# contineu-ai/ACMMP-Spherical

Measured on AMD Instinct MI355X. Metric: Mpixels/sec PatchMatch propagation + ms/depth-map, 2000x1500, 1/2/4/8 GPU, higher is better.
Workload: dtype f32

## Files before the change

acmmp-spherical_amd/acmmp/capi.py:

```python
from __future__ import annotations

import ctypes as C
import dataclasses
import mmap
import os
import threading
import weakref

import numpy as np

from .types import CAMERA_DTYPE, PARAMS_DTYPE

HERE = os.path.dirname(os.path.abspath(__file__))
LIB_PATH = os.environ.get("ACMMP_LIB") or os.path.join(HERE, "libacmmp.so")

class _HostPool:

    def __init__(self, cap: int | None = None):
        if cap is None:
            cap = int(os.environ.get("ACMMP_HOST_POOL_BYTES", str(1 << 30)))
        self.cap, self.held = cap, 0
        self.free = {}
        self.order = []
        self.lock = threading.Lock()

    def take(self, n: int):
        with self.lock:
            lst = self.free.get(n)
            if lst:
                mm = lst.pop()
                self.order = [(k, m) for (k, m) in self.order if m is not mm]
                self.held -= n
                return mm
        mm = mmap.mmap(-1, n, flags=mmap.MAP_PRIVATE | mmap.MAP_ANONYMOUS)
        if hasattr(mmap, "MADV_HUGEPAGE"):
            mm.madvise(mmap.MADV_HUGEPAGE)
        return mm

    def give(self, mm, n: int):
        if n > self.cap:
            return
        with self.lock:
            while self.held + n > self.cap and self.order:
                k, old = self.order.pop(0)
                self.free[k].remove(old)
                self.held -= k
            self.free.setdefault(n, []).append(mm)
            self.order.append((n, mm))
            self.held += n

    def release(self):
        with self.lock:
            self.free, self.order, self.held = {}, [], 0


_POOL = _HostPool()


def host_empty(shape, dtype=np.float32) -> np.ndarray:
    dt = np.dtype(dtype)
    count = int(np.prod(shape))
    n = count * dt.itemsize
    if n < (4 << 20):
        return np.empty(shape, dt)
    size = (n + (2 << 20) - 1) // (2 << 20) * (2 << 20) + (2 << 20)
    mm = _POOL.take(size)
    base = np.frombuffer(mm, np.uint8)
    off = (-base.ctypes.data) % (2 << 20)
    del base
    flat = np.frombuffer(mm, dt, count, off)
    weakref.finalize(flat, _POOL.give, mm, size)
    return flat.reshape(shape)


STATUS = {0: "ok", 1: "invalid argument", 2: "HIP runtime error", 3: "out of device memory",
          4: "call order violated", 5: "unsupported configuration", 6: "no HIP device"}

EXPORTS = [
    "acmmp_abi_version", "acmmp_device_count", "acmmp_create", "acmmp_destroy", "acmmp_status_str", "acmmp_last_error",
    "acmmp_set_params", "acmmp_upload_views", "acmmp_upload_depths", "acmmp_set_state",
    "acmmp_set_scaled_state", "acmmp_set_planar_prior", "acmmp_run_patchmatch", "acmmp_run_patchmatch_ex",
    "acmmp_download", "acmmp_download_aux", "acmmp_device_outputs", "acmmp_synchronize", "acmmp_last_timing",
    "acmmp_last_kernel_timing", "acmmp_last_work", "acmmp_last_planar_timing", "acmmp_texel_bytes", "acmmp_set_math", "acmmp_get_math", "acmmp_jbu",
    "acmmp_debug_ncc", "acmmp_debug_geom", "acmmp_debug_ncc_nb", "acmmp_debug_ncc_ref", "acmmp_debug_band_cvec",
    "acmmp_support_points", "acmmp_delaunay", "acmmp_prior_plane_params", "acmmp_depth_from_plane_param",
    "acmmp_planar_prior_host", "acmmp_set_planar_prior_from_maps", "acmmp_set_planar_prior_from_state",
    "acmmp_download_planar_prior",
    "acmmp_upload_depths_device", "acmmp_upload_views_device", "acmmp_export_depth", "acmmp_export_state", "acmmp_set_state_device", "acmmp_device_alloc", "acmmp_device_free", "acmmp_memcpy",
    "acmmp_comm_unique_id", "acmmp_comm_create", "acmmp_comm_destroy", "acmmp_comm_broadcast", "acmmp_comm_after",
    "acmmp_comm_allreduce_max", "acmmp_comm_band_exchange", "acmmp_run_patchmatch_band",
    "acmmp_band_begin", "acmmp_band_sweep", "acmmp_band_sweeps_left", "acmmp_band_halo_ranges",
    "acmmp_band_copy_rows", "acmmp_band_get_rows", "acmmp_band_set_rows", "acmmp_band_end",
    "acmmp_strip_plan",
    "acmmp_fusion_create", "acmmp_fusion_set_view", "acmmp_fusion_run", "acmmp_fusion_last_error",
    "acmmp_fusion_destroy", "acmmp_fusion_run_scene", "acmmp_fusion_scene_points", "acmmp_fusion_reset_used",
    "acmmp_fusion_download_used", "acmmp_fusion_voxelize", "acmmp_fusion_voxel_points", "acmmp_fusion_voxel_table",
    "acmmp_fusion_set_scene", "acmmp_fusion_voxel_clean", "acmmp_fusion_clean_points", "acmmp_fusion_voxel_labels",
    "acmmp_fusion_component_table",
    "acmmp_fusion_voxel_visibility", "acmmp_fusion_visible_points", "acmmp_fusion_visibility_tallies",
    "acmmp_fusion_voxel_mesh", "acmmp_fusion_mesh_vertices", "acmmp_fusion_mesh_faces", "acmmp_fusion_mesh_samples",
    "acmmp_fusion_mesh_table", "acmmp_fusion_set_mesh", "acmmp_fusion_mesh_render", "acmmp_fusion_render_maps",
    "acmmp_fusion_render_plan",
    "acmmp_fusion_set_reference_cloud", "acmmp_fusion_cloud_distance", "acmmp_fusion_distance_results",
    "acmmp_fusion_distance_grid",
    "acmmp_fusion_surface_distance", "acmmp_fusion_surface_results", "acmmp_fusion_surface_plan",
    "acmmp_fusion_surface_grid",
    "acmmp_fusion_set_cloud_transform", "acmmp_fusion_get_cloud_transform", "acmmp_fusion_cloud_align",
    "acmmp_fusion_align_records", "acmmp_fusion_cloud_align_plane", "acmmp_fusion_align_plane_records",
    "acmmp_image_cache_create", "acmmp_image_cache_destroy", "acmmp_image_cache_stats",
    "acmmp_upload_views_keyed", "acmmp_device_checksum", "acmmp_device_identity", "acmmp_clock_probe",
]


class AcmmpError(RuntimeError):
    pass


def strip_plan(rows: int, want_strips: int):
    L = load_library()
    bounds = np.zeros(65, np.int32)
    waits = np.full(192, -1, np.int32)
    ns = int(L.acmmp_strip_plan(int(rows), int(want_strips), _p(bounds), _p(waits)))
    if ns < 1:
        raise AcmmpError(f"strip_plan: invalid arguments (rows={rows})")
    return [int(b) for b in bounds[:ns + 1]], [[int(w) for w in waits[3 * i:3 * i + 3] if w >= 0] for i in range(ns)]


_lib = None


def load_library(path: str = LIB_PATH):
    global _lib
    if _lib is not None:
        return _lib
    if not os.path.exists(path):
        raise AcmmpError(f"{path} is missing: build it with `python acmmp-spherical_amd/build.py` "
                         "(there is no CPU fallback)")
    L = C.CDLL(path)
    vp, i32, u64 = C.c_void_p, C.c_int, C.c_uint64
    L.acmmp_abi_version.restype = i32
    L.acmmp_device_count.restype = i32
    L.acmmp_create.argtypes = [i32, C.POINTER(vp)]
    L.acmmp_destroy.argtypes = [vp]
    L.acmmp_destroy.restype = None
    L.acmmp_status_str.argtypes = [i32]
    L.acmmp_status_str.restype = C.c_char_p
    L.acmmp_last_error.argtypes = [vp]
    L.acmmp_last_error.restype = C.c_char_p
    L.acmmp_set_params.argtypes = [vp, vp]
    L.acmmp_upload_views.argtypes = [vp, i32, vp, vp, vp]
    L.acmmp_upload_depths.argtypes = [vp, i32, vp, vp, vp]
    L.acmmp_set_state.argtypes = [vp, vp, vp]
    L.acmmp_set_scaled_state.argtypes = [vp, vp, i32, i32]
    L.acmmp_set_planar_prior.argtypes = [vp, vp, vp]
    L.acmmp_run_patchmatch.argtypes = [vp, u64]
    L.acmmp_run_patchmatch_ex.argtypes = [vp, u64, i32, i32]
    L.acmmp_download.argtypes = [vp, vp, vp]
    L.acmmp_download_aux.argtypes = [vp, vp, vp]
    L.acmmp_device_outputs.argtypes = [vp, C.POINTER(vp), C.POINTER(vp)]
    L.acmmp_last_timing.argtypes = [vp, vp]
    L.acmmp_last_kernel_timing.argtypes = [vp, vp, vp]
    L.acmmp_last_work.argtypes = [vp, vp, vp]
    L.acmmp_last_planar_timing.argtypes = [vp, vp]
    L.acmmp_texel_bytes.argtypes = [vp]
    L.acmmp_set_math.argtypes = [vp, i32]
    L.acmmp_get_math.argtypes = [vp]
    L.acmmp_synchronize.argtypes = [vp]
    L.acmmp_jbu.argtypes = [vp, vp, i32, i32, vp, i32, i32, i32, vp]
    L.acmmp_debug_ncc.argtypes = [vp, i32, vp, vp, vp, vp]
    L.acmmp_debug_geom.argtypes = [vp, i32, vp, vp, vp, vp]
    L.acmmp_debug_ncc_nb.argtypes = [vp, i32, vp, vp, vp, vp]
    L.acmmp_debug_ncc_ref.argtypes = [vp, i32, vp, vp, vp, vp]
    L.acmmp_support_points.argtypes = [vp, i32, i32, vp, i32, vp]
    L.acmmp_delaunay.argtypes = [vp, i32, i32, i32, vp, i32, vp]
    L.acmmp_prior_plane_params.argtypes = [vp, vp, i32, i32, vp, vp]
    L.acmmp_depth_from_plane_param.argtypes = [vp, vp, i32, i32]
    L.acmmp_upload_depths_device.argtypes = [vp, i32, vp, vp, vp]
    L.acmmp_upload_views_device.argtypes = [vp, i32, vp, vp, vp]
    L.acmmp_export_depth.argtypes = [vp, vp]
    L.acmmp_export_state.argtypes = [vp, vp, vp]
    L.acmmp_set_state_device.argtypes = [vp, vp, vp]
    L.acmmp_device_alloc.argtypes = [i32, C.c_size_t, C.POINTER(vp)]
    L.acmmp_device_free.argtypes = [i32, vp]
    L.acmmp_memcpy.argtypes = [i32, vp, vp, C.c_size_t, i32]
    L.acmmp_comm_unique_id.argtypes = [vp]
    L.acmmp_comm_create.argtypes = [i32, vp, i32, i32, C.POINTER(vp)]
    L.acmmp_comm_destroy.argtypes = [vp]
    L.acmmp_comm_broadcast.argtypes = [vp, i32, vp, vp, vp]
    L.acmmp_comm_after.argtypes = [vp, vp]
    L.acmmp_comm_allreduce_max.argtypes = [vp, vp, i32]
    L.acmmp_comm_band_exchange.argtypes = [vp, vp, i32, i32, i32]
    L.acmmp_run_patchmatch_band.argtypes = [vp, vp, u64, i32, i32, i32, i32]
    L.acmmp_band_begin.argtypes = [vp, u64, i32, i32]
    L.acmmp_band_sweep.argtypes = [vp, C.POINTER(i32)]
    L.acmmp_band_sweeps_left.argtypes = [vp]
    L.acmmp_band_halo_ranges.argtypes = [vp, vp]
    L.acmmp_strip_plan.argtypes = [i32, i32, vp, vp]
    L.acmmp_band_copy_rows.argtypes = [vp, vp, i32, i32, i32]
    L.acmmp_band_get_rows.argtypes = [vp, i32, i32, i32, vp, vp, vp]
    L.acmmp_band_set_rows.argtypes = [vp, i32, i32, i32, vp, vp, vp]
    L.acmmp_debug_band_cvec.argtypes = [vp, i32, i32, i32, vp]
    L.acmmp_band_end.argtypes = [vp, i32]
    L.acmmp_fusion_create.argtypes = [i32, i32, vp, C.POINTER(vp)]
    L.acmmp_fusion_set_view.argtypes = [vp, i32, vp, vp, vp]
    L.acmmp_fusion_run.argtypes = [vp, i32, i32, vp, vp, i32, vp]
    L.acmmp_fusion_last_error.argtypes = [vp]
    L.acmmp_fusion_destroy.argtypes = [vp]
    L.acmmp_fusion_run_scene.argtypes = [vp, i32, vp, vp, vp, i32, vp, C.POINTER(C.c_int64)]
    L.acmmp_fusion_scene_points.argtypes = [vp, C.c_int64, C.c_int64, vp, vp, vp, vp]
    L.acmmp_fusion_reset_used.argtypes = [vp]
    L.acmmp_fusion_download_used.argtypes = [vp, i32, vp]
    L.acmmp_fusion_voxelize.argtypes = [vp, C.c_float, vp, i32, vp, vp, vp, vp]
    L.acmmp_fusion_voxel_points.argtypes = [vp, C.c_int64, C.c_int64, vp, vp]
    L.acmmp_fusion_voxel_table.argtypes = [vp, C.c_int64, vp, vp, vp, vp]
    L.acmmp_fusion_set_scene.argtypes = [vp, C.c_int64, vp, vp, vp, vp]
    L.acmmp_fusion_voxel_clean.argtypes = [vp, i32, i32, C.c_int64, C.c_int64, vp, vp, vp, vp, vp]
    L.acmmp_fusion_clean_points.argtypes = [vp, C.c_int64, C.c_int64, vp, vp, vp]
    L.acmmp_fusion_voxel_labels.argtypes = [vp, C.c_int64, C.c_int64, vp, vp]
    L.acmmp_fusion_component_table.argtypes = [vp, C.c_int64, C.c_int64, vp, vp, vp]
    L.acmmp_fusion_voxel_visibility.argtypes = [vp, i32, i32, vp, C.c_float, i32, i32, i32, vp, vp, vp, vp]
    L.acmmp_fusion_visible_points.argtypes = [vp, C.c_int64, C.c_int64, vp, vp, vp]
    L.acmmp_fusion_visibility_tallies.argtypes = [vp, C.c_int64, C.c_int64, vp]
    L.acmmp_fusion_voxel_mesh.argtypes = [vp, i32, i32, vp, C.c_float, i32, vp, vp, vp, vp, vp, vp]
    L.acmmp_fusion_mesh_vertices.argtypes = [vp, C.c_int64, C.c_int64, vp]
    L.acmmp_fusion_mesh_faces.argtypes = [vp, C.c_int64, C.c_int64, vp]
    L.acmmp_fusion_mesh_samples.argtypes = [vp, C.c_int64, C.c_int64, vp, vp, vp]
    L.acmmp_fusion_mesh_table.argtypes = [vp, C.c_int64, vp, vp, vp, vp]
    L.acmmp_fusion_set_mesh.argtypes = [vp, C.c_int64, vp, C.c_int64, vp]
    L.acmmp_fusion_mesh_render.argtypes = [vp, i32, vp, C.c_float, vp, vp]
    L.acmmp_fusion_render_maps.argtypes = [vp, vp, vp, vp, vp]
    L.acmmp_fusion_render_plan.argtypes = [vp, i32, vp, vp, vp]
    L.acmmp_fusion_set_reference_cloud.argtypes = [vp, C.c_int64, vp]
    L.acmmp_fusion_cloud_distance.argtypes = [vp, i32, i32, C.c_float, i32, vp, vp]
    L.acmmp_fusion_distance_results.argtypes = [vp, C.c_int64, C.c_int64, vp, vp]
    L.acmmp_fusion_distance_grid.argtypes = [vp, C.c_float, vp, vp, vp, vp]
    L.acmmp_fusion_surface_distance.argtypes = [vp, i32, C.c_float, i32, vp, vp]
    L.acmmp_fusion_surface_results.argtypes = [vp, C.c_int64, C.c_int64, vp, vp]
    L.acmmp_fusion_surface_plan.argtypes = [vp, i32, vp, vp, vp, vp]
    L.acmmp_fusion_surface_grid.argtypes = [vp, C.c_float, vp, vp, vp, vp]
    L.acmmp_fusion_set_cloud_transform.argtypes = [vp, vp]
    L.acmmp_fusion_get_cloud_transform.argtypes = [vp, vp, vp]
    L.acmmp_fusion_cloud_align.argtypes = [vp, i32, i32, C.c_float, i32, i32, C.c_double, vp, vp, vp, vp]
    L.acmmp_fusion_align_records.argtypes = [vp, C.c_int64, C.c_int64, vp, vp, vp]
    L.acmmp_fusion_cloud_align_plane.argtypes = [vp, i32, C.c_float, i32, i32, C.c_double, vp, vp, vp, vp]
    L.acmmp_fusion_align_plane_records.argtypes = [vp, C.c_int64, C.c_int64, vp, vp, vp]
    L.acmmp_planar_prior_host.argtypes = [vp, vp, vp, i32, i32, C.c_float, C.c_float, vp, vp, vp]
    L.acmmp_set_planar_prior_from_maps.argtypes = [vp, vp, vp, C.c_float, C.c_float, vp]
    L.acmmp_set_planar_prior_from_state.argtypes = [vp, C.c_float, C.c_float, vp]
    L.acmmp_download_planar_prior.argtypes = [vp, vp, vp]
    L.acmmp_image_cache_create.argtypes = [i32, C.c_size_t, C.POINTER(vp)]
    L.acmmp_image_cache_destroy.argtypes = [vp]
    L.acmmp_image_cache_stats.argtypes = [vp, vp]
    L.acmmp_upload_views_keyed.argtypes = [vp, vp, i32, vp, vp, vp, vp, i32]
    L.acmmp_device_checksum.argtypes = [i32, vp, C.c_size_t, vp]
    L.acmmp_device_identity.argtypes = [i32, vp, i32, vp]
    L.acmmp_clock_probe.argtypes = [i32, C.c_float, vp]
    for name in EXPORTS:
        fn = getattr(L, name)
        if name not in ("acmmp_destroy", "acmmp_status_str", "acmmp_last_error", "acmmp_abi_version", "acmmp_device_count",
                        "acmmp_depth_from_plane_param", "acmmp_comm_destroy", "acmmp_fusion_last_error",
                        "acmmp_fusion_destroy", "acmmp_image_cache_destroy"):
            fn.restype = i32
    L.acmmp_depth_from_plane_param.restype = C.c_float
    L.acmmp_fusion_last_error.restype = C.c_char_p
    L.acmmp_image_cache_destroy.restype = None
    _lib = L
    return L


def device_count() -> int:
    return int(load_library().acmmp_device_count())


def _p(a):
    return None if a is None else a.ctypes.data_as(C.c_void_p)


def checksum_host(arr) -> int:
    w = np.frombuffer(np.ascontiguousarray(arr).tobytes(), np.uint32).astype(np.uint64)
    z = (np.arange(w.size, dtype=np.uint64) << np.uint64(32)) | w
    with np.errstate(over="ignore"):
        z = (z ^ (z >> np.uint64(30))) * np.uint64(0xbf58476d1ce4e5b9)
        z = (z ^ (z >> np.uint64(27))) * np.uint64(0x94d049bb133111eb)
        z = z ^ (z >> np.uint64(31))
# ... 220 lines not shown
        return n.value

    def download_planar_prior(self):
        prior = host_empty((self.H, self.W, 4), np.float32)
        masks = host_empty((self.H, self.W), np.uint32)
        self._check(self.L.acmmp_download_planar_prior(self.h, _p(prior), _p(masks)), "download_planar_prior")
        return prior, masks

    def run_patchmatch(self, seed: int, n_half_sweeps: int = -1, do_post: bool = True):
        self._check(self.L.acmmp_run_patchmatch_ex(self.h, C.c_uint64(seed), n_half_sweeps, int(do_post)),
                    "run_patchmatch")

    def download(self):
        planes = host_empty((self.H, self.W, 4), np.float32)
        costs = host_empty((self.H, self.W), np.float32)
        self._check(self.L.acmmp_download(self.h, _p(planes), _p(costs)), "download")
        return planes, costs

    def download_into(self, planes, costs):
        for a, tail in ((planes, (4,)), (costs, ())):
            if a.dtype != np.float32 or not a.flags.c_contiguous or a.shape != (self.H, self.W) + tail:
                raise ValueError("download_into: need C-contiguous float32 (H, W, 4) planes and (H, W) costs")
        self._check(self.L.acmmp_download(self.h, _p(planes), _p(costs)), "download")

    def download_rows_into(self, planes, costs, row0: int, row1: int):
        n = row1 - row0
        for a, tail in ((planes, (4,)), (costs, ())):
            if a.dtype != np.float32 or not a.flags.c_contiguous or a.shape != (n, self.W) + tail:
                raise ValueError("download_rows_into: need C-contiguous float32 (rows, W, 4) and (rows, W)")
        if not (0 <= row0 < row1 <= self.H):
            raise ValueError("download_rows_into: rows outside the view")
        pp, cp = self.device_outputs()
        dev = self.device
        _host_check(self.L.acmmp_memcpy(dev, _p(planes), C.c_void_p(pp + 16 * row0 * self.W), 16 * n * self.W, 1),
                    "memcpy D2H")
        _host_check(self.L.acmmp_memcpy(dev, _p(costs), C.c_void_p(cp + 4 * row0 * self.W), 4 * n * self.W, 1),
                    "memcpy D2H")

    def download_aux(self):
        sel = host_empty((self.H, self.W), np.uint32)
        pre = host_empty((self.H, self.W), np.float32)
        self._check(self.L.acmmp_download_aux(self.h, _p(sel), _p(pre)), "download_aux")
        return sel, pre

    def device_outputs(self):
        a, b = C.c_void_p(), C.c_void_p()
        self._check(self.L.acmmp_device_outputs(self.h, C.byref(a), C.byref(b)), "device_outputs")
        return a.value, b.value

    BAND_HALO = 23

    def band_begin(self, seed: int, row0: int, row1: int):
        self._check(self.L.acmmp_band_begin(self.h, seed, row0, row1), "band_begin")

    def band_sweep(self) -> int:
        colour = C.c_int32(0)
        self._check(self.L.acmmp_band_sweep(self.h, C.byref(colour)), "band_sweep")
        return colour.value

    def band_sweeps_left(self) -> int:
        return int(self.L.acmmp_band_sweeps_left(self.h))

    def band_halo_ranges(self):
        r = np.zeros(8, np.int32)
        self._check(self.L.acmmp_band_halo_ranges(self.h, _p(r)), "band_halo_ranges")
        return tuple((int(r[2 * k]), int(r[2 * k + 1])) for k in range(4))

    def band_copy_rows_from(self, src: "Context", colour: int, row_a: int, row_b: int):
        self._check(self.L.acmmp_band_copy_rows(self.h, src.h, colour, row_a, row_b), "band_copy_rows")

    def band_get_rows(self, colour: int, row_a: int, row_b: int) -> np.ndarray:
        n = (row_b - row_a) * ((self.W + 1) // 2)
        pl = np.empty((n, 4), np.float32)
        co = np.empty(n, np.float32)
        sel = np.empty(n, np.uint32)
        self._check(self.L.acmmp_band_get_rows(self.h, colour, row_a, row_b, _p(pl), _p(co), _p(sel)), "band_get_rows")
        return np.concatenate([pl.view(np.uint32), co.view(np.uint32)[:, None], sel[:, None]], axis=1)

    def debug_band_cvec(self, colour: int, row_a: int, row_b: int) -> np.ndarray:
        out = np.empty((self.N - 1, (row_b - row_a) * ((self.W + 1) // 2)), np.float32)
        self._check(self.L.acmmp_debug_band_cvec(self.h, colour, row_a, row_b, _p(out)), "debug_band_cvec")
        return out

    def band_set_rows(self, colour: int, row_a: int, row_b: int, rows: np.ndarray):
        rows = np.asarray(rows, np.uint32).reshape(-1, 6)
        pl = np.ascontiguousarray(rows[:, :4]).view(np.float32)
        co = np.ascontiguousarray(rows[:, 4]).view(np.float32)
        sel = np.ascontiguousarray(rows[:, 5])
        self._check(self.L.acmmp_band_set_rows(self.h, colour, row_a, row_b, _p(pl), _p(co), _p(sel)), "band_set_rows")

    def band_end(self, do_post: bool = True):
        self._check(self.L.acmmp_band_end(self.h, int(do_post)), "band_end")

    def run_patchmatch_band(self, seed: int, row0: int, row1: int, comm=None, rank_up: int = -1,
                            rank_down: int = -1):
        self._check(self.L.acmmp_run_patchmatch_band(self.h, comm.h if comm is not None else None, seed, row0, row1,
                                                     rank_up, rank_down), "run_patchmatch_band")

    def synchronize(self):
        self._check(self.L.acmmp_synchronize(self.h), "synchronize")

    def last_timing(self):
        ms = np.zeros(3, np.float32)
        self._check(self.L.acmmp_last_timing(self.h, _p(ms)), "last_timing")
        return {"init_ms": float(ms[0]), "prop_ms": float(ms[1]), "post_ms": float(ms[2])}

    KERNELS = ("k_eval_nb", "k_select", "k_eval_ref", "k_finish")

    def last_kernel_timing(self):
        ms = np.zeros(4, np.float32)
        n = np.zeros(4, np.int32)
        self._check(self.L.acmmp_last_kernel_timing(self.h, _p(ms), _p(n)), "last_kernel_timing")
        return {k: (float(ms[i]), int(n[i])) for i, k in enumerate(self.KERNELS)}

    def last_work(self):
        e, t = C.c_ulonglong(0), C.c_ulonglong(0)
        self._check(self.L.acmmp_last_work(self.h, C.byref(e), C.byref(t)), "last_work")
        return e.value, t.value

    def last_planar_timing(self):
        ms = np.zeros(4, np.float32)
        self._check(self.L.acmmp_last_planar_timing(self.h, _p(ms)), "last_planar_timing")
        return {"support_ms": float(ms[0]), "delaunay_ms": float(ms[1]), "planes_ms": float(ms[2]),
                "device_ms": float(ms[3])}

    def texel_bytes(self) -> int:
        return int(self.L.acmmp_texel_bytes(self.h))

    def jbu(self, ref, coarse, imagescale: int):
        ref = np.ascontiguousarray(ref, np.float32)
        coarse = np.ascontiguousarray(coarse, np.float32)
        out = np.empty_like(ref)
        self._check(self.L.acmmp_jbu(self.h, _p(ref), ref.shape[1], ref.shape[0], _p(coarse), coarse.shape[1],
                                     coarse.shape[0], imagescale, _p(out)), "jbu")
        return out

    def _debug(self, fn, px, py, planes):
        px = np.ascontiguousarray(px, np.int32)
        py = np.ascontiguousarray(py, np.int32)
        pl = np.ascontiguousarray(planes, np.float32).reshape(-1, 4)
        out = np.empty((len(px), self.N - 1), np.float32)
        self._check(fn(self.h, len(px), _p(px), _p(py), _p(pl), _p(out)), "debug")
        return out

    def debug_ncc(self, px, py, planes):
        return self._debug(self.L.acmmp_debug_ncc, px, py, planes)

    def debug_geom(self, px, py, planes):
        return self._debug(self.L.acmmp_debug_geom, px, py, planes)

    def _debug_k(self, fn, k, px, py, planes, what):
        px = np.ascontiguousarray(px, np.int32)
        py = np.ascontiguousarray(py, np.int32)
        pl = np.ascontiguousarray(planes, np.float32).reshape(len(px), k, 4)
        out = np.empty((len(px), k, self.N - 1), np.float32)
        self._check(fn(self.h, len(px), _p(px), _p(py), _p(pl), _p(out)), what)
        return out

    def debug_ncc_nb(self, px, py, planes):
        return self._debug_k(self.L.acmmp_debug_ncc_nb, 8, px, py, planes, "debug_ncc_nb")

    def debug_ncc_ref(self, px, py, planes):
        return self._debug_k(self.L.acmmp_debug_ncc_ref, 5, px, py, planes, "debug_ncc_ref")



# ... 612 lines not shown
```

acmmp-spherical_amd/csrc/capi.cpp:

```cpp
#include "../../include/acmmp.h"

#include <hip/hip_runtime.h>

#include <algorithm>
#include <chrono>
#include <cmath>
#include <cstdio>
#include <cstdlib>
#include <cstring>
#include <mutex>
#include <string>
#include <type_traits>
#include <unordered_map>
#include <vector>

#include "devbuf.h"
#include "engine.h"
#include "planar.h"

using namespace acmmp;

static_assert(sizeof(acmmp_camera) == 120, "Camera layout (main.h:40-54)");
static_assert(sizeof(acmmp_params) == 68, "PatchMatchParams layout (ACMMP.h:32-55)");
static_assert(offsetof(acmmp_params, scaled_cols) == 52, "PatchMatchParams layout");
// ... 756 lines not shown
    const acmmp_status st = planar_triangles(c->cams[0], depths, costs, c->W, c->H, &pt);
    if (st != ACMMP_OK) return fail(c, st, "planar_triangles");
    c->planar_ms[0] = 0.f;
    c->planar_ms[1] = pt.delaunay_ms;
    c->planar_ms[2] = ms_since(t0) - pt.delaunay_ms;
    return upload_planar(c, pt, depth_min, depth_max, n_triangles);
}

acmmp_status acmmp_set_planar_prior_from_state(acmmp_ctx* c, float depth_min, float depth_max, int* n_triangles) {
    if (!c) return ACMMP_ERR_INVALID_ARGUMENT;
    if (c->N == 0) return fail(c, ACMMP_ERR_STATE, "upload_views and run_patchmatch first");
    if (!c->has_result) return fail(c, ACMMP_ERR_STATE, "no depth / cost maps since the last upload_views");
    HIP_TRY(c, hipSetDevice(c->device));
    const int W = c->W, H = c->H;
    const size_t nb = static_cast<size_t>((W + 4) / 5) * ((H + 4) / 5);
    const auto t0 = planar_clock::now();
    HIP_TRY(c, c->d_support.reserve_pow2(nb, static_cast<size_t>(1) << 17));
    HIP_TRY(c, launch_support_points(c->d_costs_rm, c->d_planes_rm, W, H, c->d_support, c->stream));
    std::vector<int4> blocks(nb);
    HIP_TRY(c, hipMemcpyAsync(blocks.data(), c->d_support, sizeof(int4) * nb, hipMemcpyDeviceToHost, c->stream));
    HIP_TRY(c, hipStreamSynchronize(c->stream));
    std::vector<int> xy;
    std::vector<float> depth_at;
    for (const int4& b : blocks) {
        if (!b.x) continue;
        xy.push_back(b.y);
        xy.push_back(b.z);
        float d;
        std::memcpy(&d, &b.w, sizeof d);
        depth_at.push_back(d);
    }
    c->planar_ms[0] = ms_since(t0);
    const auto t1 = planar_clock::now();
    PlanarTriangles pt;
    const acmmp_status st = planar_triangles_pts(c->cams[0], xy, depth_at, W, H, &pt);
    if (st != ACMMP_OK) return fail(c, st, "planar_triangles");
    c->planar_ms[1] = pt.delaunay_ms;
    c->planar_ms[2] = ms_since(t1) - pt.delaunay_ms;
    return upload_planar(c, pt, depth_min, depth_max, n_triangles);
}

acmmp_status acmmp_download_planar_prior(acmmp_ctx* c, float* prior, uint32_t* masks) {
    if (!c) return ACMMP_ERR_INVALID_ARGUMENT;
    if (!c->has_prior) return fail(c, ACMMP_ERR_STATE, "no planar prior set since the last upload_views");
    HIP_TRY(c, hipSetDevice(c->device));
    HIP_TRY(c, hipStreamSynchronize(c->stream));
    const size_t P = P_of(c);
    if (prior) HIP_TRY(c, d2h(prior, c->d_prior, sizeof(float4) * P));
    if (masks) HIP_TRY(c, d2h(masks, c->d_mask, sizeof(uint32_t) * P));
    return ACMMP_OK;
}

static unsigned long long colour_pixels(const acmmp_ctx* c, const KParams& kp, int colour) {
    unsigned long long n = 0;
    for (int y = kp.row_lo; y < kp.row_hi; ++y) {
        const int first = (y + colour) & 1;
        n += first < c->W ? static_cast<unsigned long long>((c->W - first + 1) / 2) : 0ull;
    }
    return n;
}

static int ref_split_point(int V, size_t Pc, bool interp_ref) {
    const char* e_on = std::getenv("ACMMP_REF_SPLIT");
    const char* e_at = std::getenv("ACMMP_REF_SPLIT_AT");
    const int enabled = e_on ? std::atoi(e_on) : 1;
    const int at = e_at ? std::atoi(e_at) : 0;
    if (!enabled || V < 2 || Pc >= (static_cast<size_t>(1) << 29)) return 0;
    if (at > 0) return at < V ? at : 0;
    if (interp_ref && V > 8) return 8;
    return V <= 4 ? V / 2 : 4;
}

static int default_strips(int model, int W, int H, int V) {
    return (model == kSphere && V <= 4 && static_cast<long long>(W) * H >= 2000000LL) ? 2 : 1;
}

int acmmp_strip_plan(int rows, int want_strips, int* bounds, int* waits) {
    if (rows < 1 || !bounds) return 0;
    const int ns = strip_plan(rows, want_strips, bounds);
    for (int i = 0; waits && i < ns; ++i) strip_waits(ns, i, waits + 3 * i);
    return ns;
}

static acmmp_status build_kparams(acmmp_ctx* c, KParams& kp, uint64_t seed, int want_strips = 1) {
    const acmmp_params& p = c->params;
    if (!c->has_params) return fail(c, ACMMP_ERR_STATE, "set_params first");
    if (c->N == 0) return fail(c, ACMMP_ERR_STATE, "upload_views first");
    if (p.num_images != c->N) return fail(c, ACMMP_ERR_INVALID_ARGUMENT, "params.num_images != uploaded images");
    if (p.geom_consistency && !c->has_depths) return fail(c, ACMMP_ERR_STATE, "geom_consistency needs upload_depths");
    if (p.planar_prior && !c->has_prior) return fail(c, ACMMP_ERR_STATE, "planar_prior needs set_planar_prior");
    if (!p.geom_consistency && p.hierarchy && !p.planar_prior && !c->has_scaled)
        return fail(c, ACMMP_ERR_STATE, "hierarchy needs set_scaled_state");
    if (p.upsample && !p.planar_prior && p.hierarchy &&
        (c->sw != static_cast<int>(p.scaled_cols) || c->sh != static_cast<int>(p.scaled_rows)))
        return fail(c, ACMMP_ERR_INVALID_ARGUMENT, "scaled_cols/rows != scaled state size");
    if (p.hierarchy && !p.upsample && !p.geom_consistency && !p.planar_prior && (c->sw != c->W || c->sh != c->H))
        return fail(c, ACMMP_ERR_INVALID_ARGUMENT, "hierarchy reuse needs a full-size scaled state");
    const int R = p.patch_size / 2;
    if (R > 64) return fail(c, ACMMP_ERR_UNSUPPORTED, "patch radius > 64");
    int nside = 0;
    for (int i = -R; i <= R; i += p.radius_increment) ++nside;
    kp = KParams{};
    kp.model = c->model;
    kp.W = c->W; kp.H = c->H; kp.Wh = Wh_of(c); kp.N = c->N; kp.V = c->N - 1;
    kp.R = R; kp.inc = p.radius_increment; kp.nside = nside; kp.S = nside * nside;
    kp.interp = c->model == kSphere && nside == 6 && 2000LL * R <= 5LL * c->W && 1000LL * R <= 5LL * c->H;
    kp.ref_neg_tau = -1.0f;
    if (kp.interp && c->math == ACMMP_MATH_FAST && c->tex16 && kp.V <= 4) {
        kp.ref_neg_tau = 0x1p-35f;
        if (const char* e = std::getenv("ACMMP_REF_NEG_TAU")) kp.ref_neg_tau = std::strtof(e, nullptr);
        if (const char* e = std::getenv("ACMMP_REF_NEG_SKIP")) if (std::atoi(e) == 0) kp.ref_neg_tau = -1.0f;
    }
    if (const char* e = std::getenv("ACMMP_INTERP")) kp.interp = kp.interp && std::atoi(e) != 0;
    kp.homog = 1;
    if (const char* e = std::getenv("ACMMP_PIN_HOMOG")) kp.homog = std::atoi(e) != 0;
    kp.spread_max = 256.0f;
    if (const char* e = std::getenv("ACMMP_SPREAD_MAX")) kp.spread_max = std::strtof(e, nullptr);
    kp.neg_tau = 0x1p-35f;
    if (const char* e = std::getenv("ACMMP_NEG_TAU")) kp.neg_tau = std::strtof(e, nullptr);
    if (const char* e = std::getenv("ACMMP_NEG_SKIP")) if (std::atoi(e) == 0) kp.neg_tau = -1.0f;
    kp.rows = std::min(c->H, 32 * (((c->H / 2) + 15) / 16));
    kp.row_lo = 0; kp.row_hi = kp.rows;
    kp.init_lo = 0; kp.init_hi = c->H;
    kp.merge_lo = 0; kp.merge_hi = c->H;
    for (int k = 0; k < 2; ++k) { kp.filt_lo[k] = 0; kp.filt_hi[k] = kp.rows; }
    kp.dpitch = c->W + 2 * R;
    kp.depth_min = p.depth_min; kp.depth_max = p.depth_max;
    kp.sigma_spatial = p.sigma_spatial; kp.sigma_color = p.sigma_color;
    kp.top_k = p.top_k;
    kp.geom = p.geom_consistency; kp.planar = p.planar_prior; kp.hier = p.hierarchy; kp.upsample = p.upsample;
    kp.scaled_cols = p.scaled_cols; kp.scaled_rows = p.scaled_rows;
    kp.sw = c->sw; kp.sh = c->sh;
    kp.seed_lo = static_cast<uint32_t>(seed);
    kp.seed_hi = static_cast<uint32_t>(seed >> 32);
    kp.Pc = static_cast<long long>(c->H) * kp.Wh;
    const size_t Pc = static_cast<size_t>(kp.Pc);

    if (kp.S > 64) return fail(c, ACMMP_ERR_UNSUPPORTED, "more than 64 patch samples (patch_size / radius_increment)");
    kp.cams = c->d_cams;
    if (c->dirs_R != R) {
        if (c->model == kSphere) {
            c->d_dirs.reset();
            HIP_TRY(c, c->d_sph_row.alloc(static_cast<size_t>(c->H + 2 * R)));
            HIP_TRY(c, c->d_sph_col.alloc(static_cast<size_t>(c->W + 2 * R)));
        } else {
            HIP_TRY(c, c->d_dirs.alloc(static_cast<size_t>(c->W + 2 * R) * (c->H + 2 * R)));
        }
        HIP_TRY(c, launch_ray_tables(kp, c->d_dirs, c->d_sph_row, c->d_sph_col, c->stream));
        c->dirs_R = R;
    }
    kp.color_den = 2.0f * p.sigma_color * p.sigma_color;
    HIP_TRY(c, c->d_spatial.reserve(static_cast<size_t>(c->model == kSphere ? c->H : 1) * kp.S));
    HIP_TRY(c, launch_spatial_table(kp, c->d_spatial, c->stream));
    kp.nb_chunk = nb_view_chunk(kp);
    kp.nb_tile = nb_tile_order(kp);
    size_t fix_max_pc = static_cast<size_t>(1) << 24;
    if (const char* e = std::getenv("ACMMP_NBFIX_MAX_PC")) fix_max_pc = std::min<size_t>(fix_max_pc, std::strtoull(e, nullptr, 10));
    const bool fixq = c->model == kSphere && c->math == ACMMP_MATH_FAST && c->tex16 && kp.interp && Pc < fix_max_pc;
    if (!fixq && c->model == kSphere && c->math == ACMMP_MATH_FAST && c->tex16 && kp.interp && Pc >= fix_max_pc) kp.interp = 0;
    if (!kp.interp || !kp.nb_tile) kp.neg_tau = -1.0f;
    if (c->math == ACMMP_MATH_FAST && (c->model != kSphere || (kp.interp && kp.V > 4))) want_strips = 1;
    int sb[kMaxStrips + 1];
    const int ns = strip_plan(kp.rows, want_strips, sb);
    const int ref_split = ref_split_point(kp.V, Pc, kp.model == kSphere && c->math == ACMMP_MATH_FAST && c->tex16 &&
                                                        kp.interp && kp.V > 4);
    size_t ref_blocks[kMaxStrips], fix_cap[kMaxStrips], fix_total = 0, ref_total = 0;
    for (int i = 0; i < ns; ++i) {
        const size_t srows = static_cast<size_t>(sb[i + 1] - sb[i]);
        const size_t nb_blocks = static_cast<size_t>(nb_block_count(static_cast<long long>(srows), kp.Wh, kp.nb_tile));
        ref_blocks[i] = (srows * kp.Wh + kRefPix - 1) / kRefPix;
        fix_cap[i] = !fixq ? 0 : std::max(
            (nb_blocks + kNbFixRegions - 1) / kNbFixRegions * kNbPix * 8 * static_cast<size_t>(kp.nb_chunk),
            (ref_blocks[i] + kNbFixRegions - 1) / kNbFixRegions * kRefSlots * static_cast<size_t>(std::max(ref_split, 0)));
        fix_total += fix_cap[i];
        ref_total += ref_blocks[i];
    }
    kp.cams = c->d_cams;
    kp.tex16 = c->tex16;
    kp.fast = c->math == ACMMP_MATH_FAST;
    kp.dep = c->d_dep;
    kp.dirs = c->d_dirs;
    kp.sph_row = c->d_sph_row;
    kp.sph_col = c->d_sph_col;
    kp.spatial = c->d_spatial;
    kp.planes_rm = c->d_planes_rm; kp.w_rm = c->d_w_rm; kp.costs_rm = c->d_costs_rm; kp.pre_rm = c->d_pre; kp.sel_rm = c->d_sel_rm;
    kp.scaled = c->d_scaled; kp.prior = c->d_prior; kp.mask = c->d_mask;
    for (int k = 0; k < 2; ++k) {
        kp.plane_cs[k] = c->d_plane_cs[k][0];
        kp.cost_cs[k] = c->d_cost_cs[k][0];
        kp.sel_cs[k] = c->d_sel_cs[k];
        kp.rng_cs[k] = c->d_rng_cs[k];
    }
    uint8_t* dead = nullptr;
    auto carve = [&](char* slab) -> size_t {
        size_t at = 0;
        auto piece = [&](auto*& field, size_t count) {
            using T = std::remove_reference_t<decltype(*field)>;
            field = slab ? reinterpret_cast<T*>(slab + at) : nullptr;
            at = (at + sizeof(T) * count + 255) & ~static_cast<size_t>(255);
        };
        const size_t VP = static_cast<size_t>(kp.V) * Pc;
        const size_t surv_n = std::max(5 * Pc + 256, ref_total * kRefSlots);
        piece(kp.hyp_cost, 8 * VP);
        piece(kp.nbpos, 8 * Pc);
        piece(kp.cand, 5 * Pc);
        piece(kp.cand_dep, 5 * Pc);
        piece(kp.cand_cost, 5 * Pc);
        piece(kp.pst, Pc);
        piece(kp.cvec[0], VP);
        piece(kp.cvec[1], VP);
        piece(kp.cand_vcost, 5 * VP);
        piece(kp.surv, surv_n);
        piece(kp.surv_count, std::max(Pc / 51 + 2, ref_total));
        piece(kp.psum, Pc);
        piece(kp.nbfix, kNbFixRegions * fix_total);
        piece(kp.nbfix_count, static_cast<size_t>(kNbFixRegions) * ns);
        piece(kp.surv_pre, std::max(Pc / 51 + 3, ref_total + ns));
        piece(kp.surv_dense, surv_n);
        piece(kp.cand_rough, 5 * Pc);
        piece(dead, 2 * Pc);
        return at;
    };
    HIP_TRY(c, c->d_scratch.reserve(carve(nullptr)));
    carve(c->d_scratch);
    if (!fixq) kp.nbfix = nullptr;
    {
        const char* e = std::getenv("ACMMP_DEAD_SKIP");
        const bool skip = c->model == kSphere && !(e && std::atoi(e) == 0);
        for (int k = 0; k < 2; ++k) kp.dead[k] = skip ? dead + k * Pc : nullptr;
    }
    kp.nbfix_cap = static_cast<unsigned>(fix_cap[0]);
    c->strips.assign(ns, StripSlice{});
    {
        size_t ref_at = 0, fix_at = 0;
        for (int i = 0; i < ns; ++i) {
            StripSlice& t = c->strips[i];
            t.row_lo = sb[i]; t.row_hi = sb[i + 1];
            t.surv = kp.surv + ref_at * kRefSlots;
            t.surv_count = kp.surv_count + ref_at;
            t.surv_pre = kp.surv_pre + ref_at + i;
            t.surv_dense = kp.surv_dense + ref_at * kRefSlots;
            t.nbfix = kp.nbfix ? kp.nbfix + kNbFixRegions * fix_at : nullptr;
            t.nbfix_count = kp.nbfix_count + kNbFixRegions * i;
            t.nbfix_cap = static_cast<unsigned>(fix_cap[i]);
            ref_at += ref_blocks[i];
            fix_at += fix_cap[i];
        }
    }
    kp.ref_split = ref_split;
    if (!c->d_work) HIP_TRY(c, c->d_work.alloc(258));
    kp.work = c->d_work;
    kp.status = reinterpret_cast<unsigned*>(c->d_work + 256);
    kp.dead_any = reinterpret_cast<unsigned*>(c->d_work + 257);
    kp.nb_views = kp.V >= 32 ? 0xFFFFFFFFu : ((1u << kp.V) - 1u);
    kp.nb_count_work = 1;
    return ACMMP_OK;
}

static acmmp_status run_begin(acmmp_ctx* c, const KParams& kp, hipStream_t s) {
    const size_t Pc = static_cast<size_t>(kp.Pc);
    HIP_TRY(c, hipMemsetAsync(c->d_work, 0, sizeof(unsigned long long) * 258, s));
    HIP_TRY(c, hipEventRecord(c->ev[0], s));
    HIP_TRY(c, launch_init(kp, s));
    for (int k = 0; k < 2; ++k) {
        HIP_TRY(c, hipMemcpyAsync(c->d_plane_cs[k][1], c->d_plane_cs[k][0], sizeof(float4) * Pc,
                                  hipMemcpyDeviceToDevice, s));
        HIP_TRY(c, hipMemcpyAsync(c->d_cost_cs[k][1], c->d_cost_cs[k][0], sizeof(float) * Pc,
                                  hipMemcpyDeviceToDevice, s));
    }
    HIP_TRY(c, hipEventRecord(c->ev[1], s));
    return ACMMP_OK;
}

static acmmp_status run_end(acmmp_ctx* c, const KParams& kp, const int cur[2], int do_post) {
    hipStream_t s = c->stream;
    HIP_TRY(c, hipEventRecord(c->ev[2], s));
    HIP_TRY(c, launch_post(kp, do_post, s));
    HIP_TRY(c, hipEventRecord(c->ev[3], s));
    if (!c->h_work) HIP_TRY(c, c->h_work.alloc(257));
    HIP_TRY(c, hipMemcpyAsync(c->h_work, c->d_work, sizeof(unsigned long long) * 257, hipMemcpyDeviceToHost, s));
    HIP_TRY(c, hipStreamSynchronize(s));
    for (int k = 0; k < 2; ++k) {
        if (cur[k]) {
            std::swap(c->d_plane_cs[k][0], c->d_plane_cs[k][1]);
            std::swap(c->d_cost_cs[k][0], c->d_cost_cs[k][1]);
        }
    }
    for (int i = 0; i < 3; ++i) HIP_TRY(c, hipEventElapsedTime(&c->timing[i], c->ev[i], c->ev[i + 1]));
    if (const unsigned long long status = c->h_work[256])
        return fail(c, ACMMP_ERR_HIP, "run status " + std::to_string(status) + ": an interpolation fallback queue overflowed");
    c->has_result = true;
    return ACMMP_OK;
}

acmmp_status acmmp_run_patchmatch_ex(acmmp_ctx* c, uint64_t seed, int n_half_sweeps, int do_post) {
    if (!c) return ACMMP_ERR_INVALID_ARGUMENT;
    HIP_TRY(c, hipSetDevice(c->device));
// ... 144 lines not shown
    c->band_cur[0] = c->band_cur[1] = 0;
    c->band_active = true;
    return ACMMP_OK;
}

acmmp_status acmmp_band_sweep(acmmp_ctx* c, int* colour_out) {
    if (!c) return ACMMP_ERR_INVALID_ARGUMENT;
    if (!c->band_active) return fail(c, ACMMP_ERR_STATE, "band_begin first");
    if (c->band_sw >= c->band_nsw) return fail(c, ACMMP_ERR_STATE, "every half-sweep of the run is done");
    HIP_TRY(c, hipSetDevice(c->device));
    KParams& kp = c->band_kp;
    const int sw = c->band_sw, colour = sw & 1, iter = sw / 2;
    int* cur = c->band_cur;
    SweepOut out{c->d_plane_cs[colour][cur[colour] ^ 1], c->d_cost_cs[colour][cur[colour] ^ 1]};
    HIP_TRY(c, launch_propagate(kp, colour, iter, out, c->stream, nullptr));
    cur[colour] ^= 1;
    kp.plane_cs[colour] = c->d_plane_cs[colour][cur[colour]];
    kp.cost_cs[colour] = c->d_cost_cs[colour][cur[colour]];
    ++c->band_sw;
    if (colour_out) *colour_out = colour;
    return ACMMP_OK;
}

int acmmp_band_sweeps_left(const acmmp_ctx* c) { return c && c->band_active ? c->band_nsw - c->band_sw : 0; }

acmmp_status acmmp_band_halo_ranges(const acmmp_ctx* c, int ranges[8]) {
    if (!c || !ranges) return ACMMP_ERR_INVALID_ARGUMENT;
    if (!c->band_active) return ACMMP_ERR_STATE;
    band_ranges(c->band_kp, c->band_lo, c->band_hi, ranges[0], ranges[1], ranges[2], ranges[3], ranges[4], ranges[5],
                ranges[6], ranges[7]);
    return ACMMP_OK;
}

acmmp_status acmmp_band_copy_rows(acmmp_ctx* dst, acmmp_ctx* src, int colour, int row_a, int row_b) {
    if (!dst || !src || dst == src) return ACMMP_ERR_INVALID_ARGUMENT;
    BandBuffers d{}, s{};
    acmmp_status st = band_buffers(dst, colour, &d);
    if (st == ACMMP_OK) st = band_buffers(src, colour, &s);
    if (st != ACMMP_OK) return st;
    if (d.Wh != s.Wh || dst->H != src->H || row_a < 0 || row_b > dst->H || row_a > row_b)
        return fail(dst, ACMMP_ERR_INVALID_ARGUMENT, "band contexts differ in size or rows out of range");
    if (row_a == row_b) return ACMMP_OK;
    HIP_TRY(src, hipSetDevice(src->device));
    HIP_TRY(src, hipStreamSynchronize(src->stream));
    HIP_TRY(dst, hipSetDevice(dst->device));
    const size_t off = static_cast<size_t>(row_a) * d.Wh, n = static_cast<size_t>(row_b - row_a) * d.Wh;
    HIP_TRY(dst, hipMemcpyAsync(d.plane + off, s.plane + off, sizeof(float4) * n, hipMemcpyDeviceToDevice, dst->stream));
    HIP_TRY(dst, hipMemcpyAsync(d.cost + off, s.cost + off, sizeof(float) * n, hipMemcpyDeviceToDevice, dst->stream));
    HIP_TRY(dst, hipMemcpyAsync(d.sel + off, s.sel + off, sizeof(uint32_t) * n, hipMemcpyDeviceToDevice, dst->stream));
    return ACMMP_OK;
}

acmmp_status acmmp_band_get_rows(acmmp_ctx* c, int colour, int row_a, int row_b, float* planes, float* costs,
                                 uint32_t* sel) {
    if (!c || !planes || !costs || !sel) return ACMMP_ERR_INVALID_ARGUMENT;
    BandBuffers b{};
    const acmmp_status st = band_buffers(c, colour, &b);
    if (st != ACMMP_OK) return st;
    if (row_a < 0 || row_b > c->H || row_a > row_b) return fail(c, ACMMP_ERR_INVALID_ARGUMENT, "rows out of range");
    if (row_a == row_b) return ACMMP_OK;
    HIP_TRY(c, hipSetDevice(c->device));
    HIP_TRY(c, hipStreamSynchronize(c->stream));
    const size_t off = static_cast<size_t>(row_a) * b.Wh, n = static_cast<size_t>(row_b - row_a) * b.Wh;
    HIP_TRY(c, d2h(planes, b.plane + off, sizeof(float4) * n));
    HIP_TRY(c, d2h(costs, b.cost + off, sizeof(float) * n));
    HIP_TRY(c, d2h(sel, b.sel + off, sizeof(uint32_t) * n));
    return ACMMP_OK;
}

acmmp_status acmmp_debug_band_cvec(acmmp_ctx* c, int colour, int row_a, int row_b, float* out) {
    if (!c || !out) return ACMMP_ERR_INVALID_ARGUMENT;
    BandBuffers b{};
    const acmmp_status st = band_buffers(c, colour, &b);
    if (st != ACMMP_OK) return st;
    if (row_a < 0 || row_b > c->H || row_a > row_b) return fail(c, ACMMP_ERR_INVALID_ARGUMENT, "rows out of range");
    if (row_a == row_b) return ACMMP_OK;
    HIP_TRY(c, hipSetDevice(c->device));
    HIP_TRY(c, hipStreamSynchronize(c->stream));
    const KParams& kp = c->band_kp;
    const size_t off = static_cast<size_t>(row_a) * b.Wh, n = static_cast<size_t>(row_b - row_a) * b.Wh;
    for (int v = 0; v < kp.V; ++v)
        HIP_TRY(c, d2h(out + static_cast<size_t>(v) * n, kp.cvec[colour] + static_cast<size_t>(v) * kp.Pc + off, sizeof(float) * n));
    return ACMMP_OK;
}

acmmp_status acmmp_band_set_rows(acmmp_ctx* c, int colour, int row_a, int row_b, const float* planes, const float* costs,
                                 const uint32_t* sel) {
    if (!c || !planes || !costs || !sel) return ACMMP_ERR_INVALID_ARGUMENT;
    BandBuffers b{};
    const acmmp_status st = band_buffers(c, colour, &b);
    if (st != ACMMP_OK) return st;
    if (row_a < 0 || row_b > c->H || row_a > row_b) return fail(c, ACMMP_ERR_INVALID_ARGUMENT, "rows out of range");
    if (row_a == row_b) return ACMMP_OK;
    HIP_TRY(c, hipSetDevice(c->device));
    const size_t off = static_cast<size_t>(row_a) * b.Wh, n = static_cast<size_t>(row_b - row_a) * b.Wh;
    HIP_TRY(c, hipMemcpyAsync(b.plane + off, planes, sizeof(float4) * n, hipMemcpyHostToDevice, c->stream));
    HIP_TRY(c, hipMemcpyAsync(b.cost + off, costs, sizeof(float) * n, hipMemcpyHostToDevice, c->stream));
    HIP_TRY(c, hipMemcpyAsync(b.sel + off, sel, sizeof(uint32_t) * n, hipMemcpyHostToDevice, c->stream));
    HIP_TRY(c, hipStreamSynchronize(c->stream));
    return ACMMP_OK;
}

acmmp_status acmmp_band_end(acmmp_ctx* c, int do_post) {
    if (!c) return ACMMP_ERR_INVALID_ARGUMENT;
    if (!c->band_active) return fail(c, ACMMP_ERR_STATE, "band_begin first");
    HIP_TRY(c, hipSetDevice(c->device));
    const acmmp_status st = run_end(c, c->band_kp, c->band_cur, do_post);
    c->band_active = false;
    return st;
}

acmmp_status acmmp_download(acmmp_ctx* c, float* planes, float* costs) {
    if (!c) return ACMMP_ERR_INVALID_ARGUMENT;
    if (c->N == 0) return fail(c, ACMMP_ERR_STATE, "nothing to download");
    HIP_TRY(c, hipSetDevice(c->device));
    const size_t P = P_of(c);
    if (planes) HIP_TRY(c, d2h(planes, c->d_planes_rm, sizeof(float4) * P));
    if (costs) HIP_TRY(c, d2h(costs, c->d_costs_rm, sizeof(float) * P));
    return ACMMP_OK;
}

acmmp_status acmmp_download_aux(acmmp_ctx* c, uint32_t* sel, float* pre) {
    if (!c) return ACMMP_ERR_INVALID_ARGUMENT;
    if (c->N == 0) return fail(c, ACMMP_ERR_STATE, "nothing to download");
    HIP_TRY(c, hipSetDevice(c->device));
    const size_t P = P_of(c);
    if (sel) HIP_TRY(c, d2h(sel, c->d_sel_rm, sizeof(uint32_t) * P));
    if (pre) HIP_TRY(c, d2h(pre, c->d_pre, sizeof(float) * P));
    return ACMMP_OK;
}

acmmp_status acmmp_device_outputs(acmmp_ctx* c, void** planes, void** costs) {
    if (!c) return ACMMP_ERR_INVALID_ARGUMENT;
    if (planes) *planes = c->d_planes_rm;
    if (costs) *costs = c->d_costs_rm;
    return ACMMP_OK;
}

acmmp_status acmmp_synchronize(acmmp_ctx* c) {
    if (!c) return ACMMP_ERR_INVALID_ARGUMENT;
    HIP_TRY(c, hipSetDevice(c->device));
    HIP_TRY(c, hipDeviceSynchronize());
    return ACMMP_OK;
}

acmmp_status acmmp_last_timing(const acmmp_ctx* c, float ms[3]) {
    if (!c || !ms) return ACMMP_ERR_INVALID_ARGUMENT;
    for (int i = 0; i < 3; ++i) ms[i] = c->timing[i];
    return ACMMP_OK;
}

acmmp_status acmmp_last_planar_timing(const acmmp_ctx* c, float ms[4]) {
    if (!c || !ms) return ACMMP_ERR_INVALID_ARGUMENT;
    for (int i = 0; i < 4; ++i) ms[i] = c->planar_ms[i];
    return ACMMP_OK;
}

acmmp_status acmmp_last_work(const acmmp_ctx* c, unsigned long long* evaluated, unsigned long long* total) {
    if (!c || !evaluated || !total) return ACMMP_ERR_INVALID_ARGUMENT;
    *evaluated = c->work_busy;
    *total = c->work_total;
    return ACMMP_OK;
}

int acmmp_texel_bytes(const acmmp_ctx* c) {
    if (!c || c->N == 0) return 0;
// ... 76 lines not shown
```

acmmp-spherical_amd/csrc/engine.h:

```cpp
#pragma once
#include <hip/hip_runtime.h>
#include <stdint.h>

#include "acmmp.h"

namespace acmmp {

constexpr int kPinhole = 0;
constexpr int kSphere = 11;
constexpr int kMaxViews = 32;
constexpr int kNbPix = 32;
constexpr int kNbFixRegions = 256;
constexpr int kRefLanes = 5;
constexpr int kRefPix = 51;
constexpr int kRefSlots = kRefPix * kRefLanes;
constexpr unsigned kStatusFixOverflow = 1u;

struct DevCam {
    float FRxy[6];
    float FRz[3];
    float Ft[3];
    float fkx, fky;
    float cx, cy;
    const uint16_t* img16_base;
// ... 12 lines not shown
    float inv_fx, inv_fy;
    float C[3];
    long long dep_off;
    int dep_w, dep_h;
    int img_bytes;
    const float* img_base;
};

struct PixState {
    float4 plane_now;
    float4 cur_plane;
    uint4 vw;
    float cost_now, depth_now, cur_cost, restricted_cost;
    uint32_t cur_sel, flags;
    float weight_norm;
    uint32_t src;
};

struct KParams {
    int model;
    int tex16;
    int fast;
    int W, H, Wh, N, V;
    int R, inc, nside, S;
    int interp;
    int homog;
    float spread_max;
    int rows;
    int row_lo, row_hi;
    int init_lo, init_hi;
    int merge_lo, merge_hi;
    int filt_lo[2], filt_hi[2];
    int dpitch;
    float depth_min, depth_max, sigma_spatial, sigma_color;
    int top_k;
    int geom, planar, hier, upsample;
    float scaled_cols, scaled_rows;
    int sw, sh;
    uint32_t seed_lo, seed_hi;
    const DevCam* cams;
    const float* dep;
    const float4* dirs;
    const float2* sph_row;
    const float2* sph_col;
    const float* spatial;
    float color_den;
    float neg_tau;
    float4* planes_rm;
    float* w_rm;
    float* costs_rm;
    float* pre_rm;
    uint32_t* sel_rm;
    const float4* scaled;
    const float4* prior;
    const uint32_t* mask;
    float4* plane_cs[2];
    float* cost_cs[2];
    uint32_t* sel_cs[2];
    uint32_t* rng_cs[2];
    float* hyp_cost;
    float* cvec[2];
    float* cand_vcost;
    int* nbpos;
    float4* cand;
    float* cand_dep;
    float* cand_cost;
    PixState* pst;
    unsigned long long* work;
    uint32_t nb_views;
    int nb_chunk;
    int nb_tile;
    int nb_count_work;
    long long Pc;
    int ref_split;
    float ref_neg_tau;
    uint32_t* surv;
    unsigned* surv_count;
    unsigned* surv_pre;
    uint32_t* surv_dense;
    float4* psum;
    uint32_t* nbfix;
    unsigned* nbfix_count;
    unsigned nbfix_cap;
    uint32_t* cand_rough;
    uint8_t* dead[2];
    unsigned* dead_any;
    unsigned* status;
};

struct SweepOut {
    float4* plane;
    float* cost;
};

constexpr int kMaxStrips = 64;
constexpr int kMaxStripStreams = 4;

struct StripSlice {
    int row_lo, row_hi;
    uint32_t* surv;
    unsigned* surv_count;
    unsigned* surv_pre;
    uint32_t* surv_dense;
    uint32_t* nbfix;
    unsigned* nbfix_count;
    unsigned nbfix_cap;
};

inline int strip_plan(int rows, int want, int* bounds) {
    const int units = rows / 4, per = (ACMMP_BAND_HALO + 3) / 4;
    int ns = want < 1 ? 1 : (want > kMaxStrips ? kMaxStrips : want);
    if (ns > units / per) ns = units / per;
    if (ns < 1) ns = 1;
    int at = 0;
    for (int i = 0; i < ns; ++i) {
        bounds[i] = 4 * at;
        at += units / ns + (i < units % ns ? 1 : 0);
    }
    bounds[0] = 0;
    bounds[ns] = rows;
    return ns;
}

inline void strip_waits(int ns, int i, int waits[3]) {
    waits[0] = (ns > 1 && i > 0) ? i - 1 : -1;
    waits[1] = ns > 1 ? i : -1;
    waits[2] = (ns > 1 && i + 1 < ns) ? i + 1 : -1;
}

inline int cdiv(long long a, int b) { return static_cast<int>((a + b - 1) / b); }

hipError_t launch_ray_tables(const KParams& kp, float4* dirs, float2* sph_row, float2* sph_col, hipStream_t s);
hipError_t launch_spatial_table(const KParams& kp, float* spatial, hipStream_t s);
hipError_t launch_init(const KParams& kp, hipStream_t s);
hipError_t launch_propagate(const KParams& kp, int colour, int iter, SweepOut out, hipStream_t s,
                            hipEvent_t* ev = nullptr, bool all_marks = true);
hipError_t launch_post(const KParams& kp, int do_post, hipStream_t s);
DevCam make_devcam(const acmmp_camera& cam);
void set_relative_frame(DevCam& d, const acmmp_camera& ref, const acmmp_camera& cam);
struct BandBuffers {
    float4* plane;
    float* cost;
    uint32_t* sel;
    int Wh;
    hipStream_t stream;
    int device;
};
acmmp_status band_buffers(acmmp_ctx* c, int colour, BandBuffers* out);
acmmp_status engine_stream(acmmp_ctx* c, int* device, hipStream_t* stream);

hipError_t launch_jbu(const float* ref, int W, int H, const float* coarse, int sw, int sh, int imagescale,
                      float* out, hipStream_t s);
hipError_t launch_export_depth(const float4* planes, long long P, float* dst, hipStream_t s);
hipError_t launch_copy(const void* src, void* dst, size_t bytes, hipStream_t s);
struct ClockStamp {
    unsigned long long cycles, ticks;
};
hipError_t launch_clock_probe(const float* rnd, int iters, int blocks, ClockStamp* stamps, float* sink, hipStream_t s);
hipError_t launch_checksum(const void* ptr, size_t bytes, unsigned long long* out, hipStream_t s);
int nb_view_chunk(const KParams& kp);
int nb_tile_order(const KParams& kp);
inline long long nb_block_count(long long rows, long long Wh, int tile) {
    return tile ? ((rows + 3) / 4) * ((Wh + 7) / 8) : (rows * Wh + 31) / 32;
}
hipError_t launch_debug(const KParams& kp, int which, int n, const int* px, const int* py, const float4* planes,
                        float* out, hipStream_t s);
hipError_t launch_debug_nb(const KParams& kp, int n, const int* px, const int* py, const float4* planes, float* out,
                           hipStream_t s);
hipError_t launch_debug_ref(const KParams& kp, int n, const int* px, const int* py, const float4* planes, float* out,
                            hipStream_t s);
hipError_t launch_to_f16_pairs(const float* src, int W, int H, uint32_t* dst, int* inexact, hipStream_t s);
// ... 14 lines not shown
```

acmmp-spherical_amd/csrc/kernels.hip:

```cpp
#include <algorithm>
#include <cstdlib>

#include "camera_dev.h"
#include "detmath.h"
#include "engine.h"

#ifndef ACMMP_TU
#define ACMMP_TU -1
#endif
#define ACMMP_IN_TU(n) (ACMMP_TU < 0 || ACMMP_TU == (n))

namespace acmmp {

typedef float f32x2 __attribute__((ext_vector_type(2)));
__device__ __forceinline__ f32x2 pk_fma(f32x2 a, f32x2 b, f32x2 c) { return __builtin_elementwise_fma(a, b, c); }
__device__ __forceinline__ f32x2 splat2(float x) { return (f32x2){x, x}; }


__device__ __forceinline__ uint4 philox10(uint32_t c0, uint32_t c1, uint32_t c2, uint32_t c3, uint32_t k0,
                                          uint32_t k1) {
#pragma unroll
    for (int r = 0; r < 10; ++r) {
        const uint32_t lo0 = 0xD2511F53u * c0, hi0 = __umulhi(0xD2511F53u, c0);
        const uint32_t lo1 = 0xCD9E8D57u * c2, hi1 = __umulhi(0xCD9E8D57u, c2);
// ... 143 lines not shown
    t = pk_fma((f32x2){c.FRxy[2], c.FRxy[3]}, splat2(P.y), t);
    t = pk_fma((f32x2){c.FRxy[4], c.FRxy[5]}, splat2(P.z), t);
    tz = fmaf(c.FRz[2], P.z, fmaf(c.FRz[1], P.y, fmaf(c.FRz[0], P.x, fz)));
}

template <int MODEL, typename Cam>
__device__ __forceinline__ void project_fast(Cam& c, float3 P, float& ox, float& oy, const float* ft = nullptr) {
    f32x2 t;
    float tz;
    rigid_fast(c, P, t, tz, ft);
    if (MODEL == kSphere) {
        sphere_pixel_fast(c, t, tz, ox, oy);
    } else {
        const f32x2 o = t * splat2(__builtin_amdgcn_rcpf(tz));
        ox = o.x;
        oy = o.y;
    }
}

template <int MODEL, typename Cam>
__device__ __forceinline__ float3 cam_point_fast(Cam& c, int x, int y, float depth, float4 d) {
    if (MODEL == kSphere) return make_float3(d.x * depth, d.y * depth, d.z * depth);
    return make_float3((depth * (static_cast<float>(x) - c.K[2])) * c.inv_fx,
                       (depth * (static_cast<float>(y) - c.K[5])) * c.inv_fy, depth);
}

__device__ __forceinline__ float depth_from_plane_fast(float4 ph, float4 d) {
    const float denom = dot3(ph.x, ph.y, ph.z, d.x, d.y, d.z);
    return (fabsf(denom) < 1e-6f) ? 1e6f : (-ph.w * __builtin_amdgcn_rcpf(denom));
}

__device__ __forceinline__ float dist_to_origin(float4 d, float depth, float4 n) {
    return -dot3(n.x, n.y, n.z, d.x * depth, d.y * depth, d.z * depth);
}

__device__ __forceinline__ float4 to_world(const DevCam& c, float4 n) {
    return make_float4(dot3(c.R[0], c.R[3], c.R[6], n.x, n.y, n.z), dot3(c.R[1], c.R[4], c.R[7], n.x, n.y, n.z),
                       dot3(c.R[2], c.R[5], c.R[8], n.x, n.y, n.z), n.w);
}
__device__ __forceinline__ float4 to_ref(const DevCam& c, float4 n) {
    return make_float4(dot3(c.R[0], c.R[1], c.R[2], n.x, n.y, n.z), dot3(c.R[3], c.R[4], c.R[5], n.x, n.y, n.z),
                       dot3(c.R[6], c.R[7], c.R[8], n.x, n.y, n.z), n.w);
}

__device__ __forceinline__ float dot3n(float4 a, float4 b) { return dot3(a.x, a.y, a.z, b.x, b.y, b.z); }


__device__ __forceinline__ int clampi(int v, int lo, int hi) { return v < lo ? lo : (v > hi ? hi : v); }

__device__ __forceinline__ float texel_padded(const float* img, int pitch, int W, int H, int ix, int iy) {
    return img[static_cast<long long>(clampi(iy, 0, H - 1) + 1) * pitch + clampi(ix, 0, W - 1) + 1];
}

__device__ __forceinline__ float texel_plain(const float* img, int W, int H, int ix, int iy) {
    return img[static_cast<long long>(clampi(iy, 0, H - 1)) * W + clampi(ix, 0, W - 1)];
}


template <int MODEL>
__device__ __forceinline__ float4 ray_at(const KParams& kp, int x, int y) {
    if (MODEL == kSphere) {
        const float2 r = kp.sph_row[y + kp.R];
        const float2 c = kp.sph_col[x + kp.R];
        return make_float4(r.y * c.x, -r.x, r.y * c.y, 0.0f);
    }
    return kp.dirs[static_cast<long long>(y + kp.R) * kp.dpitch + (x + kp.R)];
}
__device__ __forceinline__ long long cs_index(const KParams& kp, int x, int y) {
    return static_cast<long long>(y) * kp.Wh + (x >> 1);
}
__device__ __forceinline__ int uniform_int(int v) { return __builtin_amdgcn_readfirstlane(v); }


struct Patch {
    const float4* rw;
    const float* rr;
    const float2* wr;
    const float2* row;
    const float2* col;
    int stride;
    float center;
    float sbw, sref, srr;
    const uint32_t* neg = nullptr;
};

typedef float float2u __attribute__((ext_vector_type(2), aligned(4)));

__device__ __forceinline__ float bilinear_pair(const float* img, int pitch, int W, int H, float x, float y) {
    const float fx = floorf(x), fy = floorf(y);
    const float a = x - fx, b = y - fy;
    const int ix = clampi(f2i_sat(fx), -1, W - 1);
    const int iy = clampi(f2i_sat(fy), -1, H - 1);
    const float* p0 = img + static_cast<long long>(iy + 1) * pitch + (ix + 1);
    const float2u top = *reinterpret_cast<const float2u*>(p0);
    const float2u bot = *reinterpret_cast<const float2u*>(p0 + pitch);
    const float r0 = fmaf(a, top.y - top.x, top.x);
    const float r1 = fmaf(a, bot.y - bot.x, bot.x);
    return fmaf(b, r1 - r0, r0);
}

typedef unsigned u32x2 __attribute__((ext_vector_type(2)));
struct Tap {
    float a, b;
    f32x2 top, bot;
    u32x2 pw;
};

template <int TEX, bool Y_IN_RANGE, typename Cam>
__device__ __forceinline__ Tap fetch_tap(__amdgpu_buffer_rsrc_t rs, Cam& c, float x, float y) {
    const float fx = floorf(x), fy = floorf(y);
    Tap t;
    t.a = x - fx;
    t.b = y - fy;
    if (TEX == 1) {
        t.a = __builtin_amdgcn_fractf(x);
        t.b = __builtin_amdgcn_fractf(y);
        const unsigned ix4 = (static_cast<unsigned>(clamp_m1(cvt_flr_i32(x), c.Wm1)) << 2) + 4u;
        if (Y_IN_RANGE) {
            const unsigned off = mad_u24(static_cast<unsigned>(cvt_flr_i32(y)), c.pitch4, ix4);
            t.pw = __builtin_amdgcn_raw_buffer_load_b64(rs, off, c.pitch4, 0);
        } else {
            const unsigned off = mad_u24(static_cast<unsigned>(clamp_m1(cvt_flr_i32(y), c.Hm1) + 1), c.pitch4, ix4);
            t.pw = __builtin_amdgcn_raw_buffer_load_b64(rs, off, 0, 0);
        }
        return t;
    }
    const unsigned ix4 = (static_cast<unsigned>(clamp_m1(cvt_i32(fx), c.Wm1)) << 2) + 4u;
    if (Y_IN_RANGE) {
        const unsigned off = mad_u24(static_cast<unsigned>(cvt_i32(fy)), c.pitch4, ix4);
        t.top = __builtin_bit_cast(f32x2, __builtin_amdgcn_raw_buffer_load_b64(rs, off, c.pitch4, 0));
        t.bot = __builtin_bit_cast(f32x2, __builtin_amdgcn_raw_buffer_load_b64(rs, off, 2 * c.pitch4, 0));
    } else {
        const unsigned off = mad_u24(static_cast<unsigned>(clamp_m1(cvt_i32(fy), c.Hm1) + 1), c.pitch4, ix4);
        t.top = __builtin_bit_cast(f32x2, __builtin_amdgcn_raw_buffer_load_b64(rs, off, 0, 0));
        t.bot = __builtin_bit_cast(f32x2, __builtin_amdgcn_raw_buffer_load_b64(rs, off, c.pitch4, 0));
    }
    return t;
}

template <typename Cam>
__device__ __forceinline__ bool pin_in_image(Cam& c, int ix, int iy) {
    return (static_cast<unsigned>(ix) <= static_cast<unsigned>(c.Wm1)) &
           (static_cast<unsigned>(iy) <= static_cast<unsigned>(c.Hm1));
}

template <int TEX>
__device__ __forceinline__ Tap fetch_tap_pin_p(__amdgpu_buffer_rsrc_t rs, int pitch4, float x, float y, int ix, int iy) {
    Tap t;
    const unsigned off = mad_u24(static_cast<unsigned>(iy), pitch4, (static_cast<unsigned>(ix) << 2) + 4u);
    if (TEX == 1) {
        t.a = __builtin_amdgcn_fractf(x);
        t.b = __builtin_amdgcn_fractf(y);
        t.pw = __builtin_amdgcn_raw_buffer_load_b64(rs, off, pitch4, 0);
        return t;
    }
    t.a = x - floorf(x);
    t.b = y - floorf(y);
    t.top = __builtin_bit_cast(f32x2, __builtin_amdgcn_raw_buffer_load_b64(rs, off, pitch4, 0));
    t.bot = __builtin_bit_cast(f32x2, __builtin_amdgcn_raw_buffer_load_b64(rs, off, 2 * pitch4, 0));
    return t;
}
template <int TEX, typename Cam>
__device__ __forceinline__ Tap fetch_tap_pin(__amdgpu_buffer_rsrc_t rs, Cam& c, float x, float y, int ix, int iy) {
    return fetch_tap_pin_p<TEX>(rs, c.pitch4, x, y, ix, iy);
}

__device__ __forceinline__ float f16_fma_lo(float a, float d, unsigned v) {
// ... 34 lines not shown
template <int MODEL>
__device__ __forceinline__ float4 patch_sample(const KParams& kp, int px, int py, int s, int i, int j, float center,
                                               float& r) {
    const DevCam& rc = kp.cams[0];
    r = texel_padded(rc.img_base, rc.img_pitch, rc.W, rc.H, px + i, py + j);
    const float sp = kp.spatial[(MODEL == kSphere ? static_cast<long long>(py) * kp.S : 0) + s];
    const float w = det_exp(sp - fabsf(r - center) / kp.color_den);
    const float4 d = ray_at<MODEL>(kp, px + i, py + j);
    return make_float4(d.x, d.y, d.z, w);
}

__device__ __forceinline__ void patch_fold_sample(float w, float r, Patch& pt) {
    pt.sbw += w;
    pt.sref = fmaf(w, r, pt.sref);
    pt.srr = fmaf(w * r, r, pt.srr);
}

template <int MODEL>
__device__ __forceinline__ void patch_sums(const KParams& kp, Patch& pt, int px, int py) {
    pt.sbw = 0.f; pt.sref = 0.f; pt.srr = 0.f;
    if (MODEL == kSphere) {
        for (int s = 0; s < kp.S; ++s) {
            float r;
            const float w = patch_sample<MODEL>(kp, px, py, s, -kp.R + (s / kp.nside) * kp.inc,
                                                -kp.R + (s % kp.nside) * kp.inc, pt.center, r).w;
            patch_fold_sample(w, r, pt);
        }
    }
}

template <int MODEL>
__device__ __forceinline__ Patch make_patch(const KParams& kp, int px, int py) {
    const DevCam& rc = kp.cams[0];
    Patch pt;
    pt.rw = nullptr; pt.rr = nullptr; pt.wr = nullptr; pt.row = pt.col = nullptr; pt.stride = 0;
    pt.center = texel_padded(rc.img_base, rc.img_pitch, rc.W, rc.H, px, py);
    patch_sums<MODEL>(kp, pt, px, py);
    return pt;
}


__device__ __forceinline__ float ncc_cost(float sbw, f32x2 srrr, f32x2 ssrs, float sss) {
    asm volatile("" : "+v"(sbw), "+v"(srrr));
    float out = 2.0f;
    if (!(sbw < 1e-6f)) {
        const float inv = 1.0f / sbw;
        const float m_ref = srrr.x * inv, m_src = ssrs.x * inv;
        const float e_rr = srrr.y * inv, e_ss = sss * inv, e_rs = ssrs.y * inv;
        const float var_ref = fmaf(-m_ref, m_ref, e_rr);
        const float var_src = fmaf(-m_src, m_src, e_ss);
        if (!(var_ref < 1e-5f || var_src < 1e-5f)) {
            const float covar = fmaf(-m_ref, m_src, e_rs);
            const float ncc = 1.0f - covar / sqrtf(var_ref * var_src);
            out = fmaxf(0.0f, fminf(2.0f, ncc));
        }
    }
    return out;
}

template <int TEX, typename Cam>
__device__ __forceinline__ float sphere_sample_texel(Cam& c, float4 ph, __amdgpu_buffer_rsrc_t rs, float4 rw) {
    const float dep = depth_from_plane_fast(ph, rw);
    float x, y;
    project_fast<kSphere>(c, cam_point_fast<kSphere>(c, 0, 0, dep, rw), x, y);
    x = fmaf(-floorf(x * c.invW), c.Wf, x);
    y = __builtin_amdgcn_fmed3f(y, 0.0f, c.Hm1f);
    return lerp_tap<TEX>(fetch_tap<TEX, true>(rs, c, x, y));
}

__device__ __forceinline__ void sphere_fold_sample(float w, float r, float sp, f32x2& ssrs, float& sss) {
    const f32x2 wwr = (f32x2){w, w * r};
    ssrs = pk_fma(wwr, splat2(sp), ssrs);
    const float ws = w * sp;
    sss = fmaf(ws, sp, sss);
}

constexpr uint32_t kFixNone = ~0u, kFixNan = ~0u - 1u;

__device__ __forceinline__ int lane_id_here() {
    int l;
    asm volatile("v_mbcnt_lo_u32_b32 %0, -1, 0\n\tv_mbcnt_hi_u32_b32 %0, -1, %0" : "=v"(l));
    return l;
}
template <int MODEL, int VB, int STAGED, bool PIPE, int TEX, int FM = 0, bool FULL = false, int NB = 0, bool PNEG = false>
__device__ __forceinline__ void ncc_chunk(const KParams& kp, int px, int py, const Patch& pt, float4 ph,
                                          const int (&vlist)[VB], int nv_rt, float (&cost)[VB],
                                          uint32_t fixkey = kFixNone) {
    const int nv = FULL ? VB : uniform_int(nv_rt);
    constexpr bool kScalarGuard = MODEL == kSphere && STAGED == 3 && FM;
    auto has = [&](int v) -> bool {
        if (FULL) return true;
        if constexpr (kScalarGuard) {
            int n;
            asm volatile("s_mov_b32 %0, %1" : "=s"(n) : "s"(nv));
            return v < n;
        }
        return v < nv;
    };
    if (MODEL == kSphere && pt.sbw < 1e-6f) {
#pragma unroll
        for (int v = 0; v < VB; ++v) cost[v] = 2.0f;
        return;
    }
    const DevCam& rc = kp.cams[0];
    float sbw[VB], sss[VB];
    f32x2 ssrs[VB], srrr[VB];
    bool cval[VB];
    int cv[VB];
#pragma unroll
    for (int v = 0; v < VB; ++v) cv[v] = uniform_int(v < nv ? vlist[v] : vlist[0]);
    typedef const __attribute__((address_space(4))) DevCam ConstCam;
    ConstCam* ccams = (ConstCam*)(kp.cams);
#define PCV(v) ccams[cv[v]]
    const float4 dc = ray_at<MODEL>(kp, px, py);
    const float3 Pc3 = FM ? cam_point_fast<MODEL>(rc, px, py, depth_from_plane_fast(ph, dc), dc)
                          : world_point_ray<MODEL>(rc, px, py, depth_from_plane(ph, dc), dc);
#pragma unroll
    for (int v = 0; v < VB; ++v) {
        sbw[v] = pt.sbw;
        srrr[v] = (f32x2){pt.sref, pt.srr};
        sss[v] = 0.f;
        ssrs[v] = splat2(0.f);
        cval[v] = true;
        if (MODEL == kPinhole && v < nv) {
            float ox, oy, od;
            if (FM) project_fast<MODEL>(PCV(v), Pc3, ox, oy);
            else project<MODEL>(PCV(v), Pc3, ox, oy, od);
            cval[v] = !(ox < 0.0f || ox >= PCV(v).Wf || oy < 0.0f || oy >= PCV(v).Hf);
        }
    }
    constexpr bool kFtV = FM && MODEL == kSphere && STAGED == 3 && !(TEX == 1);
    float ftv[VB][3];
#pragma unroll
    for (int v = 0; v < VB; ++v) {
#pragma unroll
        for (int k = 0; k < 3; ++k) {
            ftv[v][k] = 0.f;
            if (kFtV) asm volatile("v_mov_b32 %0, %1" : "=v"(ftv[v][k]) : "s"(PCV(v).Ft[k]));
        }
    }
    const int R = kp.R, inc = kp.inc;
    constexpr int G = PIPE ? VB : 1;
#define ACMMP_ACCUMULATE_Z(v, T, W_, WWR_, R_, OK_, ZERO_)                   \
    do {                                                             \
        const float sp = (ZERO_) ? 0.f : lerp_tap<TEX>(T);           \
        if (MODEL == kPinhole) {                                     \
            const bool ok_ = (OK_);                                  \
            const f32x2 wwr_ = ok_ ? (WWR_) : splat2(0.f);           \
            const float sp_ = ok_ ? sp : 0.f;                        \
            sbw[v] += wwr_.x;                                        \
            srrr[v] = pk_fma(wwr_, splat2(R_), srrr[v]);             \
            ssrs[v] = pk_fma(wwr_, splat2(sp_), ssrs[v]);            \
            const float ws = wwr_.x * sp_;                           \
            sss[v] = fmaf(ws, sp_, sss[v]);                          \
        } else if (has(v)) {                                         \
            ssrs[v] = pk_fma(WWR_, splat2(sp), ssrs[v]);             \
            const float ws = (W_) * sp;                              \
            sss[v] = fmaf(ws, sp, sss[v]);                           \
        }                                                            \
    } while (0)
#define ACMMP_ACCUMULATE_T(v, T, W_, WWR_, R_, OK_) ACMMP_ACCUMULATE_Z(v, T, W_, WWR_, R_, OK_, false)
#define ACMMP_ACCUMULATE(v) ACMMP_ACCUMULATE_T(v, tap[v], w, wwr, r, ok[v])
    constexpr bool kInterp = FM && MODEL == kSphere && STAGED == 3 && TEX == 1;
    int interp_done = 0;
    uint32_t rough_nan = 0u;
    if constexpr (kInterp) {
        if (kp.interp) if (fixkey != kFixNone) {
// ... 216 lines not shown
                z0[v] = hz;
                hiz[v] = hi[2];
                hjz[v] = hj[2];
            }
        }
        __amdgpu_buffer_rsrc_t rsv[VB];
        int wm1[VB], hm1[VB], p4[VB];
        float ftz[VB];
#pragma unroll
        for (int v = 0; v < VB; ++v) {
            ConstCam& c = PCV(v);
            rsv[v] = TEX == 1
                ? __builtin_amdgcn_make_buffer_rsrc(const_cast<uint16_t*>(c.img16_base), 0, c.img16_bytes, 0x00020000)
                : __builtin_amdgcn_make_buffer_rsrc(const_cast<float*>(c.img_base), 0, c.img_bytes, 0x00020000);
            wm1[v] = uniform_int(c.Wm1);
            hm1[v] = uniform_int(c.Hm1);
            p4[v] = uniform_int(c.pitch4);
            ftz[v] = c.Ft[2];
        }
        int s = 0;
        for (int i = -R; i <= R; i += inc) {
            const float fi = static_cast<float>(i);
            f32x2 nr[VB];
            float zr[VB];
#pragma unroll
            for (int v = 0; v < VB; ++v) {
                nr[v] = pk_fma(splat2(fi), hi2[v], n0[v]);
                zr[v] = fmaf(fi, hiz[v], z0[v]);
            }
            auto issue = [&](int jv, int sv, Tap (&tp)[VB], bool (&okv)[VB], float& w_o, float& r_o, f32x2& wwr_o) {
                const float fj = static_cast<float>(jv);
                const float4 q = pt.rw[sv * pt.stride];
                r_o = pt.rr[sv * pt.stride];
                const float D = dot3(ph.x, ph.y, ph.z, q.x, q.y, q.z);
                const float dS = (fabsf(D) < 1e-6f ? w_clamp : -D) - s0;
                w_o = q.w;
                wwr_o = (f32x2){w_o, w_o * r_o};
#pragma unroll
                for (int v = 0; v < VB; ++v) {
                    okv[v] = false;
                    if (has(v)) {
                        f32x2 nn = pk_fma(splat2(fj), hj2[v], nr[v]);
                        float tz = fmaf(fj, hjz[v], zr[v]);
                        nn = pk_fma(splat2(dS), ft2[v], nn);
                        tz = fmaf(dS, ftz[v], tz);
                        const f32x2 o = pk_fma(nn, splat2(__builtin_amdgcn_rcpf(tz)), xy0[v]);
                        const int ix = cvt_flr_i32(o.x), iy = cvt_flr_i32(o.y);
                        okv[v] = (static_cast<unsigned>(ix) <= static_cast<unsigned>(wm1[v])) &
                                 (static_cast<unsigned>(iy) <= static_cast<unsigned>(hm1[v]));
                        tp[v] = fetch_tap_pin_p<TEX>(rsv[v], p4[v], o.x, o.y, ix, iy);
                    }
                }
            };
            int j = -R;
            if constexpr (NB ? ACMMP_PIN_PAIRS : ACMMP_PIN_PAIRS_REF) {
                for (; j + inc <= R; j += 2 * inc, s += 2) {
                    Tap ta[VB], tb[VB];
                    bool oka[VB], okb[VB];
                    float wa, ra, wb, rb;
                    f32x2 wwra, wwrb;
                    issue(j, s, ta, oka, wa, ra, wwra);
                    issue(j + inc, s + 1, tb, okb, wb, rb, wwrb);
#pragma unroll
                    for (int v = 0; v < VB; ++v)
                        if (has(v)) ACMMP_ACCUMULATE_T(v, ta[v], wa, wwra, ra, oka[v]);
#pragma unroll
                    for (int v = 0; v < VB; ++v)
                        if (has(v)) ACMMP_ACCUMULATE_T(v, tb[v], wb, wwrb, rb, okb[v]);
                }
            }
            for (; j <= R; j += inc, ++s) {
                Tap tap[VB];
                bool ok[VB];
                float w, r;
                f32x2 wwr;
                issue(j, s, tap, ok, w, r, wwr);
#pragma unroll
                for (int v = 0; v < VB; ++v)
                    if (has(v)) ACMMP_ACCUMULATE(v);
            }
        }
    }
    if (!interp_done) {
        const float neg_lim = PNEG ? kp.ref_neg_tau * pt.sbw : 0.f;
#define ACMMP_ACCUMULATE_N(v) ACMMP_ACCUMULATE_Z(v, tap[v], w, wwr, r, ok[v], PNEG && mine)
        int s = 0, ii = 0;
        for (int i = -R; i <= R; i += inc, ++ii) {
            int jj = 0;
            const float2 cs = STAGED == 4 ? pt.col[ii] : make_float2(0.f, 0.f);
            for (int j = -R; j <= R; j += inc, ++s, ++jj) {
                float r;
                float4 rw;
                if (STAGED == 4) {
                    const float2 rs = pt.row[jj];
                    const float2 q = pt.wr[s];
                    rw = make_float4(rs.y * cs.x, -rs.x, rs.y * cs.y, q.x);
                    r = q.y;
                } else if (STAGED == 3) {
                    const float4 q = pt.rw[s * pt.stride];
                    if (MODEL == kSphere) {
                        rw = make_float4(q.x, pt.rr[jj * pt.stride], q.y, q.z);
                        r = q.w;
                    } else {
                        rw = q;
                        r = pt.rr[s * pt.stride];
                    }
                } else {
                    rw = patch_sample<MODEL>(kp, px, py, s, i, j, pt.center, r);
                }
                const bool mine = PNEG && rw.w <= neg_lim;
                if constexpr (PNEG) if (__all(mine)) continue;
                const float w = mine ? 0.f : rw.w;
                float3 P;
                const float dep = FM ? depth_from_plane_fast(ph, rw) : depth_from_plane(ph, rw);
                if (FM)
                    P = cam_point_fast<MODEL>(ccams[0], px + i, py + j, dep, rw);
                else if (!PIPE)
                    P = world_point_ray<MODEL>(ccams[0], px + i, py + j, dep, rw);
                else
                    P = world_point_ray<MODEL>(rc, px + i, py + j, dep, rw);
                const float wr = w * r;
                const f32x2 wwr = (f32x2){w, wr};
                Tap tap[VB];
                bool ok[VB];
#pragma unroll
                for (int v = 0; v < VB; ++v) {
                    ok[v] = false;
                    if (has(v)) {
                        ConstCam& c = PCV(v);
                        float sx, sy, sd;
                        if (FM) project_fast<MODEL>(c, P, sx, sy, kFtV ? ftv[v] : nullptr);
                        else project<MODEL>(c, P, sx, sy, sd);
                        ok[v] = true;
                        const __amdgpu_buffer_rsrc_t rs = TEX == 1
                            ? __builtin_amdgcn_make_buffer_rsrc(const_cast<uint16_t*>(c.img16_base), 0, c.img16_bytes, 0x00020000)
                            : __builtin_amdgcn_make_buffer_rsrc(const_cast<float*>(c.img_base), 0, c.img_bytes, 0x00020000);
                        if (MODEL == kSphere) {
                            sx = fmaf(-floorf(sx * c.invW), c.Wf, sx);
                            sy = FM ? __builtin_amdgcn_fmed3f(sy, 0.0f, c.Hm1f) : clamp0(sy, c.Hm1f);
                            tap[v] = fetch_tap<TEX, true>(rs, c, sx, sy);
                        } else {
                            const int ix = cvt_flr_i32(sx), iy = cvt_flr_i32(sy);
                            ok[v] = pin_in_image(c, ix, iy);
                            tap[v] = fetch_tap_pin<TEX>(rs, c, sx, sy, ix, iy);
                        }
                        if (G == 1) ACMMP_ACCUMULATE_N(v);
                    }
                    if (FULL && MODEL == kSphere) __builtin_amdgcn_sched_barrier(0);
                    if (G > 1 && ((v + 1) % G == 0 || v == VB - 1)) {
#pragma unroll
                        for (int u = v - (v % G); u <= v; ++u)
                            if (has(u)) ACMMP_ACCUMULATE_N(u);
                    }
                }
            }
        }
    }
#undef ACMMP_ACCUMULATE
#undef ACMMP_ACCUMULATE_N
#undef ACMMP_ACCUMULATE_T
#undef ACMMP_ACCUMULATE_Z
#pragma unroll
    for (int v = 0; v < VB; ++v) {
        cost[v] = cval[v] ? ncc_cost(sbw[v], srrr[v], ssrs[v], sss[v]) : 2.0f;
        if (kInterp && ((rough_nan >> v) & 1u)) cost[v] = __builtin_nanf("");
    }
#undef PCV
}

template <int MODEL>
__device__ __forceinline__ float geom_cost(const KParams& kp, int sv, float4 ph, int px, int py, float4 dc) {
    const DevCam& rc = kp.cams[0];
    const DevCam& sc = kp.cams[sv];
    const float depth = depth_from_plane(ph, dc);
    const float3 fwd = world_point_ray<MODEL>(rc, px, py, depth, dc);
    float sx, sy, sd;
    project<MODEL>(sc, fwd, sx, sy, sd);
    const float src_depth = texel_plain(kp.dep + sc.dep_off, sc.dep_w, sc.dep_h, f2i_sat(sx), f2i_sat(sy));
    if (src_depth == 0.0f) return 3.0f;
    const float3 s3 = world_point<MODEL>(sc, sx, sy, src_depth);
    float bx, by, bd;
    project<MODEL>(rc, s3, bx, by, bd);
    const float dcol = static_cast<float>(px) - bx, drow = static_cast<float>(py) - by;
    return fminf(3.0f, sqrtf(fmaf(drow, drow, dcol * dcol)));
}

__device__ __forceinline__ uint32_t wave_or(uint32_t mask, int V) {
    uint32_t r = 0u;
    for (int v = 0; v < V; ++v)
        if (__ballot((mask >> v) & 1u)) r |= 1u << v;
    return uniform_int(static_cast<int>(r));
}


__device__ __forceinline__ float sample_depth_inv(Rng& rs, float dmin, float dmax) {
    dmin = fmaxf(dmin, 1e-6f);
    dmax = fmaxf(dmax, dmin + 1e-6f);
    const float inv_min = 1.0f / dmax;
    const float inv_max = 1.0f / dmin;
    const float u = rs.uniform();
    const float inv = fmaf(u, inv_max - inv_min, inv_min);
    return 1.0f / inv;
}

__device__ __forceinline__ float4 random_normal(float4 v, Rng& rs) {
    float q1 = 1.0f, q2 = 1.0f, s = 2.0f;
    while (s >= 1.0f) {
        q1 = fmaf(2.0f, rs.uniform(), -1.0f);
        q2 = fmaf(2.0f, rs.uniform(), -1.0f);
        s = fmaf(q2, q2, q1 * q1);
    }
    const float sq = sqrtf(1.0f - s);
    float4 n = make_float4((2.0f * q1) * sq, (2.0f * q2) * sq, fmaf(-2.0f, s, 1.0f), 0.0f);
    if (dot3n(n, v) > 0.0f) { n.x = -n.x; n.y = -n.y; n.z = -n.z; }
    normalize3(n.x, n.y, n.z);
    return n;
}

__device__ __forceinline__ float4 perturbed_normal(float4 v, float4 n, Rng& rs, float perturbation) {
    const float a1 = (rs.uniform() - 0.5f) * perturbation;
    const float a2 = (rs.uniform() - 0.5f) * perturbation;
    const float a3 = (rs.uniform() - 0.5f) * perturbation;
    float s1, c1, s2, c2, s3, c3;
    det_sincos(a1, &s1, &c1);
    det_sincos(a2, &s2, &c2);
    det_sincos(a3, &s3, &c3);
    const float R0 = c2 * c3;
    const float R1 = fmaf(-c1, s3, (c3 * s1) * s2);
    const float R2 = fmaf(c1 * c3, s2, s1 * s3);
    const float R3 = c2 * s3;
    const float R4 = fmaf(s1 * s2, s3, c1 * c3);
    const float R5 = fmaf(-c3, s1, (c1 * s2) * s3);
    const float R6 = -s2;
    const float R7 = c2 * s1;
    const float R8 = c1 * c2;
    float4 p = make_float4(dot3(R0, R1, R2, n.x, n.y, n.z), dot3(R3, R4, R5, n.x, n.y, n.z),
                           dot3(R6, R7, R8, n.x, n.y, n.z), n.w);
    if (dot3n(p, v) >= 0.0f) p = n;
    normalize3(p.x, p.y, p.z);
    return p;
}


template <int MODEL, int VB, int STAGED, bool PIPE, int TEX, int FM, int NOFULL = 0, bool PNEG = false, typename F>
__device__ __forceinline__ void for_all_views_t(const KParams& kp, int px, int py, const Patch& pt, float4 ph,
                                                uint32_t wave_mask, F&& f, uint32_t fixkey = kFixNone) {
    int v = 0;
    const int V = kp.V;
    while (true) {
        int vlist[VB];
        int nv = 0;
#pragma unroll
        for (int k = 0; k < VB; ++k) vlist[k] = 1;
        while (v < V && nv < VB) {
            if ((wave_mask >> v) & 1u) {
#pragma unroll
                for (int k = 0; k < VB; ++k)
                    if (k == nv) vlist[k] = v + 1;
                ++nv;
            }
            ++v;
        }
        if (nv == 0) break;
        float cost[VB];
        constexpr bool kFullCopy = (MODEL == kSphere ? VB <= 2 : true) && VB > 1 &&
                                   !(NOFULL && MODEL == kSphere && STAGED == 3 && FM && TEX == 1);
        if (kFullCopy && nv == VB)
            ncc_chunk<MODEL, VB, STAGED, PIPE, TEX, FM, true, NOFULL, PNEG>(kp, px, py, pt, ph, vlist, nv, cost, fixkey);
        else
            ncc_chunk<MODEL, VB, STAGED, PIPE, TEX, FM, false, NOFULL, PNEG>(kp, px, py, pt, ph, vlist, nv, cost, fixkey);
#pragma unroll
        for (int k = 0; k < VB; ++k)
            if (k < nv) f(vlist[k] - 1, cost[k]);
        if (v >= V) break;
    }
}

template <int MODEL, int VB, int STAGED, bool PIPE, bool PIPE_FM = PIPE, typename F>
__device__ __forceinline__ void for_all_views(const KParams& kp, int px, int py, const Patch& pt, float4 ph,
                                              uint32_t wave_mask, F&& f) {
    if (kp.fast) {
        if (kp.tex16) for_all_views_t<MODEL, VB, STAGED, PIPE_FM, 1, 1>(kp, px, py, pt, ph, wave_mask, f);
        else for_all_views_t<MODEL, VB, STAGED, PIPE_FM, 0, 1>(kp, px, py, pt, ph, wave_mask, f);
    } else {
        if (kp.tex16) for_all_views_t<MODEL, VB, STAGED, PIPE, 1, 0>(kp, px, py, pt, ph, wave_mask, f);
        else for_all_views_t<MODEL, VB, STAGED, PIPE, 0, 0>(kp, px, py, pt, ph, wave_mask, f);
    }
}

template <int MODEL, int VB, int STAGED, bool PIPE, int TF, bool PIPE_FM = PIPE, bool PNEG = false, typename F>
__device__ __forceinline__ void for_all_views_tf(const KParams& kp, int px, int py, const Patch& pt, float4 ph,
                                                 uint32_t wave_mask, F&& f, uint32_t fixkey = kFixNone) {
    if constexpr (TF == 0) {
        if (kp.fast) for_all_views_t<MODEL, VB, STAGED, PIPE_FM, 0, 1>(kp, px, py, pt, ph, wave_mask, f);
        else for_all_views_t<MODEL, VB, STAGED, PIPE, 0, 0>(kp, px, py, pt, ph, wave_mask, f);
    } else {
        for_all_views_t<MODEL, VB, STAGED, TF == 2 ? PIPE_FM : PIPE, 1, TF == 2 ? 1 : 0, 0, PNEG && TF == 2 && MODEL == kSphere>(
            kp, px, py, pt, ph, wave_mask, f, fixkey);
    }
}
static inline int tf_of(const KParams& kp) { return kp.tex16 ? (kp.fast ? 2 : 1) : 0; }

__device__ __forceinline__ float vw_get(const uint32_t (&vwp)[4], int v) {
    const uint32_t word = v < 8 ? vwp[0] : (v < 16 ? vwp[1] : (v < 24 ? vwp[2] : vwp[3]));
    return static_cast<float>((word >> ((v & 7) * 4)) & 15u);
}

constexpr unsigned kXcdStrip = 256;
__device__ __forceinline__ long long xcd_block(unsigned b) {
    const unsigned x = b & 7u, k = b >> 3;
    const unsigned j = k / kXcdStrip, r = k - j * kXcdStrip;
    return (static_cast<long long>(j) * 8 + x) * kXcdStrip + r;
}

static inline unsigned xcd_grid(long long nblocks) {
    const long long strips = (nblocks + kXcdStrip - 1) / kXcdStrip;
    return static_cast<unsigned>((strips + 7) / 8 * 8 * kXcdStrip);
}


#if ACMMP_IN_TU(0)
__global__ void k_to_f16_pairs(const float* __restrict__ src, int W2, int rows, uint32_t* __restrict__ dst,
                               int* __restrict__ inexact) {
    const long long i = static_cast<long long>(blockIdx.x) * blockDim.x + threadIdx.x;
    if (i >= static_cast<long long>(W2) * rows) return;
    uint32_t out = 0;
#pragma unroll
    for (int k = 0; k < 2; ++k) {
        const float x = src[i + k * W2];
        const _Float16 h = static_cast<_Float16>(x);
        if (!(static_cast<float>(h) == x) || (x != 0.0f && !(fabsf(x) >= 6.103515625e-05f)) || fabsf(x) > 65504.0f)
            atomicOr(inexact, 1);
        out |= static_cast<uint32_t>(__builtin_bit_cast(uint16_t, h)) << (16 * k);
    }
    dst[i] = out;
}

__global__ void k_pad_image(const float* __restrict__ src, size_t pitch, int W, int H, float* __restrict__ dst,
                            int dpitch) {
    const int x = blockIdx.x * blockDim.x + threadIdx.x - 1;
    const int y = blockIdx.y * blockDim.y + threadIdx.y - 1;
    if (x > W || y > H) return;
    dst[static_cast<long long>(y + 1) * dpitch + (x + 1)] =
        src[static_cast<long long>(clampi(y, 0, H - 1)) * pitch + clampi(x, 0, W - 1)];
}

__global__ void k_ray_tables(const KParams kp, float4* __restrict__ dirs, float2* __restrict__ sph_row,
                             float2* __restrict__ sph_col) {
    const int x = blockIdx.x * blockDim.x + threadIdx.x;
    const int y = blockIdx.y * blockDim.y + threadIdx.y;
    const int TW = kp.W + 2 * kp.R, TH = kp.H + 2 * kp.R;
    const DevCam& c = kp.cams[0];
    if (kp.model == kSphere) {
        if (y == 0 && x < TW) {
            const float lon = (static_cast<float>(x - kp.R) - c.cx) / static_cast<float>(c.W) * 2.0f * kCudartPiF;
            float sl, cl;
            det_sincos(lon, &sl, &cl);
            sph_col[x] = make_float2(sl, cl);
        }
        if (y == 1 && x < TH) {
            const float lat = -(static_cast<float>(x - kp.R) - c.cy) / static_cast<float>(c.H) * kCudartPiF;
            float sa, ca;
            det_sincos(lat, &sa, &ca);
            sph_row[x] = make_float2(sa, ca);
        }
        return;
    }
    if (x >= TW || y >= TH) return;
    const float3 d = pixel_to_dir(c, x - kp.R, y - kp.R);
    dirs[static_cast<long long>(y) * kp.dpitch + x] = make_float4(d.x, d.y, d.z, 0.0f);
}

__global__ void k_spatial(const KParams kp, float* __restrict__ spatial) {
    const int y = blockIdx.x * blockDim.x + threadIdx.x;
    const int rows = kp.model == kSphere ? kp.H : 1;
    if (y >= rows) return;
    const DevCam& rc = kp.cams[0];
    float scale_x = 1.0f, scale_y = 1.0f, sig = kp.sigma_spatial;
    if (kp.model == kSphere) {
        const float lat_c = -(static_cast<float>(y) - rc.cy) / static_cast<float>(rc.H) * kCudartPiF;
        scale_x = (2.0f * kCudartPiF / static_cast<float>(rc.W)) * det_cos(lat_c);
        scale_y = (kCudartPiF / static_cast<float>(rc.H));
        sig = kp.sigma_spatial * (kCudartPiF / static_cast<float>(rc.H));
    }
    int s = 0;
    for (int i = -kp.R; i <= kp.R; i += kp.inc) {
        for (int j = -kp.R; j <= kp.R; j += kp.inc, ++s) {
            const float dx = kp.model == kSphere ? static_cast<float>(i) * scale_x : static_cast<float>(i);
            const float dy = kp.model == kSphere ? static_cast<float>(j) * scale_y : static_cast<float>(j);
            const float sd = sqrtf(fmaf(dy, dy, dx * dx));
            spatial[static_cast<long long>(y) * kp.S + s] = (-sd) / (2.0f * sig * sig);
        }
    }
}

#endif


__device__ __forceinline__ void sort_small(float* d, int n) {
    int j;
    for (int i = 1; i < n; i++) {
        const float tmp = d[i];
        for (j = i; j >= 1 && tmp < d[j - 1]; j--) d[j] = d[j - 1];
        d[j] = tmp;
    }
}

template <int MODEL, int VB, int VMAXB, int TF, bool PNEG = false>
__device__ float initial_cost(const KParams& kp, int px, int py, const Patch& pt, float4 ph, uint32_t* sel,
                              float* cvec = nullptr) {
    constexpr int VMAX = VMAXB < 8 ? VMAXB : kMaxViews;
    float cv[VMAX], cvc[VMAX];
    int nvalid = 0;
    const uint32_t all = kp.V >= 32 ? 0xFFFFFFFFu : ((1u << kp.V) - 1u);
    for_all_views_tf<MODEL, VB, 0, true, TF, true, PNEG>(kp, px, py, pt, ph, all, [&](int v, float c) {
        cv[v] = c;
        cvc[v] = c;
        if (c < 2.0f) nvalid++;
    });
    if (cvec)
        for (int v = 0; v < kp.V; ++v) cvec[v * kp.Pc] = cvc[v];
    sort_small(cv, kp.V);
    *sel = 0;
    const int top_k = nvalid < kp.top_k ? nvalid : kp.top_k;
    if (top_k > 0) {
        float cost = 0.0f;
        for (int i = 0; i < top_k; ++i) cost += cv[i];
        const float thr = cv[top_k - 1];
        for (int i = 0; i < kp.V; ++i)
            if (cvc[i] <= thr) *sel |= (1u << i);
        return cost / static_cast<float>(top_k);
    }
    return 2.0f;
}

__device__ __forceinline__ float spatial_gauss(float x1, float y1, float x2, float y2, float sigma) {
    const float dx = x1 - x2, dy = y1 - y2;
    const float dis = (dx * dx + dy * dy) - 0.0f;
    return det_exp(-dis / (2.0f * sigma * sigma));
}
__device__ __forceinline__ float range_gauss(float x, float sigma) {
    const float xp = x - 0.0f;
    return det_exp(-(xp * xp) / (2.0f * sigma * sigma));
}


enum InitBranch { kInitRandom = 0, kInitPlanar = 1, kInitUpsample = 2, kInitReuse = 3 };

[[maybe_unused]] constexpr int kInitVB = 4;

template <int MODEL, int VB, int BR, int VMAXB, int TF, bool PNEG = false>
__global__ __launch_bounds__(256) void k_init(const KParams kp) {
    const long long tile = xcd_block(blockIdx.x);
    const int tiles_x = (kp.W + 15) >> 4;
    const int x = static_cast<int>(tile % tiles_x) * 16 + threadIdx.x;
    const int y = kp.init_lo + static_cast<int>(tile / tiles_x) * 16 + threadIdx.y;
    if (x >= kp.W || y >= kp.init_hi) return;
    const DevCam& rc = kp.cams[0];
    const long long center = static_cast<long long>(y) * kp.W + x;
    const int colour = (x + y) & 1;
    const long long ci = cs_index(kp, x, y);
    const Patch pt = make_patch<MODEL>(kp, x, y);
    if (MODEL == kSphere && kp.dead[0]) {
        const bool dead = pt.sbw < 1e-6f;
        (colour ? kp.dead[1] : kp.dead[0])[ci] = dead ? 1 : 0;
        if (dead) *kp.dead_any = 1u;
    }
    float* cvec = kp.cvec[colour] + ci;
    Rng rs;
    rs.init(kp.seed_lo, kp.seed_hi, static_cast<uint32_t>(center), 0u);
    const float4 dc = ray_at<MODEL>(kp, x, y);
    float4 ph;
    float cost;
    uint32_t sel = 0;
    if (BR == kInitRandom) {
        const float depth = fmaf(rs.uniform(), kp.depth_max - kp.depth_min, kp.depth_min);
        ph = random_normal(dc, rs);
        ph.w = dist_to_origin(dc, depth, ph);
        cost = initial_cost<MODEL, VB, VMAXB, TF, PNEG>(kp, x, y, pt, ph, &sel, cvec);
    } else if (BR == kInitPlanar) {
        if (kp.mask[center] > 0 && kp.costs_rm[center] >= 0.1f) {
            const float perturbation = 0.02f;
            const float4 prior = kp.prior[center];
            float dp = prior.w;
            const float dmin_p = (1 - 3 * perturbation) * dp;
            const float dmax_p = (1 + 3 * perturbation) * dp;
            dp = fmaf(rs.uniform(), dmax_p - dmin_p, dmin_p);
            ph = perturbed_normal(dc, prior, rs, static_cast<float>(3 * perturbation * kMPi));
            ph.w = dp;
        } else {
            ph = kp.planes_rm[center];
            const float depth = ph.w;
            ph.w = dist_to_origin(dc, depth, ph);
        }
        cost = initial_cost<MODEL, VB, VMAXB, TF, PNEG>(kp, x, y, pt, ph, &sel, cvec);
    } else if (BR == kInitUpsample) {
        const float scale = static_cast<float>(1.0 * static_cast<double>(kp.scaled_cols) / static_cast<double>(kp.W));
        const float sigmad = 0.50f, sigmar = 25.5f;
        const int Imagescale = f2i_sat(fmaxf(static_cast<float>(kp.W) / kp.scaled_cols,
                                             static_cast<float>(kp.H) / kp.scaled_rows));
        const int nn = (Imagescale * Imagescale + 1) / 2;
        const float o_y = static_cast<float>(y) * scale, o_x = static_cast<float>(x) * scale;
        const float* ref = rc.img_base;
        const float refPix = texel_padded(ref, rc.img_pitch, rc.W, rc.H, x, y);
        float nf = 0.0f;
        float nx = 0.f, ny = 0.f, nz = 0.f;
        for (int j = -nn; j <= nn; ++j) {
            int r_y = f2i_sat(o_y + static_cast<float>(j));
            r_y = (r_y > 0 ? (static_cast<float>(r_y) < kp.scaled_rows ? r_y : f2i_sat(kp.scaled_rows - 1)) : 0);
            const int r_ys = y + j;
            for (int i = -nn; i <= nn; ++i) {
                int r_x = f2i_sat(o_x + static_cast<float>(i));
                r_x = (r_x > 0 ? (static_cast<float>(r_x) < kp.scaled_cols ? r_x : f2i_sat(kp.scaled_cols - 1)) : 0);
                const int s_center = f2i_sat(static_cast<float>(r_y) * kp.scaled_cols + static_cast<float>(r_x));
                const float4 sn = kp.scaled[s_center];
                const float nbPix = texel_padded(ref, rc.img_pitch, rc.W, rc.H, x + i, r_ys);
                const float tg = spatial_gauss(o_x, o_y, static_cast<float>(r_x), static_cast<float>(r_y), sigmad) *
                                 range_gauss(fabsf(refPix - nbPix), sigmar);
                nf += tg;
                nx = nx + sn.x * tg;
                ny = ny + sn.y * tg;
                nz = nz + sn.z * tg;
            }
        }
        nx = nx / nf; ny = ny / nf; nz = nz / nf;
        normalize3(nx, ny, nz);
        const float4 cur = kp.planes_rm[center];
        uint32_t sel0;
        kp.pre_rm[center] = initial_cost<MODEL, VB, VMAXB, TF, PNEG>(kp, x, y, pt, cur, &sel0);
        ph = to_ref(rc, make_float4(nx, ny, nz, 0.0f));
        ph.w = dist_to_origin(dc, cur.w, ph);
        cost = initial_cost<MODEL, VB, VMAXB, TF, PNEG>(kp, x, y, pt, ph, &sel, cvec);
    } else {
        ph = kp.hier ? kp.scaled[center] : kp.planes_rm[center];
        ph = to_ref(rc, ph);
        const float depth = ph.w;
        ph.w = dist_to_origin(dc, depth, ph);
        cost = initial_cost<MODEL, VB, VMAXB, TF, PNEG>(kp, x, y, pt, ph, &sel, cvec);
    }
    kp.plane_cs[colour][ci] = ph;
    kp.cost_cs[colour][ci] = cost;
    kp.sel_cs[colour][ci] = sel;
    kp.rng_cs[colour][ci] = rs.n;
}


__device__ __forceinline__ float cost_at(const KParams& kp, int x, int y) {
    const float* b = ((x + y) & 1) ? kp.cost_cs[1] : kp.cost_cs[0];
    return b[cs_index(kp, x, y)];
}
__device__ __forceinline__ float4 plane_at(const KParams& kp, int pos) {
    const int x = pos & 0xFFFF, y = pos >> 16;
    const float4* b = ((x + y) & 1) ? kp.plane_cs[1] : kp.plane_cs[0];
    return b[cs_index(kp, x, y)];
}
__device__ __forceinline__ int packpos(int x, int y) { return x | (y << 16); }

__device__ __forceinline__ int pick_neighbour(const KParams& kp, int d, int px, int py) {
    const int width = kp.W, height = kp.H;
    float cmin;
    int cpos;
    auto take = [&](bool ok, int x, int y) {
        const float c = cost_at(kp, x, y);
        const bool better = ok && c < cmin;
        cmin = better ? c : cmin;
        cpos = better ? packpos(x, y) : cpos;
    };
    switch (d) {
    case 1:
        if (!(py > 2)) return -1;
        cmin = cost_at(kp, px, py - 3); cpos = packpos(px, py - 3);
#pragma unroll
        for (int i = 1; i < 11; ++i) {
            const bool ok = py > 2 + 2 * i;
            take(ok, px, ok ? py - 3 - 2 * i : py - 3);
        }
        return cpos;
    case 3:
        if (!(py < height - 3)) return -1;
        cmin = cost_at(kp, px, py + 3); cpos = packpos(px, py + 3);
#pragma unroll
        for (int i = 1; i < 11; ++i) {
            const bool ok = py < height - 3 - 2 * i;
            take(ok, px, ok ? py + 3 + 2 * i : py + 3);
        }
        return cpos;
    case 5:
        if (!(px > 2)) return -1;
        cmin = cost_at(kp, px - 3, py); cpos = packpos(px - 3, py);
#pragma unroll
        for (int i = 1; i < 11; ++i) {
            const bool ok = px > 2 + 2 * i;
            take(ok, ok ? px - 3 - 2 * i : px - 3, py);
        }
        return cpos;
    case 7:
        if (!(px < width - 3)) return -1;
        cmin = cost_at(kp, px + 3, py); cpos = packpos(px + 3, py);
#pragma unroll
        for (int i = 1; i < 11; ++i) {
            const bool ok = px < width - 3 - 2 * i;
            take(ok, ok ? px + 3 + 2 * i : px + 3, py);
        }
        return cpos;
    case 0:
        if (!(py > 0)) return -1;
        cmin = cost_at(kp, px, py - 1); cpos = packpos(px, py - 1);
#pragma unroll
        for (int i = 0; i < 3; ++i) {
            const bool a = py > 1 + i && px > i, b = py > 1 + i && px < width - 1 - i;
            take(a, a ? px - i : px, a ? py - 2 - i : py - 1);
            take(b, b ? px + i : px, b ? py - 2 - i : py - 1);
        }
        return cpos;
    case 2:
        if (!(py < height - 1)) return -1;
        cmin = cost_at(kp, px, py + 1); cpos = packpos(px, py + 1);
#pragma unroll
        for (int i = 0; i < 3; ++i) {
            const bool a = py < height - 2 - i && px > i, b = py < height - 2 - i && px < width - 1 - i;
            take(a, a ? px - i : px, a ? py + 2 + i : py + 1);
            take(b, b ? px + i : px, b ? py + 2 + i : py + 1);
        }
        return cpos;
    case 4:
        if (!(px > 0)) return -1;
// ... 31 lines not shown
    return kp.dead[0] && *((ConstWord*)(kp.dead_any)) != 0u;
}
__device__ __forceinline__ bool dead_pixel(const KParams& kp, int colour, long long ci) {
    const uint8_t* m = colour ? kp.dead[1] : kp.dead[0];
    return dead_view(kp) && m[ci];
}

constexpr int kEvalVB = 4;
constexpr bool kNbPipeExact = false, kNbPipeFast = true;
#ifndef ACMMP_NB_PIN_VB
#define ACMMP_NB_PIN_VB 2
#endif
template <int MODEL, int VB, int FM>
constexpr int nb_vb() {
    constexpr int cap = (MODEL == kPinhole && FM) ? ACMMP_NB_PIN_VB : kEvalVB;
    return VB > cap ? cap : VB;
}
constexpr int kNbLanes = 8;

static inline size_t nb_lds_bytes(int model, int S, int nside, int npix = kNbPix) {
    return model == kSphere ? (sizeof(float4) * S + sizeof(float) * nside) * npix
                            : (sizeof(float4) + sizeof(float)) * S * npix;
}

template <int MODEL, int NPIX = kNbPix, int NLANES = kNbLanes>
__device__ __forceinline__ Patch coop_patch_nb(const KParams& kp, bool valid, int px, int py, int lp, int h,
                                               float4* lds) {
    float4* rw = lds + lp;
    float* tail = reinterpret_cast<float*>(lds + NPIX * kp.S);
    float* rr = tail + lp;
    if (valid) {
        const DevCam& rc = kp.cams[0];
        const float center = texel_padded(rc.img_base, rc.img_pitch, rc.W, rc.H, px, py);
        for (int s = h; s < kp.S; s += NLANES) {
            const int i = -kp.R + (s / kp.nside) * kp.inc, j = -kp.R + (s % kp.nside) * kp.inc;
            float r;
            const float4 q = patch_sample<MODEL>(kp, px, py, s, i, j, center, r);
            if (MODEL == kSphere) {
                rw[s * NPIX] = make_float4(q.x, q.z, q.w, r);
                if (s < kp.nside) rr[s * NPIX] = q.y;
            } else {
                rw[s * NPIX] = q;
                rr[s * NPIX] = r;
            }
        }
    }
    __syncthreads();
    Patch pt;
    pt.rw = rw; pt.rr = rr; pt.wr = nullptr; pt.row = pt.col = nullptr; pt.stride = NPIX;
    pt.center = 0.f;
    pt.sbw = 0.f; pt.sref = 0.f; pt.srr = 0.f;
    if (MODEL == kSphere && valid) {
        for (int s = 0; s < kp.S; ++s) {
            patch_fold_sample(rw[s * NPIX].z, rw[s * NPIX].w, pt);
        }
    }
    return pt;
}

constexpr size_t kNbMaskBytes = 8 * (256 / 64);
__device__ __forceinline__ void stage_neg_mask(const KParams& kp, bool valid, Patch& pt, int h, float4* lds) {
    uint32_t* words = reinterpret_cast<uint32_t*>(reinterpret_cast<float*>(lds + kNbPix * kp.S) + kNbPix * kp.nside) +
                      2 * uniform_int(static_cast<int>(threadIdx.x >> 6));
    const bool live = valid && !(pt.sbw < 1e-6f);
    const float lim = kp.neg_tau * pt.sbw;
    unsigned long long keep = 0ull;
    for (int s0 = 0; s0 < kp.S; s0 += kNbLanes) {
        const int s = s0 + h;
        const bool k = live && s < kp.S && !(pt.rw[(s < kp.S ? s : 0) * kNbPix].z <= lim);
        unsigned long long b = __ballot(k);
        b |= b >> 32; b |= b >> 16; b |= b >> 8;
        keep |= (b & 0xffull) << s0;
    }
    const unsigned long long neg = ~keep & ((1ull << 36) - 1ull);
    if ((threadIdx.x & 63u) == 0u) {
        words[0] = static_cast<uint32_t>(neg);
        words[1] = static_cast<uint32_t>(neg >> 32);
    }
    pt.neg = words;
}

static inline size_t sep_lds_bytes(int S, int nside, int npix) { return (8 * static_cast<size_t>(S) + 16 * nside) * npix; }

template <int NPIX, int NLANES>
__device__ __forceinline__ Patch coop_patch_sep(const KParams& kp, bool valid, int px, int py, int lp, int h,
                                                float4* lds) {
    float2* base = reinterpret_cast<float2*>(lds);
    float2* wr = base + lp * kp.S;
    float2* row = base + NPIX * kp.S + lp * 2 * kp.nside;
    float2* col = row + kp.nside;
    if (valid) {
        const DevCam& rc = kp.cams[0];
        const float center = texel_padded(rc.img_base, rc.img_pitch, rc.W, rc.H, px, py);
        for (int s = h; s < kp.S; s += NLANES) {
            const int i = -kp.R + (s / kp.nside) * kp.inc, j = -kp.R + (s % kp.nside) * kp.inc;
            float r;
            const float4 q = patch_sample<kSphere>(kp, px, py, s, i, j, center, r);
            wr[s] = make_float2(q.w, r);
        }
        for (int k = h; k < kp.nside; k += NLANES) {
            row[k] = kp.sph_row[py - kp.R + k * kp.inc + kp.R];
            col[k] = kp.sph_col[px - kp.R + k * kp.inc + kp.R];
        }
    }
    __syncthreads();
    Patch pt;
    pt.rw = nullptr; pt.rr = nullptr; pt.wr = wr; pt.row = row; pt.col = col; pt.stride = 1;
    pt.center = 0.f;
    pt.sbw = 0.f; pt.sref = 0.f; pt.srr = 0.f;
    if (valid) {
        for (int s = 0; s < kp.S; ++s) {
            patch_fold_sample(wr[s].x, wr[s].y, pt);
        }
    }
    return pt;
}

constexpr bool kRefPipe = true;
template <int MODEL, int VB>
constexpr int ref_vb() { return (VB == 4 || (VB > 4 && MODEL == kSphere)) ? 2 : (VB > kEvalVB ? kEvalVB : VB); }
template <int MODEL, int VB, int TF>
constexpr int ref_vb_eval() {
    return (MODEL == kPinhole && TF == 2 && ref_vb<MODEL, VB>() > 2) ? 2 : ref_vb<MODEL, VB>();
}

#if ACMMP_IN_TU(0)
__global__ __launch_bounds__(256) void k_pick(const KParams kp, const int colour) {
    const long long q = static_cast<long long>(blockIdx.x) * blockDim.x + threadIdx.x;
    const int d = blockIdx.y;
    static_assert(kNbFixRegions == 256, "one counter per thread of block (0, 0)");
    if (kp.nbfix && blockIdx.x == 0 && d == 0) kp.nbfix_count[threadIdx.x] = 0u;
    int px = 0, py = 0;
    if (!colour_pixel(kp, colour, q, px, py)) return;
    const long long ci = static_cast<long long>(py) * kp.Wh + (px >> 1);
    if (dead_pixel(kp, colour, ci)) return;
    kp.nbpos[d * kp.Pc + ci] = pick_neighbour(kp, d, px, py);
}

#endif

template <int MODEL, int VB, int TEX, int FM, int NEG = 0>
#ifndef ACMMP_NB_PIN_WAVES
#define ACMMP_NB_PIN_WAVES 5
#endif
#ifndef ACMMP_NB_SPH_WAVES
#define ACMMP_NB_SPH_WAVES 5
#endif
__global__ __launch_bounds__(256, MODEL == kSphere ? (FM ? ACMMP_NB_SPH_WAVES : 8) : (FM ? ACMMP_NB_PIN_WAVES : 1)) void k_eval_nb(
    const KParams kp, const int colour) {
    extern __shared__ float4 lds4[];
    const int t = threadIdx.x;
    const int lp = t / kNbLanes, h = t - lp * kNbLanes;
    long long wrow = 0, wcol = 0;
    if (kp.nb_tile) {
        const int tpr = (kp.Wh + 7) >> 3;
        const int tr = static_cast<int>(blockIdx.x) / tpr;
        wrow = tr * 4 + (t >> 6);
        wcol = (static_cast<int>(blockIdx.x) - tr * tpr) * 8;
    }
    const long long q = kp.nb_tile ? wrow * kp.Wh + wcol + (lp & 7) : static_cast<long long>(blockIdx.x) * kNbPix + lp;
    int px = 0, py = 0;
    const long long Pc = kp.Pc;
    bool dead = false;
    if (MODEL == kSphere) dead = dead_pixel(kp, colour, min(static_cast<long long>(kp.row_lo) * kp.Wh + q, Pc - 1));
    bool valid = (!kp.nb_tile || wcol + (lp & 7) < kp.Wh) && colour_pixel(kp, colour, q, px, py);
    const long long ci = static_cast<long long>(py) * kp.Wh + (px >> 1);
    if (dead) valid = false;
    Patch pt = coop_patch_nb<MODEL>(kp, valid, px, py, lp, h, lds4);
    if constexpr (NEG) stage_neg_mask(kp, valid, pt, h, lds4);
    const int busy = __syncthreads_count(valid && h == 0 && !(MODEL == kSphere && pt.sbw < 1e-6f));
    if (t == 0 && busy && kp.nb_count_work) atomicAdd(kp.work + (blockIdx.x & 255u), static_cast<unsigned long long>(busy));
    if (!valid) return;
    const int pos = kp.nbpos[h * Pc + ci];
    if (pos < 0) return;
    const float4 ph = plane_at(kp, pos);
    const uint32_t all = kp.nb_views;
    const uint32_t wbase = static_cast<uint32_t>(uniform_int(static_cast<int>(
        kp.nb_tile ? (kp.row_lo + wrow) * kp.Wh + wcol : kp.row_lo * kp.Wh + blockIdx.x * kNbPix + (t >> 6) * 8)));
    const uint32_t fixkey = kp.nbfix ? wbase : kFixNone;
    for_all_views_t<MODEL, nb_vb<MODEL, VB, FM>(), 3, FM ? kNbPipeFast : kNbPipeExact, TEX, FM, NEG ? 2 : 1>(
        kp, px, py, pt, ph, all, [&](int v, float c) {
            const int l = lane_id_here();
            kp.hyp_cost[(static_cast<long long>(l & 7) * kp.V + v) * Pc + (wbase + (l >> 3))] = c;
        }, fixkey);
}

constexpr int kFixLanes = 6, kFixPerWave = 64 / kFixLanes, kFixPerBlock = 4 * kFixPerWave;

template <int TEX>
__device__ __forceinline__ void fix_row(const KParams& kp, int px, int py, float4 ph, int v, int j, float4* smp) {
    typedef const __attribute__((address_space(4))) DevCam ConstCam;
    const DevCam& rc = kp.cams[0];
    const float center = texel_padded(rc.img_base, rc.img_pitch, rc.W, rc.H, px, py);
// ... 392 lines not shown
                    cur_plane = nb;
                    cur_cost = fmin;
                    src_cur = min_idx;
                }
            }
        }
    }

    float4 plane_now = cur_plane;
    int src_now = src_cur;
    if (!kp.planar) {
        const int mpos = sel_pos(min_idx);
        if (mpos >= 0) {
            const float4 nb = plane_at(kp, mpos);
            const float db = depth_from_plane(nb, dc);
            const float fmin = sel_f(final_costs, min_idx);
            if (db >= kp.depth_min && db <= kp.depth_max && fmin < cost_now) {
                depth_now = db;
                plane_now = nb;
                cost_now = fmin;
                cur_sel = temp_sel;
                src_now = min_idx;
            }
        }
    }

    uint32_t flags = use_prior ? 1u : 0u;
    if (weight_norm > 0.0f) {
        flags |= 2u;
        const float perturbation = 0.02f;
        const float depth_sigma = (kp.depth_max - kp.depth_min) / 64.0f;
        const float angle_sigma = kCudartPiF * (5.0f / 180.0f);
        float depth_rand;
        float4 n_rand;
        if (use_prior) {
            const float4 prior = kp.prior[center];
            const float dprior = depth_from_plane(prior, dc);
            depth_rand = sample_depth_inv(rs, fmaxf(dprior - 3 * depth_sigma, kp.depth_min),
                                          fminf(dprior + 3 * depth_sigma, kp.depth_max));
            n_rand = perturbed_normal(dc, prior, rs, angle_sigma);
        } else {
            depth_rand = sample_depth_inv(rs, kp.depth_min, kp.depth_max);
            n_rand = random_normal(dc, rs);
        }
        float lo = fmaxf((1.0f - perturbation) * depth_now, kp.depth_min);
        float hi = fminf((1.0f + perturbation) * depth_now, kp.depth_max);
        if (!(hi > lo)) { lo = kp.depth_min; hi = kp.depth_max; }
        float depth_perturbed = depth_now;
        bool ok = false;
        for (int k = 0; k < 32; ++k) {
            const float cand = sample_depth_inv(rs, lo, hi);
            if (cand >= kp.depth_min && cand <= kp.depth_max) { depth_perturbed = cand; ok = true; break; }
        }
        if (!ok) depth_perturbed = fminf(fmaxf(depth_now, kp.depth_min), kp.depth_max);
        const float4 n_pert = perturbed_normal(dc, plane_now, rs, perturbation * kCudartPiF);
#pragma unroll
        for (int i = 0; i < 5; ++i) {
            const float dep = (i == 0 || i == 2) ? depth_rand : (i == 4 ? depth_perturbed : depth_now);
            float4 tp = (i == 1 || i == 2) ? n_rand : (i == 3 ? n_pert : plane_now);
            tp.w = dist_to_origin(dc, dep, tp);
            kp.cand[i * Pc + ci] = tp;
            kp.cand_dep[i * Pc + ci] = dep;
        }
    }
    PixState st;
    st.plane_now = plane_now;
    st.cur_plane = cur_plane;
    st.vw = make_uint4(vwp[0], vwp[1], vwp[2], vwp[3]);
    st.cost_now = cost_now;
    st.depth_now = depth_now;
    st.cur_cost = cur_cost;
    st.restricted_cost = restricted_cost;
    st.cur_sel = cur_sel;
    st.flags = flags;
    st.weight_norm = weight_norm;
    st.src = static_cast<uint32_t>(src_now) | (static_cast<uint32_t>(src_cur) << 8);
    kp.pst[ci] = st;
    kp.rng_cs[colour][ci] = rs.n;
}

#ifndef ACMMP_REF_INTERP_WAVES
#define ACMMP_REF_INTERP_WAVES 4
#endif
template <int MODEL, int VB, bool GEOM, int TF, bool PNEG = false>
__global__ __launch_bounds__(256, (MODEL == kSphere && VB > 4 && TF == 2) ? ACMMP_REF_INTERP_WAVES : 1) void k_eval_ref(const KParams kp, const int colour) {
    extern __shared__ float4 lds4[];
    const int t = threadIdx.x;
    const int lp = t / kRefLanes, h = t - lp * kRefLanes;
    const long long q = static_cast<long long>(blockIdx.x) * kRefPix + lp;
    int px = 0, py = 0;
    bool valid = t < kRefPix * kRefLanes && colour_pixel(kp, colour, q, px, py);
    const long long Pc = kp.Pc;
    const long long ci = valid ? static_cast<long long>(py) * kp.Wh + (px >> 1) : 0;
    uint4 vw = make_uint4(0u, 0u, 0u, 0u);
    float weight_norm = 0.0f;
    if (valid) {
        const PixState& st = kp.pst[ci];
        valid = (st.flags & 2u) != 0u;
        vw = st.vw;
        weight_norm = st.weight_norm;
    }
    constexpr int kStaged = (MODEL == kSphere && VB <= 4) ? 4 : 3;
    Patch pt;
    if constexpr (kStaged == 4) pt = coop_patch_sep<kRefPix, kRefLanes>(kp, valid, px, py, lp, h, lds4);
    else pt = coop_patch_nb<MODEL, kRefPix, kRefLanes>(kp, valid, px, py, lp, h, lds4);
    constexpr int VBA = ref_vb_eval<MODEL, VB, TF>();
    if (!valid) return;
    if (kp.ref_split > 0 && h == 0) {
        const DevCam& rc = kp.cams[0];
        kp.psum[ci] = make_float4(pt.sbw, pt.sref, pt.srr,
                                  texel_padded(rc.img_base, rc.img_pitch, rc.W, rc.H, px, py));
    }
    const float4 dc = ray_at<MODEL>(kp, px, py);
    const float4 tp = kp.cand[h * Pc + ci];
    const float depth_before = depth_from_plane(tp, dc);
    if (depth_before < kp.depth_min || depth_before > kp.depth_max || depth_before >= 1e6f) return;
    const uint32_t vwp[4] = {vw.x, vw.y, vw.z, vw.w};
    uint32_t mask = 0u;
    for (int v = 0; v < kp.V; ++v) if (vw_get(vwp, v) > 0.0f) mask |= 1u << v;
    float temp_cost = 0.0f;
    const uint32_t umask = wave_or(mask, kp.V);
    const int S = kp.ref_split;
    const bool split = S > 0 && __any(!(MODEL == kSphere && pt.sbw < 1e-6f));
    const uint32_t amask = split ? (umask & ((1u << S) - 1u)) : umask;
    float* vcost = kp.cand_vcost + static_cast<long long>(h) * kp.V * Pc + ci;
    for (int v = 0; v < kp.V; ++v)
        if (!((amask >> v) & 1u)) vcost[v * Pc] = __builtin_nanf("");
    constexpr bool kRefInterp = MODEL == kSphere && kStaged == 3 && TF == 2;
    uint32_t rough = 0u;
    for_all_views_tf<MODEL, VBA, kStaged, kRefPipe, TF, kRefPipe, PNEG>(kp, px, py, pt, tp, amask, [&](int v, float c) {
        vcost[v * Pc] = c;
        const bool r = kRefInterp && c != c;
        if (r) rough |= 1u << v;
        const float w = vw_get(vwp, v);
        if (w > 0.0f && !r) {
            if (GEOM) temp_cost = fmaf(w, fmaf(0.1f, geom_cost<MODEL>(kp, v + 1, tp, px, py, dc), c), temp_cost);
            else temp_cost = fmaf(w, c, temp_cost);
        }
    }, kRefInterp ? kFixNan : kFixNone);
    const float partial = temp_cost / weight_norm;
    if (!split) { kp.cand_cost[h * Pc + ci] = partial; return; }
    const PixState& st = kp.pst[ci];
    const bool done = !(st.flags & 1u) && !(partial < st.cost_now);
    kp.cand_cost[h * Pc + ci] = done ? partial : temp_cost;
    if constexpr (kRefInterp) {
        const uint32_t need = done ? 0u : (rough & mask);
        if (!done) kp.cand_rough[h * Pc + ci] = need;
        const unsigned long long any = __ballot(need != 0u);
        if (any) {
            const int lane = lane_id_here();
            const unsigned region = blockIdx.x % kNbFixRegions;
            for (int v = 0; v < S; ++v) {
                const bool redo = (need >> v) & 1u;
                const unsigned long long b = __ballot(redo);
                if (!b) continue;
                const int leader = __ffsll(static_cast<long long>(b)) - 1;
                unsigned base = 0u;
                if (lane == leader) base = atomicAdd(kp.nbfix_count + region, static_cast<unsigned>(__popcll(b)));
                base = __builtin_amdgcn_readlane(base, leader);
                const unsigned slot = base + static_cast<unsigned>(__popcll(b & ((1ull << lane) - 1ull)));
                if (redo && slot < kp.nbfix_cap)
                    kp.nbfix[static_cast<long long>(region) * kp.nbfix_cap + slot] =
                        (static_cast<uint32_t>(ci) << 8) | (static_cast<uint32_t>(h) << 5) | static_cast<uint32_t>(v);
            }
        }
    }
    const unsigned long long b = __ballot(!done);
    if (b) {
        const int lane = __lane_id();
        const int leader = __ffsll(static_cast<long long>(b)) - 1;
        unsigned base = 0u;
        if (lane == leader) base = atomicAdd(kp.surv_count + blockIdx.x, static_cast<unsigned>(__popcll(b)));
        base = __shfl(base, leader);
        if (!done)
            kp.surv[static_cast<long long>(blockIdx.x) * kRefSlots + base + __popcll(b & ((1ull << lane) - 1ull))] =
                static_cast<uint32_t>(ci * 8 + h);
    }
}

#if ACMMP_IN_TU(4)
__global__ __launch_bounds__(1024) void k_tail_scan(const KParams kp, const int nref) {
    constexpr int kPass = 8192, kPer = kPass / 1024;
    __shared__ unsigned cnt[kPass];
    __shared__ unsigned part[1024];
    const int t = threadIdx.x;
    unsigned carry = 0u;
    for (int base = 0; base < nref; base += kPass) {
        const int m = min(kPass, nref - base);
        for (int i = t; i < m; i += 1024) cnt[i] = kp.surv_count[base + i];
        __syncthreads();
        unsigned v[kPer], sum = 0u;
#pragma unroll
        for (int k = 0; k < kPer; ++k) {
            v[k] = t * kPer + k < m ? cnt[t * kPer + k] : 0u;
            sum += v[k];
        }
        part[t] = sum;
        __syncthreads();
        for (int off = 1; off < 1024; off <<= 1) {
            const unsigned add = t >= off ? part[t - off] : 0u;
            __syncthreads();
            part[t] += add;
            __syncthreads();
        }
        unsigned acc = carry + part[t] - sum;
#pragma unroll
        for (int k = 0; k < kPer; ++k) {
            cnt[t * kPer + k] = acc;
            acc += v[k];
        }
        carry += part[1023];
        __syncthreads();
        for (int i = t; i < m; i += 1024) kp.surv_pre[base + i] = cnt[i];
        __syncthreads();
    }
    if (t == 0) kp.surv_pre[nref] = carry;
}

__global__ __launch_bounds__(256) void k_tail_compact(const KParams kp) {
    const int b = blockIdx.x, r = threadIdx.x;
    if (r < static_cast<int>(kp.surv_count[b]))
        kp.surv_dense[kp.surv_pre[b] + r] = kp.surv[static_cast<long long>(b) * kRefSlots + r];
}
#endif

template <int MODEL, int VB, bool GEOM, int TF, bool PNEG = false>
__global__ __launch_bounds__(256) void k_eval_ref_tail(const KParams kp, const int colour, const int nref) {
    const unsigned total = kp.surv_pre[nref];
    const unsigned x = blockIdx.x & 7u, k = blockIdx.x >> 3, nk = gridDim.x >> 3;
    const unsigned seg0 = static_cast<unsigned>(static_cast<unsigned long long>(total) * x / 8u);
    const unsigned seg1 = static_cast<unsigned>(static_cast<unsigned long long>(total) * (x + 1u) / 8u);
    const long long Pc = kp.Pc;
    const int S = kp.ref_split;
    for (unsigned i = seg0 + k * 256u + threadIdx.x; i < seg1; i += nk * 256u) {
        const uint32_t rec = kp.surv_dense[i];
        const long long ci = rec >> 3;
        const int h = static_cast<int>(rec & 7u);
        const int py = static_cast<int>(ci / kp.Wh);
        const int px = 2 * static_cast<int>(ci - static_cast<long long>(py) * kp.Wh) + ((py + colour) & 1);
        const PixState& st = kp.pst[ci];
        const uint4 vw = st.vw;
        const float weight_norm = st.weight_norm;
        const uint32_t vwp[4] = {vw.x, vw.y, vw.z, vw.w};
        constexpr bool kRefInterp = MODEL == kSphere && VB > 4 && TF == 2;
        const uint32_t need = kRefInterp ? kp.cand_rough[h * Pc + ci] : 0u;
        uint32_t mask = 0u;
        for (int v = S; v < kp.V; ++v) if (vw_get(vwp, v) > 0.0f) mask |= 1u << v;
        const uint32_t umask = wave_or(mask, kp.V);
        const float4 dc = ray_at<MODEL>(kp, px, py);
        const float4 tp = kp.cand[h * Pc + ci];
        Patch pt;
        const float4 ps = kp.psum[ci];
        pt.rw = nullptr; pt.rr = nullptr; pt.wr = nullptr; pt.row = pt.col = nullptr; pt.stride = 0;
        pt.sbw = ps.x; pt.sref = ps.y; pt.srr = ps.z; pt.center = ps.w;
        float temp_cost = need ? 0.0f : kp.cand_cost[h * Pc + ci];
        float* vcost = kp.cand_vcost + static_cast<long long>(h) * kp.V * Pc + ci;
        auto add_term = [&](int v, float c) {
            const float w = vw_get(vwp, v);
            if (w > 0.0f) {
                if (GEOM) temp_cost = fmaf(w, fmaf(0.1f, geom_cost<MODEL>(kp, v + 1, tp, px, py, dc), c), temp_cost);
                else temp_cost = fmaf(w, c, temp_cost);
            }
        };
        if (kRefInterp && need)
            for (int v = 0; v < S; ++v) add_term(v, vcost[v * Pc]);
#ifndef ACMMP_TAIL_SPH_VB
#define ACMMP_TAIL_SPH_VB 4
#endif
#ifndef ACMMP_TAIL_PIN_VB
#define ACMMP_TAIL_PIN_VB 4
#endif
        constexpr int VBT = (MODEL == kSphere && VB > 4) ? ACMMP_TAIL_SPH_VB
                          : (MODEL == kPinhole && VB > 4) ? ACMMP_TAIL_PIN_VB : ref_vb<MODEL, VB>();
        for_all_views_tf<MODEL, VBT, 0, kRefPipe, TF, kRefPipe, PNEG>(kp, px, py, pt, tp, umask, [&](int v, float c) {
            vcost[v * Pc] = c;
            add_term(v, c);
        });
        kp.cand_cost[h * Pc + ci] = temp_cost / weight_norm;
    }
}

template <int MODEL>
__global__ __launch_bounds__(256) void k_finish(const KParams kp, const int colour, const SweepOut out) {
    const long long q = static_cast<long long>(blockIdx.x) * blockDim.x + threadIdx.x;
    int px = 0, py = 0;
    if (!colour_pixel(kp, colour, q, px, py)) return;
    const long long Pc = kp.Pc;
    const long long ci = static_cast<long long>(py) * kp.Wh + (px >> 1);
    const long long center = static_cast<long long>(py) * kp.W + px;
    const float4 dc = ray_at<MODEL>(kp, px, py);
    const PixState st = kp.pst[ci];
    float4 plane_now = st.plane_now;
    float cost_now = st.cost_now;
    float restricted_cost = st.restricted_cost;
    int src_now = static_cast<int>(st.src & 255u);
    const int src_cur = static_cast<int>((st.src >> 8) & 255u);
    if (st.flags & 2u) {
        const bool use_prior = (st.flags & 1u) != 0u;
        const float gamma = 0.5f;
        const float depth_sigma = (kp.depth_max - kp.depth_min) / 64.0f;
        const float two_dss = 2 * depth_sigma * depth_sigma;
        const float angle_sigma = kCudartPiF * (5.0f / 180.0f);
        const float two_ass = 2 * angle_sigma * angle_sigma;
        const float beta = 0.18f;
        float4 prior = make_float4(0.f, 0.f, 0.f, 0.f);
        float dprior = 0.f;
        if (use_prior) {
            prior = kp.prior[center];
            dprior = depth_from_plane(prior, dc);
        }
        for (int i = 0; i < 5; ++i) {
            const float4 tp = kp.cand[i * Pc + ci];
            const float depth_before = depth_from_plane(tp, dc);
            if (depth_before < kp.depth_min || depth_before > kp.depth_max || depth_before >= 1e6f) continue;
            const float temp_cost = kp.cand_cost[i * Pc + ci];
            if (use_prior) {
                const float ddiff = kp.cand_dep[i * Pc + ci] - dprior;
                const float ac = fminf(fmaxf(dot3n(prior, tp), -1.0f), 1.0f);
                const float ad = det_acos(ac);
                const float pr = fmaf(det_exp((-ddiff) * ddiff / two_dss), det_exp((-ad) * ad / two_ass), gamma);
                const float rtc = det_exp((-temp_cost) * temp_cost / beta) * pr;
                if (rtc > restricted_cost) {
                    plane_now = tp; cost_now = temp_cost; restricted_cost = rtc; src_now = 9 + i;
                }
            } else if (temp_cost < cost_now) {
                plane_now = tp;
                cost_now = temp_cost;
                src_now = 9 + i;
            }
        }
    }
    float4 cur_plane = st.cur_plane;
    float cur_cost = st.cur_cost;
    int src = src_cur;
    if (kp.hier) {
// ... 200 lines not shown
#if ACMMP_IN_TU(0)
hipError_t launch_to_f16_pairs(const float* src, int W, int H, uint32_t* dst, int* inexact, hipStream_t s) {
    const long long n = static_cast<long long>(W + 2) * (H + 1);
    k_to_f16_pairs<<<static_cast<unsigned>((n + 255) / 256), 256, 0, s>>>(src, W + 2, H + 1, dst, inexact);
    return hipGetLastError();
}


hipError_t launch_pad_image(const float* src, size_t pitch_floats, int W, int H, float* dst, int dst_pitch,
                            hipStream_t s) {
    dim3 blk(64, 4), grd(cdiv(W + 2, 64), cdiv(H + 2, 4));
    k_pad_image<<<grd, blk, 0, s>>>(src, pitch_floats, W, H, dst, dst_pitch);
    return hipGetLastError();
}

hipError_t launch_ray_tables(const KParams& kp, float4* dirs, float2* sph_row, float2* sph_col, hipStream_t s) {
    if (kp.model == kSphere) {
        const int n = std::max(kp.W, kp.H) + 2 * kp.R;
        k_ray_tables<<<dim3(cdiv(n, 256), 2), dim3(256, 1), 0, s>>>(kp, dirs, sph_row, sph_col);
    } else {
        dim3 blk(64, 4), grd(cdiv(kp.W + 2 * kp.R, 64), cdiv(kp.H + 2 * kp.R, 4));
        k_ray_tables<<<grd, blk, 0, s>>>(kp, dirs, sph_row, sph_col);
    }
    return hipGetLastError();
}

hipError_t launch_spatial_table(const KParams& kp, float* spatial, hipStream_t s) {
    const int rows = kp.model == kSphere ? kp.H : 1;
    k_spatial<<<cdiv(rows, 64), 64, 0, s>>>(kp, spatial);
    return hipGetLastError();
}

#endif

static inline int pick_vb(int V) { return V <= 1 ? 1 : (V <= 2 ? 2 : (V <= 4 ? 4 : 8)); }

static inline bool uses_fix_queue(const KParams& kp, bool refinement) {
    return kp.nbfix && kp.model == kSphere && kp.fast && kp.tex16 && kp.interp && (!refinement || kp.V > 4);
}

static inline size_t ref_lds_bytes(const KParams& kp) {
    return (kp.model == kSphere && pick_vb(kp.V) <= 4) ? sep_lds_bytes(kp.S, kp.nside, kRefPix)
                                                       : nb_lds_bytes(kp.model, kp.S, kp.nside, kRefPix);
}

static inline int ref_block_count(const KParams& kp) {
    return cdiv(static_cast<long long>(kp.row_hi - kp.row_lo) * kp.Wh, kRefPix);
}

#define ACMMP_DISPATCH(MODEL_RT, V_RT, BODY)                                             \
    do {                                                                                \
        const int vb_ = pick_vb(V_RT);                                                  \
        if ((MODEL_RT) == kSphere) {                                                    \
            constexpr int M = kSphere;                                                  \
            if (vb_ == 1) { constexpr int VBC = 1; BODY; }                              \
            else if (vb_ == 2) { constexpr int VBC = 2; BODY; }                         \
            else if (vb_ == 4) { constexpr int VBC = 4; BODY; }                         \
            else { constexpr int VBC = 8; BODY; }                                       \
        } else {                                                                        \
            constexpr int M = kPinhole;                                                 \
            if (vb_ == 1) { constexpr int VBC = 1; BODY; }                              \
            else if (vb_ == 2) { constexpr int VBC = 2; BODY; }                         \
            else if (vb_ == 4) { constexpr int VBC = 4; BODY; }                         \
            else { constexpr int VBC = 8; BODY; }                                       \
        }                                                                               \
    } while (0)

#define ACMMP_DISPATCH_TF(KP, BODY)                                                     \
    do {                                                                                \
        const int tf_ = tf_of(KP);                                                      \
        if (tf_ == 2) { constexpr int TF = 2; BODY; }                                   \
        else if (tf_ == 1) { constexpr int TF = 1; BODY; }                              \
        else { constexpr int TF = 0; BODY; }                                            \
    } while (0)

template <int M, int VBC, int TF>
constexpr bool ref_neg_inst() { return M == kSphere && VBC <= 4 && TF == 2; }

#if ACMMP_IN_TU(1)
template <int M, int BR, int VBC, int TF>
static void launch_init_inst(const KParams& kp, dim3 grd, dim3 blk, hipStream_t s) {
    if constexpr (ref_neg_inst<M, VBC, TF>()) {
        if (kp.ref_neg_tau >= 0.0f) {
            k_init<M, kInitVB, BR, VBC, TF, true><<<grd, blk, 0, s>>>(kp);
            return;
        }
    }
    k_init<M, kInitVB, BR, VBC, TF><<<grd, blk, 0, s>>>(kp);
}

hipError_t launch_init(const KParams& kp, hipStream_t s) {
    if (kp.init_hi <= kp.init_lo) return hipSuccess;
    dim3 blk(16, 16), grd(xcd_grid(static_cast<long long>(cdiv(kp.W, 16)) * cdiv(kp.init_hi - kp.init_lo, 16)));
    const int br = (!kp.geom && !kp.hier) ? kInitRandom : kp.planar ? kInitPlanar : kp.upsample ? kInitUpsample
                                                                                                 : kInitReuse;
    if (br == kInitRandom) ACMMP_DISPATCH_TF(kp, ACMMP_DISPATCH(kp.model, kp.V, (launch_init_inst<M, kInitRandom, VBC, TF>(kp, grd, blk, s))));
    else if (br == kInitPlanar)
        ACMMP_DISPATCH_TF(kp, ACMMP_DISPATCH(kp.model, kp.V, (launch_init_inst<M, kInitPlanar, VBC, TF>(kp, grd, blk, s))));
    else if (br == kInitUpsample)
        ACMMP_DISPATCH_TF(kp, ACMMP_DISPATCH(kp.model, kp.V, (launch_init_inst<M, kInitUpsample, VBC, TF>(kp, grd, blk, s))));
    else ACMMP_DISPATCH_TF(kp, ACMMP_DISPATCH(kp.model, kp.V, (launch_init_inst<M, kInitReuse, VBC, TF>(kp, grd, blk, s))));
    return hipGetLastError();
}

hipError_t launch_debug(const KParams& kp, int which, int n, const int* px, const int* py, const float4* planes,
                        float* out, hipStream_t s) {
    dim3 blk(64), grd(cdiv(n, 64));
    ACMMP_DISPATCH(kp.model, kp.V, (k_debug<M, VBC><<<grd, blk, 0, s>>>(kp, which, n, px, py, planes, out)));
    return hipGetLastError();
}

#endif

hipError_t launch_eval_nb(const KParams& kp, int colour, hipStream_t s);
hipError_t launch_eval_nb_views(const KParams& kp, int colour, hipStream_t s);
hipError_t launch_select(const KParams& kp, int colour, int iter, hipStream_t s);
hipError_t launch_eval_ref(const KParams& kp, int colour, hipStream_t s);

template <int TEX, int LANES>
__global__ __launch_bounds__(256) void k_debug_nb_fix(const KParams kp, const int* __restrict__ qx,
                                                      const int* __restrict__ qy, const float4* __restrict__ planes,
                                                      float* __restrict__ out) {
    __shared__ float4 smp[kFixPerBlock][36];
    const int t = threadIdx.x, l = t & 63;
    const int ew = l / kFixLanes, j = l - ew * kFixLanes, e = (t >> 6) * kFixPerWave + ew;
    const unsigned region = blockIdx.x % kNbFixRegions, stripes = gridDim.x / kNbFixRegions;
    const unsigned n = min(kp.nbfix_count[region], kp.nbfix_cap);
    const uint32_t* qu = kp.nbfix + static_cast<long long>(region) * kp.nbfix_cap;
    for (unsigned i0 = (blockIdx.x / kNbFixRegions) * kFixPerBlock; i0 < n; i0 += stripes * kFixPerBlock) {
        const unsigned i = i0 + static_cast<unsigned>(e);
        const bool act = ew < kFixPerWave && i < n;
        long long k = 0;
        int v = 0;
        if (act) {
            const uint32_t key = qu[i];
            const int qq = static_cast<int>(key >> 8), h = static_cast<int>((key >> 5) & 7u);
            v = static_cast<int>(key & 31u);
            k = static_cast<long long>(qq) * LANES + h;
            fix_row<TEX>(kp, qx[qq], qy[qq], planes[k], v, j, smp[e]);
        }
        __syncthreads();
        if (act && j == 0) out[k * kp.V + v] = fix_fold(smp[e]);
        __syncthreads();
    }
}

#if ACMMP_IN_TU(2)
int nb_view_chunk(const KParams& kp) {
    const char* e = std::getenv("ACMMP_NB_VIEW_CHUNK");
    int c = e ? std::atoi(e) : 0;
    if (!e) {
        const double bytes = 4.0 * (kp.W + 2) * (kp.H + 2) * kp.V;
        c = (kp.V > 8 && bytes > 160e6) ? 8 : 0;
    }
    return (c <= 0 || c >= kp.V) ? kp.V : c;
}

int nb_tile_order(const KParams&) {
    const char* e = std::getenv("ACMMP_NB_TILE");
    return e ? (std::atoi(e) != 0) : 1;
}

hipError_t launch_eval_nb(const KParams& kp0, int colour, hipStream_t s) {
    KParams kp = kp0;
    const bool fix = uses_fix_queue(kp, false);
    if (!fix) kp.nbfix = nullptr;
    const int chunk = kp.nb_chunk;
// ... 31 lines not shown
    float* o = out + k * kp.V;
    const uint32_t all = kp.V >= 32 ? 0xFFFFFFFFu : ((1u << kp.V) - 1u);
    const uint32_t fixkey = kp.nbfix ? static_cast<uint32_t>(uniform_int(static_cast<int>(blockIdx.x * kNbPix + (t >> 6) * 8))) : kFixNone;
    for_all_views_t<MODEL, nb_vb<MODEL, VB, FM>(), 3, FM ? kNbPipeFast : kNbPipeExact, TEX, FM, NEG ? 2 : 1>(
        kp, px, py, pt, ph, all, [&](int v, float c) { o[v] = c; }, fixkey);
}

hipError_t launch_debug_nb(const KParams& kp0, int n, const int* px, const int* py, const float4* planes, float* out,
                           hipStream_t s) {
    KParams kp = kp0;
    const bool fix = uses_fix_queue(kp, false) && n < (1 << 24);
    if (!fix) kp.nbfix = nullptr;
    if (fix && static_cast<long long>(cdiv(cdiv(n, kNbPix), kNbFixRegions)) * 256 * kp.V > kp.nbfix_cap)
        return hipErrorInvalidValue;
    hipError_t e0 = hipSuccess;
    if (fix && (e0 = hipMemsetAsync(kp.nbfix_count, 0, sizeof(unsigned) * kNbFixRegions, s)) != hipSuccess) return e0;
    const size_t lds_nb = nb_lds_bytes(kp.model, kp.S, kp.nside);
    const size_t lds_neg = lds_nb + kNbMaskBytes;
    const dim3 grd = static_cast<unsigned>(cdiv(n, kNbPix));
    if (kp.fast) {
        if (kp.tex16 && kp.neg_tau >= 0.0f) ACMMP_DISPATCH(kp.model, kp.V, (k_debug_nb<M, VBC, 1, 1, M == kSphere><<<grd, 256, lds_neg, s>>>(kp, n, px, py, planes, out)));
        else if (kp.tex16) ACMMP_DISPATCH(kp.model, kp.V, (k_debug_nb<M, VBC, 1, 1><<<grd, 256, lds_nb, s>>>(kp, n, px, py, planes, out)));
        else ACMMP_DISPATCH(kp.model, kp.V, (k_debug_nb<M, VBC, 0, 1><<<grd, 256, lds_nb, s>>>(kp, n, px, py, planes, out)));
    } else {
        if (kp.tex16) ACMMP_DISPATCH(kp.model, kp.V, (k_debug_nb<M, VBC, 1, 0><<<grd, 256, lds_nb, s>>>(kp, n, px, py, planes, out)));
        else ACMMP_DISPATCH(kp.model, kp.V, (k_debug_nb<M, VBC, 0, 0><<<grd, 256, lds_nb, s>>>(kp, n, px, py, planes, out)));
    }
    if (fix) k_debug_nb_fix<1, kNbLanes><<<kNbFixRegions, 256, 0, s>>>(kp, px, py, planes, out);
    return hipGetLastError();
}

hipError_t launch_eval_nb_views(const KParams& kp, int colour, hipStream_t s) {
    const size_t lds_nb = nb_lds_bytes(kp.model, kp.S, kp.nside);
    const size_t lds_neg = lds_nb + kNbMaskBytes;
    const dim3 grd = static_cast<unsigned>(nb_block_count(kp.row_hi - kp.row_lo, kp.Wh, kp.nb_tile));
    if (kp.fast) {
        if (kp.tex16 && kp.neg_tau >= 0.0f) ACMMP_DISPATCH(kp.model, kp.V, (k_eval_nb<M, VBC, 1, 1, M == kSphere><<<grd, 256, lds_neg, s>>>(kp, colour)));
        else if (kp.tex16) ACMMP_DISPATCH(kp.model, kp.V, (k_eval_nb<M, VBC, 1, 1><<<grd, 256, lds_nb, s>>>(kp, colour)));
        else ACMMP_DISPATCH(kp.model, kp.V, (k_eval_nb<M, VBC, 0, 1><<<grd, 256, lds_nb, s>>>(kp, colour)));
    } else {
        if (kp.tex16) ACMMP_DISPATCH(kp.model, kp.V, (k_eval_nb<M, VBC, 1, 0><<<grd, 256, lds_nb, s>>>(kp, colour)));
        else ACMMP_DISPATCH(kp.model, kp.V, (k_eval_nb<M, VBC, 0, 0><<<grd, 256, lds_nb, s>>>(kp, colour)));
    }
    return hipGetLastError();
}
#endif

#if ACMMP_IN_TU(3)
hipError_t launch_select(const KParams& kp, int colour, int iter, hipStream_t s) {
    const long long npix = static_cast<long long>(kp.row_hi - kp.row_lo) * kp.Wh;
    const int vs = kp.V <= 4 ? pick_vb(kp.V) : (kp.V <= 8 ? 8 : (kp.V <= 16 ? 16 : 32));
#define ACMMP_SELECT(MV)                                                                                              \
    do {                                                                                                              \
        if (kp.model == kSphere) {                                                                                    \
            constexpr bool N = MV <= 4;         \
            if (kp.ref_neg_tau >= 0.0f && N) {                                                                        \
                if (kp.geom) k_select<kSphere, MV, true, N><<<cdiv(npix, 256), 256, 0, s>>>(kp, colour, iter);        \
                else k_select<kSphere, MV, false, N><<<cdiv(npix, 256), 256, 0, s>>>(kp, colour, iter);               \
            } else if (kp.geom) k_select<kSphere, MV, true><<<cdiv(npix, 256), 256, 0, s>>>(kp, colour, iter);        \
            else k_select<kSphere, MV, false><<<cdiv(npix, 256), 256, 0, s>>>(kp, colour, iter);                      \
        } else {                                                                                                      \
            if (kp.geom) k_select<kPinhole, MV, true><<<cdiv(npix, 256), 256, 0, s>>>(kp, colour, iter);              \
            else k_select<kPinhole, MV, false><<<cdiv(npix, 256), 256, 0, s>>>(kp, colour, iter);                     \
        }                                                                                                             \
    } while (0)
    switch (vs) {
        case 1: ACMMP_SELECT(1); break;
        case 2: ACMMP_SELECT(2); break;
        case 4: ACMMP_SELECT(4); break;
        case 8: ACMMP_SELECT(8); break;
        case 16: ACMMP_SELECT(16); break;
        default: ACMMP_SELECT(32); break;
    }
#undef ACMMP_SELECT
    return hipGetLastError();
}
#endif

#if ACMMP_IN_TU(4)
template <int M, int VBC, bool GEOM, int TF>
static void launch_ref_inst(const KParams& kp, int colour, dim3 grd, size_t lds, hipStream_t s) {
    if constexpr (ref_neg_inst<M, VBC, TF>()) {
        if (kp.ref_neg_tau >= 0.0f) {
            k_eval_ref<M, VBC, GEOM, TF, true><<<grd, 256, lds, s>>>(kp, colour);
            return;
        }
    }
    k_eval_ref<M, VBC, GEOM, TF><<<grd, 256, lds, s>>>(kp, colour);
}
template <int M, int VBC, bool GEOM, int TF>
static void launch_tail_inst(const KParams& kp, int colour, int nref, dim3 grd, hipStream_t s) {
    if constexpr (ref_neg_inst<M, VBC, TF>()) {
        if (kp.ref_neg_tau >= 0.0f) {
            k_eval_ref_tail<M, VBC, GEOM, TF, true><<<grd, 256, 0, s>>>(kp, colour, nref);
            return;
        }
    }
    k_eval_ref_tail<M, VBC, GEOM, TF><<<grd, 256, 0, s>>>(kp, colour, nref);
}

hipError_t launch_eval_ref(const KParams& kp0, int colour, hipStream_t s) {
    KParams kp = kp0;
    if (kp.ref_split <= 0) kp.interp = 0;
    const size_t lds_ref = ref_lds_bytes(kp);
    hipError_t e = hipSuccess;
    const int nref = ref_block_count(kp);
    const dim3 grd_ref = static_cast<unsigned>(nref);
    const bool ref_fix = uses_fix_queue(kp, true);
    if (ref_fix && (e = hipMemsetAsync(kp.nbfix_count, 0, sizeof(unsigned) * kNbFixRegions, s)) != hipSuccess) return e;
    if (kp.geom) ACMMP_DISPATCH_TF(kp, ACMMP_DISPATCH(kp.model, kp.V, (launch_ref_inst<M, VBC, true, TF>(kp, colour, grd_ref, lds_ref, s))));
    else ACMMP_DISPATCH_TF(kp, ACMMP_DISPATCH(kp.model, kp.V, (launch_ref_inst<M, VBC, false, TF>(kp, colour, grd_ref, lds_ref, s))));
    if (ref_fix) k_nb_fix<1, true><<<16 * kNbFixRegions, 256, 0, s>>>(kp, colour);
    if (kp.ref_split > 0) {
#ifndef ACMMP_TAIL_NK
#define ACMMP_TAIL_NK 2048
#endif
        k_tail_scan<<<1, 1024, 0, s>>>(kp, nref);
        k_tail_compact<<<static_cast<unsigned>(nref), 256, 0, s>>>(kp);
        const unsigned grd = 8u * static_cast<unsigned>(std::min<long long>(ACMMP_TAIL_NK, std::max<long long>(1, cdiv(static_cast<long long>(nref) * kRefSlots, 8 * 256))));
        if (kp.geom) ACMMP_DISPATCH_TF(kp, ACMMP_DISPATCH(kp.model, kp.V, (launch_tail_inst<M, VBC, true, TF>(kp, colour, nref, grd, s))));
        else ACMMP_DISPATCH_TF(kp, ACMMP_DISPATCH(kp.model, kp.V, (launch_tail_inst<M, VBC, false, TF>(kp, colour, nref, grd, s))));
    }
    return hipGetLastError();
}

template <int MODEL, int VB, int TF, bool PNEG = false>
__global__ __launch_bounds__(256) void k_debug_ref(const KParams kp, int n, const int* __restrict__ qx,
                                                   const int* __restrict__ qy, const float4* __restrict__ planes,
                                                   float* __restrict__ out) {
    extern __shared__ float4 lds4[];
    const int t = threadIdx.x;
    const int lp = t / kRefLanes, h = t - lp * kRefLanes;
    const int q = blockIdx.x * kRefPix + lp;
    const bool valid = t < kRefPix * kRefLanes && q < n;
    const int px = valid ? qx[q] : 0, py = valid ? qy[q] : 0;
    constexpr int kStaged = (MODEL == kSphere && VB <= 4) ? 4 : 3;
    Patch pt;
    if constexpr (kStaged == 4) pt = coop_patch_sep<kRefPix, kRefLanes>(kp, valid, px, py, lp, h, lds4);
    else pt = coop_patch_nb<MODEL, kRefPix, kRefLanes>(kp, valid, px, py, lp, h, lds4);
    constexpr int VBA = ref_vb_eval<MODEL, VB, TF>();
    if (!valid) return;
    const long long k = static_cast<long long>(q) * kRefLanes + h;
    const float4 ph = planes[k];
    float* o = out + k * kp.V;
    const uint32_t all = kp.V >= 32 ? 0xFFFFFFFFu : ((1u << kp.V) - 1u);
    constexpr bool kRefInterp = MODEL == kSphere && kStaged == 3 && TF == 2;
    uint32_t rough = 0u;
    for_all_views_tf<MODEL, VBA, kStaged, kRefPipe, TF, kRefPipe, PNEG>(kp, px, py, pt, ph, all, [&](int v, float c) {
        o[v] = c;
        if (kRefInterp && c != c) rough |= 1u << v;
    }, kRefInterp && kp.nbfix ? kFixNan : kFixNone);
    if (kRefInterp && kp.nbfix) {
        const unsigned long long any = __ballot(rough != 0u);
        if (any) {
            const int lane = lane_id_here();
            const unsigned region = blockIdx.x % kNbFixRegions;
            for (int v = 0; v < kp.V; ++v) {
                const bool redo = (rough >> v) & 1u;
                const unsigned long long b = __ballot(redo);
                if (!b) continue;
                const int leader = __ffsll(static_cast<long long>(b)) - 1;
                unsigned base = 0u;
                if (lane == leader) base = atomicAdd(kp.nbfix_count + region, static_cast<unsigned>(__popcll(b)));
                base = __builtin_amdgcn_readlane(base, leader);
                const unsigned slot = base + static_cast<unsigned>(__popcll(b & ((1ull << lane) - 1ull)));
                if (redo && slot < kp.nbfix_cap)
                    kp.nbfix[static_cast<long long>(region) * kp.nbfix_cap + slot] =
                        (static_cast<uint32_t>(q) << 8) | (static_cast<uint32_t>(h) << 5) | static_cast<uint32_t>(v);
            }
        }
    }
}

template <int M, int VBC, int TF>
static void launch_debug_ref_inst(const KParams& kp, int n, const int* px, const int* py, const float4* planes, float* out,
                                  dim3 grd, size_t lds, hipStream_t s) {
    if constexpr (ref_neg_inst<M, VBC, TF>()) {
// ... 72 lines not shown
```

include/acmmp.h:

```cpp
#ifndef ACMMP_C_ABI_H
#define ACMMP_C_ABI_H

#include <stddef.h>
#include <stdint.h>

#ifdef __cplusplus
extern "C" {
#endif

#define ACMMP_ABI_VERSION 1

#define ACMMP_PINHOLE 0
#define ACMMP_SPHERE 11

typedef struct acmmp_camera {
    int32_t model;
    float params[4];
    float R[9];
    float t[3];
    float K[9];
    int32_t width, height;
    float depth_min, depth_max;
} acmmp_camera;

// ... 38 lines not shown
typedef struct acmmp_fusion acmmp_fusion;
#define ACMMP_COMM_ID_BYTES 128

acmmp_status acmmp_create(int device, acmmp_ctx **out);
void acmmp_destroy(acmmp_ctx *ctx);
const char *acmmp_status_str(acmmp_status s);
const char *acmmp_last_error(const acmmp_ctx *ctx);
int acmmp_abi_version(void);

int acmmp_device_count(void);

enum { ACMMP_MATH_EXACT = 0, ACMMP_MATH_FAST = 1 };
acmmp_status acmmp_set_math(acmmp_ctx *ctx, int mode);
int acmmp_get_math(const acmmp_ctx *ctx);

acmmp_status acmmp_set_params(acmmp_ctx *ctx, const acmmp_params *params);

acmmp_status acmmp_upload_views(acmmp_ctx *ctx, int n, const float *const *images,
                                const size_t *pitch_bytes, const acmmp_camera *cams);

acmmp_status acmmp_upload_views_device(acmmp_ctx *ctx, int n, const float *const *dev_images,
                                       const size_t *pitch_bytes, const acmmp_camera *cams);

acmmp_status acmmp_image_cache_create(int device, size_t budget_bytes, acmmp_image_cache **out);
void acmmp_image_cache_destroy(acmmp_image_cache *cache);
acmmp_status acmmp_image_cache_stats(acmmp_image_cache *cache, unsigned long long out[5]);

acmmp_status acmmp_upload_views_keyed(acmmp_ctx *ctx, acmmp_image_cache *cache, int n, const uint64_t *keys,
                                      const float *const *images, const size_t *pitch_bytes,
                                      const acmmp_camera *cams, int device_src);

acmmp_status acmmp_upload_depths(acmmp_ctx *ctx, int n, const float *const *depths,
                                 const int *w, const int *h);

acmmp_status acmmp_upload_depths_device(acmmp_ctx *ctx, int n, const float *const *dev_depths,
                                        const int *w, const int *h);

acmmp_status acmmp_export_depth(acmmp_ctx *ctx, float *dev_dst);

acmmp_status acmmp_set_state(acmmp_ctx *ctx, const float *planes, const float *costs);

acmmp_status acmmp_export_state(acmmp_ctx *ctx, float *dev_planes, float *dev_costs);
acmmp_status acmmp_set_state_device(acmmp_ctx *ctx, const float *dev_planes, const float *dev_costs);

acmmp_status acmmp_set_scaled_state(acmmp_ctx *ctx, const float *planes, int sw, int sh);

acmmp_status acmmp_set_planar_prior(acmmp_ctx *ctx, const float *prior_planes, const uint32_t *masks);

acmmp_status acmmp_run_patchmatch(acmmp_ctx *ctx, uint64_t seed);

acmmp_status acmmp_run_patchmatch_ex(acmmp_ctx *ctx, uint64_t seed, int n_half_sweeps, int do_post);

acmmp_status acmmp_download(acmmp_ctx *ctx, float *planes, float *costs);
acmmp_status acmmp_download_aux(acmmp_ctx *ctx, uint32_t *selected_views, float *pre_costs);

acmmp_status acmmp_device_outputs(acmmp_ctx *ctx, void **planes, void **costs);

acmmp_status acmmp_synchronize(acmmp_ctx *ctx);

acmmp_status acmmp_last_timing(const acmmp_ctx *ctx, float ms[3]);

acmmp_status acmmp_last_kernel_timing(const acmmp_ctx *ctx, float ms[4], int launches[4]);

acmmp_status acmmp_last_work(const acmmp_ctx *ctx, unsigned long long *evaluated, unsigned long long *total);

acmmp_status acmmp_last_planar_timing(const acmmp_ctx *ctx, float ms[4]);

int acmmp_texel_bytes(const acmmp_ctx *ctx);

#define ACMMP_BAND_HALO 23

int acmmp_strip_plan(int rows, int want_strips, int *bounds, int *waits);

acmmp_status acmmp_band_begin(acmmp_ctx *ctx, uint64_t seed, int row0, int row1);
acmmp_status acmmp_band_sweep(acmmp_ctx *ctx, int *colour);
int acmmp_band_sweeps_left(const acmmp_ctx *ctx);
acmmp_status acmmp_band_halo_ranges(const acmmp_ctx *ctx, int ranges[8]);
acmmp_status acmmp_band_copy_rows(acmmp_ctx *dst, acmmp_ctx *src, int colour, int row_a, int row_b);
acmmp_status acmmp_band_get_rows(acmmp_ctx *ctx, int colour, int row_a, int row_b, float *planes, float *costs,
                                 uint32_t *selected_views);
acmmp_status acmmp_band_set_rows(acmmp_ctx *ctx, int colour, int row_a, int row_b, const float *planes,
                                 const float *costs, const uint32_t *selected_views);
acmmp_status acmmp_debug_band_cvec(acmmp_ctx *ctx, int colour, int row_a, int row_b, float *out);
acmmp_status acmmp_band_end(acmmp_ctx *ctx, int do_post);


acmmp_status acmmp_device_alloc(int device, size_t bytes, void **ptr);
acmmp_status acmmp_device_free(int device, void *ptr);
acmmp_status acmmp_memcpy(int device, void *dst, const void *src, size_t bytes, int kind);

acmmp_status acmmp_device_checksum(int device, const void *ptr, size_t bytes, uint64_t *out);

acmmp_status acmmp_device_identity(int device, char *pci_bus_id, int len, uint8_t uuid[16]);
acmmp_status acmmp_clock_probe(int device, float warm_ms, double out[4]);

acmmp_status acmmp_comm_unique_id(uint8_t id[ACMMP_COMM_ID_BYTES]);
acmmp_status acmmp_comm_create(int device, const uint8_t id[ACMMP_COMM_ID_BYTES], int nranks, int rank,
                               acmmp_comm **out);
void acmmp_comm_destroy(acmmp_comm *comm);

acmmp_status acmmp_comm_after(acmmp_comm *comm, acmmp_ctx *ctx);

acmmp_status acmmp_comm_broadcast(acmmp_comm *comm, int n, void *const *bufs, const size_t *bytes,
                                  const int *roots);

acmmp_status acmmp_comm_allreduce_max(acmmp_comm *comm, double *vals, int n);

acmmp_status acmmp_comm_band_exchange(acmmp_comm *comm, acmmp_ctx *ctx, int colour, int rank_up, int rank_down);

acmmp_status acmmp_run_patchmatch_band(acmmp_ctx *ctx, acmmp_comm *comm, uint64_t seed, int row0, int row1,
                                       int rank_up, int rank_down);

acmmp_status acmmp_fusion_create(int device, int n_views, const acmmp_camera *cams, acmmp_fusion **out);
acmmp_status acmmp_fusion_set_view(acmmp_fusion *f, int view, const float *depth, const float *normals,
                                   const uint8_t *bgr);
acmmp_status acmmp_fusion_run(acmmp_fusion *f, int ref, int n_src, const int *src_views, float *points, int cap,
                              int *n_points);
const char *acmmp_fusion_last_error(const acmmp_fusion *f);
void acmmp_fusion_destroy(acmmp_fusion *f);

#define ACMMP_FUSE_UNIQUE 1
acmmp_status acmmp_fusion_run_scene(acmmp_fusion *f, int n_refs, const int *refs, const int *n_src,
                                    const int *src_views, int flags, int *counts, int64_t *n_points);
acmmp_status acmmp_fusion_scene_points(acmmp_fusion *f, int64_t first, int64_t n, float *points,
                                       int32_t *ref_index, int32_t *pixel, uint32_t *src_mask);
acmmp_status acmmp_fusion_reset_used(acmmp_fusion *f);
acmmp_status acmmp_fusion_download_used(acmmp_fusion *f, int view, uint8_t *mask);

acmmp_status acmmp_fusion_voxelize(acmmp_fusion *f, float voxel_size, const float *origin, int min_points,
                                   int64_t *n_voxels, int64_t *n_occupied, int64_t *n_rejected, float *origin_used);
acmmp_status acmmp_fusion_voxel_points(acmmp_fusion *f, int64_t first, int64_t n, float *points, int32_t *counts);
acmmp_status acmmp_fusion_voxel_table(acmmp_fusion *f, int64_t force_slots, int64_t *slots, int64_t *occupied,
                                      int64_t *max_probe, int64_t *wrapped);

acmmp_status acmmp_fusion_set_scene(acmmp_fusion *f, int64_t n, const float *points, const int32_t *ref_index,
                                    const int32_t *pixel, const uint32_t *src_mask);

acmmp_status acmmp_fusion_voxel_clean(acmmp_fusion *f, int connectivity, int min_neighbours,
                                      int64_t min_component_voxels, int64_t min_component_points, int64_t *n_kept,
                                      int64_t *n_components, int64_t *n_components_kept, int64_t *n_unsupported,
                                      int64_t *rounds);
acmmp_status acmmp_fusion_clean_points(acmmp_fusion *f, int64_t first, int64_t n, float *points, int32_t *counts,
                                       int64_t *component);
acmmp_status acmmp_fusion_voxel_labels(acmmp_fusion *f, int64_t first, int64_t n, int64_t *label, int32_t *support);
acmmp_status acmmp_fusion_component_table(acmmp_fusion *f, int64_t first, int64_t n, int64_t *root, int64_t *voxels,
                                          int64_t *points);

#define ACMMP_VIS_FROM_VOXELS 0
#define ACMMP_VIS_FROM_CLEAN 1
acmmp_status acmmp_fusion_voxel_visibility(acmmp_fusion *f, int source, int n_list, const int *views, float rel_tol,
                                           int radius, int min_support, int max_conflicts, int64_t *n_kept,
                                           int64_t *n_unsupported, int64_t *n_conflicting, int64_t class_totals[4]);
acmmp_status acmmp_fusion_visible_points(acmmp_fusion *f, int64_t first, int64_t n, float *points, int32_t *counts,
                                         int32_t *tallies);
acmmp_status acmmp_fusion_visibility_tallies(acmmp_fusion *f, int64_t first, int64_t n, int32_t *tallies);

#define ACMMP_MESH_FROM_VOXELS 0
#define ACMMP_MESH_FROM_CLEAN 1
#define ACMMP_MESH_FROM_VISIBLE 2
acmmp_status acmmp_fusion_voxel_mesh(acmmp_fusion *f, int source, int n_list, const int *views, float trunc,
                                     int min_weight, int64_t *n_vertices, int64_t *n_faces, int64_t *n_samples,
                                     int64_t *n_valid, int64_t *n_cubes, int64_t *n_uncoloured);
acmmp_status acmmp_fusion_mesh_vertices(acmmp_fusion *f, int64_t first, int64_t n, float *vertices);
acmmp_status acmmp_fusion_mesh_faces(acmmp_fusion *f, int64_t first, int64_t n, int32_t *faces);
acmmp_status acmmp_fusion_mesh_samples(acmmp_fusion *f, int64_t first, int64_t n, int32_t *cells, int32_t *tsdf,
                                       int64_t *entry);
// ... 127 lines not shown
```

Before: 692.6.

## Publish per-pixel kept-sample mask at init and reuse it in propagation sweeps

```diff
diff --git a/acmmp-spherical_amd/acmmp/capi.py b/acmmp-spherical_amd/acmmp/capi.py
--- a/acmmp-spherical_amd/acmmp/capi.py
+++ b/acmmp-spherical_amd/acmmp/capi.py
@@ -83,6 +83,7 @@
     "acmmp_download", "acmmp_download_aux", "acmmp_device_outputs", "acmmp_synchronize", "acmmp_last_timing",
     "acmmp_last_kernel_timing", "acmmp_last_work", "acmmp_last_planar_timing", "acmmp_texel_bytes", "acmmp_set_math", "acmmp_get_math", "acmmp_jbu",
     "acmmp_debug_ncc", "acmmp_debug_geom", "acmmp_debug_ncc_nb", "acmmp_debug_ncc_ref", "acmmp_debug_band_cvec",
+    "acmmp_debug_band_keep_mask", "acmmp_keep_mask_bytes",
     "acmmp_support_points", "acmmp_delaunay", "acmmp_prior_plane_params", "acmmp_depth_from_plane_param",
     "acmmp_planar_prior_host", "acmmp_set_planar_prior_from_maps", "acmmp_set_planar_prior_from_state",
     "acmmp_download_planar_prior",
@@ -114,6 +115,15 @@
 
 class AcmmpError(RuntimeError):
     pass
+
+
+def keep_mask_bytes(W: int, H: int, model: int = 11, patch_size: int = 11, radius_increment: int = 2, fast: bool = True,
+                    tex16: bool = True, n_src: int = 4, geom: bool = False) -> int:
+    n = int(load_library().acmmp_keep_mask_bytes(int(W), int(H), int(model), int(patch_size), int(radius_increment),
+                                                 int(bool(fast)), int(bool(tex16)), int(n_src), int(bool(geom))))
+    if n < 0:
+        raise AcmmpError(f"keep_mask_bytes: invalid arguments ({W} x {H})")
+    return n
 
 
 def strip_plan(rows: int, want_strips: int):
@@ -200,6 +210,9 @@
     L.acmmp_band_get_rows.argtypes = [vp, i32, i32, i32, vp, vp, vp]
     L.acmmp_band_set_rows.argtypes = [vp, i32, i32, i32, vp, vp, vp]
     L.acmmp_debug_band_cvec.argtypes = [vp, i32, i32, i32, vp]
+    L.acmmp_debug_band_keep_mask.argtypes = [vp, i32, i32, i32, vp]
+    L.acmmp_keep_mask_bytes.argtypes = [i32] * 9
+    L.acmmp_keep_mask_bytes.restype = C.c_longlong
     L.acmmp_band_end.argtypes = [vp, i32]
     L.acmmp_fusion_create.argtypes = [i32, i32, vp, C.POINTER(vp)]
     L.acmmp_fusion_set_view.argtypes = [vp, i32, vp, vp, vp]
@@ -586,6 +599,11 @@
         self._check(self.L.acmmp_debug_band_cvec(self.h, colour, row_a, row_b, _p(out)), "debug_band_cvec")
         return out
 
+    def debug_band_keep_mask(self, colour: int, row_a: int, row_b: int) -> np.ndarray:
+        out = np.empty((row_b - row_a) * ((self.W + 1) // 2), np.uint64)
+        self._check(self.L.acmmp_debug_band_keep_mask(self.h, colour, row_a, row_b, _p(out)), "debug_band_keep_mask")
+        return out
+
     def band_set_rows(self, colour: int, row_a: int, row_b: int, rows: np.ndarray):
         rows = np.asarray(rows, np.uint32).reshape(-1, 6)
         pl = np.ascontiguousarray(rows[:, :4]).view(np.float32)
diff --git a/acmmp-spherical_amd/csrc/capi.cpp b/acmmp-spherical_amd/csrc/capi.cpp
--- a/acmmp-spherical_amd/csrc/capi.cpp
+++ b/acmmp-spherical_amd/csrc/capi.cpp
@@ -862,6 +862,24 @@
     return ns;
 }
 
+static bool interp_geometry(int model, int nside, int R, int W, int H) {
+    return model == kSphere && nside == 6 && 2000LL * R <= 5LL * W && 1000LL * R <= 5LL * H;
+}
+static float ref_neg_tau_of(bool interp_geom, bool fast, bool tex16, int V) {
+    float tau = -1.0f;
+    if (interp_geom && fast && tex16 && V <= 4) {
+        tau = 0x1p-35f;
+        if (const char* e = std::getenv("ACMMP_REF_NEG_TAU")) tau = std::strtof(e, nullptr);
+        if (const char* e = std::getenv("ACMMP_REF_NEG_SKIP")) if (std::atoi(e) == 0) tau = -1.0f;
+    }
+    return tau;
+}
+static bool keep_mask_of(float ref_neg_tau, bool geom) {
+    bool keep = ref_neg_tau >= 0.0f && !geom;
+    if (const char* e = std::getenv("ACMMP_KEEP_MASK")) if (std::atoi(e) == 0) keep = false;
+    return keep;
+}
+
 static acmmp_status build_kparams(acmmp_ctx* c, KParams& kp, uint64_t seed, int want_strips = 1) {
     const acmmp_params& p = c->params;
     if (!c->has_params) return fail(c, ACMMP_ERR_STATE, "set_params first");
@@ -884,13 +902,10 @@
     kp.model = c->model;
     kp.W = c->W; kp.H = c->H; kp.Wh = Wh_of(c); kp.N = c->N; kp.V = c->N - 1;
     kp.R = R; kp.inc = p.radius_increment; kp.nside = nside; kp.S = nside * nside;
-    kp.interp = c->model == kSphere && nside == 6 && 2000LL * R <= 5LL * c->W && 1000LL * R <= 5LL * c->H;
-    kp.ref_neg_tau = -1.0f;
-    if (kp.interp && c->math == ACMMP_MATH_FAST && c->tex16 && kp.V <= 4) {
-        kp.ref_neg_tau = 0x1p-35f;
-        if (const char* e = std::getenv("ACMMP_REF_NEG_TAU")) kp.ref_neg_tau = std::strtof(e, nullptr);
-        if (const char* e = std::getenv("ACMMP_REF_NEG_SKIP")) if (std::atoi(e) == 0) kp.ref_neg_tau = -1.0f;
-    }
+    kp.interp = interp_geometry(c->model, nside, R, c->W, c->H);
+    kp.ref_neg_tau = ref_neg_tau_of(kp.interp, c->math == ACMMP_MATH_FAST, c->tex16, kp.V);
+    const bool keep = keep_mask_of(kp.ref_neg_tau, p.geom_consistency != 0);
+    kp.keep = keep ? 1 : 0;
     if (const char* e = std::getenv("ACMMP_INTERP")) kp.interp = kp.interp && std::atoi(e) != 0;
     kp.homog = 1;
     if (const char* e = std::getenv("ACMMP_PIN_HOMOG")) kp.homog = std::atoi(e) != 0;
@@ -992,7 +1007,7 @@
         piece(kp.cand_vcost, 5 * VP);
         piece(kp.surv, surv_n);
         piece(kp.surv_count, std::max(Pc / 51 + 2, ref_total));
-        piece(kp.psum, Pc);
+        piece(kp.psum, psum_count(Pc, keep));
         piece(kp.nbfix, kNbFixRegions * fix_total);
         piece(kp.nbfix_count, static_cast<size_t>(kNbFixRegions) * ns);
         piece(kp.surv_pre, std::max(Pc / 51 + 3, ref_total + ns));
@@ -1303,6 +1318,34 @@
     for (int v = 0; v < kp.V; ++v)
         HIP_TRY(c, d2h(out + static_cast<size_t>(v) * n, kp.cvec[colour] + static_cast<size_t>(v) * kp.Pc + off, sizeof(float) * n));
     return ACMMP_OK;
+}
+
+acmmp_status acmmp_debug_band_keep_mask(acmmp_ctx* c, int colour, int row_a, int row_b, uint64_t* out) {
+    if (!c || !out) return ACMMP_ERR_INVALID_ARGUMENT;
+    BandBuffers b{};
+    const acmmp_status st = band_buffers(c, colour, &b);
+    if (st != ACMMP_OK) return st;
+    if (row_a < 0 || row_b > c->H || row_a > row_b) return fail(c, ACMMP_ERR_INVALID_ARGUMENT, "rows out of range");
+    const KParams& kp = c->band_kp;
+    if (!kp.keep) return fail(c, ACMMP_ERR_STATE, "the run has no kept-sample mask");
+    if (row_a == row_b) return ACMMP_OK;
+    HIP_TRY(c, hipSetDevice(c->device));
+    HIP_TRY(c, hipStreamSynchronize(c->stream));
+    const size_t off = static_cast<size_t>(row_a) * b.Wh, n = static_cast<size_t>(row_b - row_a) * b.Wh;
+    HIP_TRY(c, d2h(out, keep_words(kp) + static_cast<size_t>(colour) * kp.Pc + off, sizeof(uint64_t) * n));
+    return ACMMP_OK;
+}
+
+long long acmmp_keep_mask_bytes(int W, int H, int model, int patch_size, int radius_increment, int fast, int tex16,
+                                int n_src, int geom) {
+    if (W < 1 || H < 1 || patch_size < 1 || radius_increment < 1 || n_src < 1) return -1;
+    const int R = patch_size / 2;
+    int nside = 0;
+    for (int i = -R; i <= R; i += radius_increment) ++nside;
+    const float tau = ref_neg_tau_of(interp_geometry(model, nside, R, W, H), fast != 0, tex16 != 0, n_src);
+    const bool keep = keep_mask_of(tau, geom != 0);
+    const size_t Pc = static_cast<size_t>(H) * ((W + 1) / 2);
+    return static_cast<long long>(sizeof(float4) * (psum_count(Pc, keep) - psum_count(Pc, false)));
 }
 
 acmmp_status acmmp_band_set_rows(acmmp_ctx* c, int colour, int row_a, int row_b, const float* planes, const float* costs,
diff --git a/acmmp-spherical_amd/csrc/engine.h b/acmmp-spherical_amd/csrc/engine.h
--- a/acmmp-spherical_amd/csrc/engine.h
+++ b/acmmp-spherical_amd/csrc/engine.h
@@ -118,11 +118,18 @@
     uint32_t* nbfix;
     unsigned* nbfix_count;
     unsigned nbfix_cap;
+    int keep;
     uint32_t* cand_rough;
     uint8_t* dead[2];
     unsigned* dead_any;
     unsigned* status;
 };
+static_assert(sizeof(KParams) == 568, "KParams is every kernel's first argument: a size change moves the ones behind it");
+
+inline size_t psum_count(size_t Pc, bool keep) { return keep ? 3 * Pc : Pc; }
+__host__ __device__ inline unsigned long long* keep_words(const KParams& kp) {
+    return reinterpret_cast<unsigned long long*>(kp.psum + 2 * kp.Pc);
+}
 
 struct SweepOut {
     float4* plane;
diff --git a/acmmp-spherical_amd/csrc/kernels.hip b/acmmp-spherical_amd/csrc/kernels.hip
--- a/acmmp-spherical_amd/csrc/kernels.hip
+++ b/acmmp-spherical_amd/csrc/kernels.hip
@@ -249,7 +249,11 @@
     float center;
     float sbw, sref, srr;
     const uint32_t* neg = nullptr;
+    unsigned long long keep = 0ull;
+    unsigned long long* keep_out = nullptr;
 };
+
+enum NegMode { kNegNone = 0, kNegTest = 1, kNegWord = 2, kNegPublish = 3 };
 
 typedef float float2u __attribute__((ext_vector_type(2), aligned(4)));
 
@@ -450,7 +454,7 @@
     asm volatile("v_mbcnt_lo_u32_b32 %0, -1, 0\n\tv_mbcnt_hi_u32_b32 %0, -1, %0" : "=v"(l));
     return l;
 }
-template <int MODEL, int VB, int STAGED, bool PIPE, int TEX, int FM = 0, bool FULL = false, int NB = 0, bool PNEG = false>
+template <int MODEL, int VB, int STAGED, bool PIPE, int TEX, int FM = 0, bool FULL = false, int NB = 0, int PNEG = kNegNone>
 __device__ __forceinline__ void ncc_chunk(const KParams& kp, int px, int py, const Patch& pt, float4 ph,
                                           const int (&vlist)[VB], int nv_rt, float (&cost)[VB],
                                           uint32_t fixkey = kFixNone) {
@@ -833,7 +837,8 @@
         }
     }
     if (!interp_done) {
-        const float neg_lim = PNEG ? kp.ref_neg_tau * pt.sbw : 0.f;
+        const float neg_lim = (PNEG == kNegTest || PNEG == kNegPublish) ? kp.ref_neg_tau * pt.sbw : 0.f;
+        [[maybe_unused]] unsigned long long published = 0ull;
 #define ACMMP_ACCUMULATE_N(v) ACMMP_ACCUMULATE_Z(v, tap[v], w, wwr, r, ok[v], PNEG && mine)
         int s = 0, ii = 0;
         for (int i = -R; i <= R; i += inc, ++ii) {
@@ -842,6 +847,11 @@
             for (int j = -R; j <= R; j += inc, ++s, ++jj) {
                 float r;
                 float4 rw;
+                bool mine = false;
+                if constexpr (PNEG == kNegWord) {
+                    mine = ((pt.keep >> s) & 1ull) != 0ull;
+                    if (__all(mine)) continue;
+                }
                 if (STAGED == 4) {
                     const float2 rs = pt.row[jj];
                     const float2 q = pt.wr[s];
@@ -859,8 +869,11 @@
                 } else {
                     rw = patch_sample<MODEL>(kp, px, py, s, i, j, pt.center, r);
                 }
-                const bool mine = PNEG && rw.w <= neg_lim;
-                if constexpr (PNEG) if (__all(mine)) continue;
+                if constexpr (PNEG == kNegTest || PNEG == kNegPublish) {
+                    mine = rw.w <= neg_lim;
+                    if constexpr (PNEG == kNegPublish) published |= static_cast<unsigned long long>(mine) << s;
+                    if (__all(mine)) continue;
+                }
                 const float w = mine ? 0.f : rw.w;
                 float3 P;
                 const float dep = FM ? depth_from_plane_fast(ph, rw) : depth_from_plane(ph, rw);
@@ -906,6 +919,7 @@
                 }
             }
         }
+        if constexpr (PNEG == kNegPublish) *pt.keep_out = published;
     }
 #undef ACMMP_ACCUMULATE
 #undef ACMMP_ACCUMULATE_N
@@ -993,7 +1007,7 @@
 }
 
 
-template <int MODEL, int VB, int STAGED, bool PIPE, int TEX, int FM, int NOFULL = 0, bool PNEG = false, typename F>
+template <int MODEL, int VB, int STAGED, bool PIPE, int TEX, int FM, int NOFULL = 0, int PNEG = kNegNone, typename F>
 __device__ __forceinline__ void for_all_views_t(const KParams& kp, int px, int py, const Patch& pt, float4 ph,
                                                 uint32_t wave_mask, F&& f, uint32_t fixkey = kFixNone) {
     int v = 0;
@@ -1039,14 +1053,14 @@
     }
 }
 
-template <int MODEL, int VB, int STAGED, bool PIPE, int TF, bool PIPE_FM = PIPE, bool PNEG = false, typename F>
+template <int MODEL, int VB, int STAGED, bool PIPE, int TF, bool PIPE_FM = PIPE, int PNEG = kNegNone, typename F>
 __device__ __forceinline__ void for_all_views_tf(const KParams& kp, int px, int py, const Patch& pt, float4 ph,
                                                  uint32_t wave_mask, F&& f, uint32_t fixkey = kFixNone) {
     if constexpr (TF == 0) {
         if (kp.fast) for_all_views_t<MODEL, VB, STAGED, PIPE_FM, 0, 1>(kp, px, py, pt, ph, wave_mask, f);
         else for_all_views_t<MODEL, VB, STAGED, PIPE, 0, 0>(kp, px, py, pt, ph, wave_mask, f);
     } else {
-        for_all_views_t<MODEL, VB, STAGED, TF == 2 ? PIPE_FM : PIPE, 1, TF == 2 ? 1 : 0, 0, PNEG && TF == 2 && MODEL == kSphere>(
+        for_all_views_t<MODEL, VB, STAGED, TF == 2 ? PIPE_FM : PIPE, 1, TF == 2 ? 1 : 0, 0, (TF == 2 && MODEL == kSphere) ? PNEG : kNegNone>(
             kp, px, py, pt, ph, wave_mask, f, fixkey);
     }
 }
@@ -1157,7 +1171,7 @@
     }
 }
 
-template <int MODEL, int VB, int VMAXB, int TF, bool PNEG = false>
+template <int MODEL, int VB, int VMAXB, int TF, int PNEG = kNegNone>
 __device__ float initial_cost(const KParams& kp, int px, int py, const Patch& pt, float4 ph, uint32_t* sel,
                               float* cvec = nullptr) {
     constexpr int VMAX = VMAXB < 8 ? VMAXB : kMaxViews;
@@ -1200,7 +1214,7 @@
 
 [[maybe_unused]] constexpr int kInitVB = 4;
 
-template <int MODEL, int VB, int BR, int VMAXB, int TF, bool PNEG = false>
+template <int MODEL, int VB, int BR, int VMAXB, int TF, int PNEG = kNegNone>
 __global__ __launch_bounds__(256) void k_init(const KParams kp) {
     const long long tile = xcd_block(blockIdx.x);
     const int tiles_x = (kp.W + 15) >> 4;
@@ -1211,7 +1225,9 @@
     const long long center = static_cast<long long>(y) * kp.W + x;
     const int colour = (x + y) & 1;
     const long long ci = cs_index(kp, x, y);
-    const Patch pt = make_patch<MODEL>(kp, x, y);
+    Patch pt = make_patch<MODEL>(kp, x, y);
+    [[maybe_unused]] unsigned long long kept = 0ull;
+    if constexpr (PNEG == kNegPublish) pt.keep_out = &kept;
     if (MODEL == kSphere && kp.dead[0]) {
         const bool dead = pt.sbw < 1e-6f;
         (colour ? kp.dead[1] : kp.dead[0])[ci] = dead ? 1 : 0;
@@ -1278,7 +1294,7 @@
         normalize3(nx, ny, nz);
         const float4 cur = kp.planes_rm[center];
         uint32_t sel0;
-        kp.pre_rm[center] = initial_cost<MODEL, VB, VMAXB, TF, PNEG>(kp, x, y, pt, cur, &sel0);
+        kp.pre_rm[center] = initial_cost<MODEL, VB, VMAXB, TF, PNEG == kNegPublish ? kNegTest : PNEG>(kp, x, y, pt, cur, &sel0);
         ph = to_ref(rc, make_float4(nx, ny, nz, 0.0f));
         ph.w = dist_to_origin(dc, cur.w, ph);
         cost = initial_cost<MODEL, VB, VMAXB, TF, PNEG>(kp, x, y, pt, ph, &sel, cvec);
@@ -1293,6 +1309,10 @@
     kp.cost_cs[colour][ci] = cost;
     kp.sel_cs[colour][ci] = sel;
     kp.rng_cs[colour][ci] = rs.n;
+    if constexpr (PNEG == kNegPublish) {
+        keep_words(kp)[colour * kp.Pc + ci] = kept;
+        kp.psum[colour * kp.Pc + ci] = make_float4(pt.sbw, pt.sref, pt.srr, pt.center);
+    }
 }
 
 
@@ -1490,17 +1510,20 @@
 
 static inline size_t sep_lds_bytes(int S, int nside, int npix) { return (8 * static_cast<size_t>(S) + 16 * nside) * npix; }
 
-template <int NPIX, int NLANES>
+template <int NPIX, int NLANES, bool KEEP = false>
 __device__ __forceinline__ Patch coop_patch_sep(const KParams& kp, bool valid, int px, int py, int lp, int h,
-                                                float4* lds) {
+                                                float4* lds, long long pi = 0) {
     float2* base = reinterpret_cast<float2*>(lds);
     float2* wr = base + lp * kp.S;
     float2* row = base + NPIX * kp.S + lp * 2 * kp.nside;
     float2* col = row + kp.nside;
+    [[maybe_unused]] unsigned long long keep = 0ull;
     if (valid) {
         const DevCam& rc = kp.cams[0];
         const float center = texel_padded(rc.img_base, rc.img_pitch, rc.W, rc.H, px, py);
+        if constexpr (KEEP) keep = keep_words(kp)[pi];
         for (int s = h; s < kp.S; s += NLANES) {
+            if (KEEP && ((keep >> s) & 1ull)) { wr[s] = make_float2(0.f, 0.f); continue; }
             const int i = -kp.R + (s / kp.nside) * kp.inc, j = -kp.R + (s % kp.nside) * kp.inc;
             float r;
             const float4 q = patch_sample<kSphere>(kp, px, py, s, i, j, center, r);
@@ -1516,7 +1539,13 @@
     pt.rw = nullptr; pt.rr = nullptr; pt.wr = wr; pt.row = row; pt.col = col; pt.stride = 1;
     pt.center = 0.f;
     pt.sbw = 0.f; pt.sref = 0.f; pt.srr = 0.f;
-    if (valid) {
+    if (KEEP) {
+        pt.keep = keep;
+        if (valid) {
+            const float4 ps = kp.psum[pi];
+            pt.sbw = ps.x; pt.sref = ps.y; pt.srr = ps.z;
+        }
+    } else if (valid) {
         for (int s = 0; s < kp.S; ++s) {
             patch_fold_sample(wr[s].x, wr[s].y, pt);
         }
@@ -2075,7 +2104,7 @@
 #ifndef ACMMP_REF_INTERP_WAVES
 #define ACMMP_REF_INTERP_WAVES 4
 #endif
-template <int MODEL, int VB, bool GEOM, int TF, bool PNEG = false>
+template <int MODEL, int VB, bool GEOM, int TF, int PNEG = kNegNone>
 __global__ __launch_bounds__(256, (MODEL == kSphere && VB > 4 && TF == 2) ? ACMMP_REF_INTERP_WAVES : 1) void k_eval_ref(const KParams kp, const int colour) {
     extern __shared__ float4 lds4[];
     const int t = threadIdx.x;
@@ -2095,11 +2124,11 @@
     }
     constexpr int kStaged = (MODEL == kSphere && VB <= 4) ? 4 : 3;
     Patch pt;
-    if constexpr (kStaged == 4) pt = coop_patch_sep<kRefPix, kRefLanes>(kp, valid, px, py, lp, h, lds4);
+    if constexpr (kStaged == 4) pt = coop_patch_sep<kRefPix, kRefLanes, PNEG == kNegWord>(kp, valid, px, py, lp, h, lds4, colour * Pc + ci);
     else pt = coop_patch_nb<MODEL, kRefPix, kRefLanes>(kp, valid, px, py, lp, h, lds4);
     constexpr int VBA = ref_vb_eval<MODEL, VB, TF>();
     if (!valid) return;
-    if (kp.ref_split > 0 && h == 0) {
+    if (PNEG != kNegWord && kp.ref_split > 0 && h == 0) {
         const DevCam& rc = kp.cams[0];
         kp.psum[ci] = make_float4(pt.sbw, pt.sref, pt.srr,
                                   texel_padded(rc.img_base, rc.img_pitch, rc.W, rc.H, px, py));
@@ -2217,7 +2246,7 @@
 }
 #endif
 
-template <int MODEL, int VB, bool GEOM, int TF, bool PNEG = false>
+template <int MODEL, int VB, bool GEOM, int TF, int PNEG = kNegNone>
 __global__ __launch_bounds__(256) void k_eval_ref_tail(const KParams kp, const int colour, const int nref) {
     const unsigned total = kp.surv_pre[nref];
     const unsigned x = blockIdx.x & 7u, k = blockIdx.x >> 3, nk = gridDim.x >> 3;
@@ -2243,7 +2272,9 @@
         const float4 dc = ray_at<MODEL>(kp, px, py);
         const float4 tp = kp.cand[h * Pc + ci];
         Patch pt;
-        const float4 ps = kp.psum[ci];
+        const long long pi = PNEG == kNegWord ? colour * Pc + ci : ci;
+        const float4 ps = kp.psum[pi];
+        if constexpr (PNEG == kNegWord) pt.keep = keep_words(kp)[pi];
         pt.rw = nullptr; pt.rr = nullptr; pt.wr = nullptr; pt.row = pt.col = nullptr; pt.stride = 0;
         pt.sbw = ps.x; pt.sref = ps.y; pt.srr = ps.z; pt.center = ps.w;
         float temp_cost = need ? 0.0f : kp.cand_cost[h * Pc + ci];
@@ -2610,7 +2641,8 @@
 static void launch_init_inst(const KParams& kp, dim3 grd, dim3 blk, hipStream_t s) {
     if constexpr (ref_neg_inst<M, VBC, TF>()) {
         if (kp.ref_neg_tau >= 0.0f) {
-            k_init<M, kInitVB, BR, VBC, TF, true><<<grd, blk, 0, s>>>(kp);
+            if (kp.keep) k_init<M, kInitVB, BR, VBC, TF, kNegPublish><<<grd, blk, 0, s>>>(kp);
+            else k_init<M, kInitVB, BR, VBC, TF, kNegTest><<<grd, blk, 0, s>>>(kp);
             return;
         }
     }
@@ -2808,7 +2840,13 @@
 static void launch_ref_inst(const KParams& kp, int colour, dim3 grd, size_t lds, hipStream_t s) {
     if constexpr (ref_neg_inst<M, VBC, TF>()) {
         if (kp.ref_neg_tau >= 0.0f) {
-            k_eval_ref<M, VBC, GEOM, TF, true><<<grd, 256, lds, s>>>(kp, colour);
+            if constexpr (!GEOM) {
+                if (kp.keep) {
+                    k_eval_ref<M, VBC, GEOM, TF, kNegWord><<<grd, 256, lds, s>>>(kp, colour);
+                    return;
+                }
+            }
+            k_eval_ref<M, VBC, GEOM, TF, kNegTest><<<grd, 256, lds, s>>>(kp, colour);
             return;
         }
     }
@@ -2818,7 +2856,13 @@
 static void launch_tail_inst(const KParams& kp, int colour, int nref, dim3 grd, hipStream_t s) {
     if constexpr (ref_neg_inst<M, VBC, TF>()) {
         if (kp.ref_neg_tau >= 0.0f) {
-            k_eval_ref_tail<M, VBC, GEOM, TF, true><<<grd, 256, 0, s>>>(kp, colour, nref);
+            if constexpr (!GEOM) {
+                if (kp.keep) {
+                    k_eval_ref_tail<M, VBC, GEOM, TF, kNegWord><<<grd, 256, 0, s>>>(kp, colour, nref);
+                    return;
+                }
+            }
+            k_eval_ref_tail<M, VBC, GEOM, TF, kNegTest><<<grd, 256, 0, s>>>(kp, colour, nref);
             return;
         }
     }
diff --git a/include/acmmp.h b/include/acmmp.h
--- a/include/acmmp.h
+++ b/include/acmmp.h
@@ -144,6 +144,9 @@
 acmmp_status acmmp_band_set_rows(acmmp_ctx *ctx, int colour, int row_a, int row_b, const float *planes,
                                  const float *costs, const uint32_t *selected_views);
 acmmp_status acmmp_debug_band_cvec(acmmp_ctx *ctx, int colour, int row_a, int row_b, float *out);
+acmmp_status acmmp_debug_band_keep_mask(acmmp_ctx *ctx, int colour, int row_a, int row_b, uint64_t *out);
+long long acmmp_keep_mask_bytes(int W, int H, int model, int patch_size, int radius_increment, int fast, int tex16,
+                                int n_src, int geom);
 acmmp_status acmmp_band_end(acmmp_ctx *ctx, int do_post);
 
 
```

After: 705.1 (median of 6 runs). +1.8%, better.
